# vt-asaplab/porla

Measured on AMD Instinct MI355X. Metric: BN254 G1 MSM Mscalar-mul/s at 2^20 pts, higher is better.
Workload: dtype u32x8 (256-bit modular integer); 1 GPU; KZG scheme, single 2^20-point BN254 G1 MSM per GPU, inputs resident in HBM, output 64-B affine point; pairs_per_gpu=1048576, msm_in_flight=2, warmup_steps_run=38, collective=none (single GPU)

## Files before the change

### include/porla_gpu.h

```cpp
#ifndef PORLA_GPU_H
#define PORLA_GPU_H
#include <stddef.h>
#include <stdint.h>

#if defined(__GNUC__)
#pragma GCC visibility push(default)
#endif
#ifdef __cplusplus
extern "C" {
#endif

#define PORLA_OK            0
#define PORLA_ERR_NO_DEVICE (-1)
#define PORLA_ERR_HIP       (-2)
#define PORLA_ERR_ARG       (-3)
#define PORLA_ERR_STATE     (-4)

#define PORLA_JACOBIAN_BYTES 96
#define PORLA_DIST_ID_BYTES  128

int         porla_gpu_device_count(void);
int         porla_gpu_set_device(int device);
const char *porla_gpu_last_error(void);
int         porla_shard_range(size_t n, int rank, int world, size_t *begin, size_t *end);
int         porla_gpu_profile_enable(int enable);
int         porla_gpu_profile_get(int slot, char *name, size_t name_cap, double *total_ms, long long *launches);
int         porla_gpu_release_msm_workspaces(void);
int         porla_gpu_set_msm_window(int c);
int         porla_gpu_set_msm_small(int on, int window_bits);
int         porla_gpu_set_msm_glv(int on);
int         porla_gpu_last_msm_shape(int *c, int *windows, int *glv);
int         porla_diag_fe_op(int op, int modulus, const uint8_t a_le[32], const uint8_t b_le[32], uint8_t out_le[32]);
int         porla_glv_split(int curve, const uint8_t scalar_be[32], uint8_t k1_mag_be[16], int *k1_neg,
                            uint8_t k2_mag_be[16], int *k2_neg);

int porla_bn254_msm_device(const void *d_scalars, const void *d_points, size_t n, uint8_t out_affine[64],
                           void *hip_stream);
int porla_bn254_msm_device_partial(const void *d_scalars, const void *d_points, size_t n, uint8_t out_jacobian[96],
                                   void *hip_stream);
int porla_bn254_msm_pair_device(const void *d_scalars, const void *d_points_a, const void *d_points_b, size_t n,
                                uint8_t out_a[64], uint8_t out_b[64], void *hip_stream);
int porla_bn254_msm_pair_host(const uint8_t *scalars, const uint8_t *points_a, const uint8_t *points_b, size_t n,
                              uint8_t out_a[64], uint8_t out_b[64]);
int porla_bn254_audit_msm_pair_device(const void *d_store_a, const void *d_store_b, const uint64_t *d_idx, const uint32_t *d_coef,
                                      size_t n, uint8_t out_a[64], uint8_t out_b[64], void *hip_stream);
int porla_bn254_audit_msm_pair_begin(int slot, const void *d_store_a, const void *d_store_b, const uint64_t *d_idx,
                                     const uint32_t *d_coef, size_t n, void *hip_stream);
int porla_bn254_audit_msm_pair_end(int slot, uint8_t out_a[64], uint8_t out_b[64]);
int porla_bn254_msm_device_begin(int slot, const void *d_scalars, const void *d_points, size_t n, void *hip_stream);
int porla_bn254_msm_device_end(int slot, uint8_t *out, int jacobian);
int porla_bn254_msm_host(const uint8_t *scalars, const uint8_t *points, size_t n, uint8_t out_affine[64]);
int porla_bn254_msm_host_multi(const uint8_t *scalars, const uint8_t *points, size_t n, int shards, int devices,
                               uint8_t out_affine[64]);
int porla_gpu_last_msm_multi(int *shards, int *devices);
int porla_bn254_jac_sum(const uint8_t *jacobians, size_t count, uint8_t out_affine[64]);
int porla_bn254_tree_fold(const uint8_t *sums_affine, int windows, int window_bits, uint8_t out_affine[64]);

int porla_secp256k1_msm_device(const void *d_scalars, const void *d_points, size_t n, uint8_t out_affine[64],
                               void *hip_stream);
int porla_secp256k1_msm_pair_device(const void *d_scalars, const void *d_points_a, const void *d_points_b, size_t n,
                                    uint8_t out_a[64], uint8_t out_b[64], void *hip_stream);
int porla_secp256k1_msm_pair_host(const uint8_t *scalars, const uint8_t *points_a, const uint8_t *points_b, size_t n,
                                  uint8_t out_a[64], uint8_t out_b[64]);
int porla_secp256k1_audit_msm_pair_device(const void *d_store_a, const void *d_store_b, const uint64_t *d_idx,
                                          const uint32_t *d_coef, size_t n, uint8_t out_a[64], uint8_t out_b[64], void *hip_stream);
int porla_secp256k1_audit_msm_pair_begin(int slot, const void *d_store_a, const void *d_store_b, const uint64_t *d_idx,
                                         const uint32_t *d_coef, size_t n, void *hip_stream);
int porla_secp256k1_audit_msm_pair_end(int slot, uint8_t out_a[64], uint8_t out_b[64]);
int porla_secp256k1_msm_device_partial(const void *d_scalars, const void *d_points, size_t n,
                                       uint8_t out_jacobian[96], void *hip_stream);
int porla_secp256k1_msm_device_begin(int slot, const void *d_scalars, const void *d_points, size_t n, void *hip_stream);
int porla_secp256k1_msm_device_end(int slot, uint8_t *out, int jacobian);
int porla_secp256k1_msm_host(const uint8_t *scalars, const uint8_t *points, size_t n, uint8_t out_affine[64]);
int porla_secp256k1_msm_host_multi(const uint8_t *scalars, const uint8_t *points, size_t n, int shards, int devices,
                                   uint8_t out_affine[64]);
int porla_secp256k1_jac_sum(const uint8_t *jacobians, size_t count, uint8_t out_affine[64]);
int porla_secp256k1_tree_fold(const uint8_t *sums_affine, int windows, int window_bits, uint8_t out_affine[64]);

int porla_bn254_msm_batch_device(const void *d_scalars, const void *d_points, const uint64_t *offsets, size_t k,
                                 void *d_out, void *hip_stream);
int porla_bn254_msm_batch_host(const uint8_t *scalars, const uint8_t *points, const uint64_t *offsets, size_t k,
                               uint8_t *out);
int porla_secp256k1_msm_batch_device(const void *d_scalars, const void *d_points, const uint64_t *offsets, size_t k,
                                     void *d_out, void *hip_stream);
int porla_secp256k1_msm_batch_host(const uint8_t *scalars, const uint8_t *points, const uint64_t *offsets, size_t k,
                                   uint8_t *out);

int porla_dist_unique_id(uint8_t id_out[PORLA_DIST_ID_BYTES]);
int porla_dist_init(const uint8_t id[PORLA_DIST_ID_BYTES], int rank, int world);
int porla_dist_info(int *rank, int *world);
int porla_dist_finalize(void);
int porla_dist_allgather_partials(const uint8_t partial[PORLA_JACOBIAN_BYTES], uint8_t *all_out );
int porla_bn254_dist_fold(const uint8_t partial[PORLA_JACOBIAN_BYTES], uint8_t out_affine[64]);
int porla_secp256k1_dist_fold(const uint8_t partial[PORLA_JACOBIAN_BYTES], uint8_t out_affine[64]);
int porla_bn254_msm_device_dist(const void *d_scalars, const void *d_points, size_t n_local, uint8_t out_affine[64],
                                void *hip_stream);
int porla_secp256k1_msm_device_dist(const void *d_scalars, const void *d_points, size_t n_local, uint8_t out_affine[64],
                                    void *hip_stream);

typedef struct porla_fixed_base porla_fixed_base;
int  porla_fixed_base_create(int curve, const uint8_t *points, size_t n_points, int window_bits, porla_fixed_base **out);
int  porla_fixed_base_info(const porla_fixed_base *fb, int *window_bits, int *windows, unsigned long long *table_bytes);
int  porla_fixed_base_commit_device(porla_fixed_base *fb, const void *d_rows, size_t n_rows, size_t n_coeffs,
                                    size_t row_stride, void *d_out, void *hip_stream);
int  porla_fixed_base_commit_host(porla_fixed_base *fb, const uint8_t *rows, size_t n_rows, size_t n_coeffs,
                                  size_t row_stride, uint8_t *out);
int porla_ipa_audit_device(porla_fixed_base *generators_fb, const void *d_rows64, const uint64_t *d_idx64,
                           const uint32_t *d_coef64, size_t n64, const void *d_rows32, const uint64_t *d_idx32,
                           const uint32_t *d_coef32, size_t n32, size_t n_cols, const void *d_mac_store,
                           const void *d_align_store, const uint64_t *d_mac_idx, const uint32_t *d_mac_coef, size_t n_macs,
                           uint8_t combined_mac[64], uint8_t combined_align[64], uint8_t align_value[64],
                           uint8_t commitment[64], uint8_t *b_out, void *hip_stream);
void porla_fixed_base_destroy(porla_fixed_base *fb);
int  porla_kzg_commit_batch_device(const void *d_rows, size_t n_rows, void *d_out, void *hip_stream);
int  porla_kzg_commit_batch_host(const uint8_t *rows, size_t n_rows, uint8_t *out);
int  porla_kzg_audit_device(const void *d_rows64, const uint64_t *d_idx64, const uint32_t *d_coef64, size_t n64,
                            const void *d_rows32, const uint64_t *d_idx32, const uint32_t *d_coef32, size_t n32,
                            const void *d_mac_store, const void *d_align_store, const uint64_t *d_mac_idx,
                            const uint32_t *d_mac_coef, size_t n_macs, unsigned long long random_point,
                            uint8_t combined_mac[64], uint8_t combined_align[64], uint8_t align_value[64],
                            uint8_t commitment[64], uint8_t proof_h[64], uint8_t proof_point[32], uint8_t proof_claim[32],
                            uint8_t *b_out, void *hip_stream);
#define PORLA_KZG_AUDIT_RECORD_BYTES 320
#define PORLA_KZG_AUDIT_REQ_BYTES    112
typedef struct {
    const void *d_rows64; const uint64_t *d_idx64; const uint32_t *d_coef64; size_t n64;
    const void *d_rows32; const uint64_t *d_idx32; const uint32_t *d_coef32; size_t n32;
    const void *d_mac_store; const void *d_align_store;
    const uint64_t *d_mac_idx; const uint32_t *d_mac_coef; size_t n_macs;
    unsigned long long random_point;
} porla_kzg_audit_req;
int  porla_kzg_audit_batch_device(const porla_kzg_audit_req *reqs, size_t k, void *d_out, void *d_b_out, void *hip_stream);
#define PORLA_IPA_AUDIT_RECORD_BYTES 655
#define PORLA_IPA_PROOF_BYTES        556
#define PORLA_IPA_AUDIT_REQ_BYTES    136
typedef struct {
    const void *d_rows64; const uint64_t *d_idx64; const uint32_t *d_coef64; size_t n64;
    const void *d_rows32; const uint64_t *d_idx32; const uint32_t *d_coef32; size_t n32;
    const void *d_mac_store; const void *d_align_store;
    const uint64_t *d_mac_idx; const uint32_t *d_mac_coef; size_t n_macs;
    uint8_t a_value[32];
} porla_ipa_audit_req;
int  porla_ipa_audit_batch_device(porla_fixed_base *gens_u_fb, const porla_ipa_audit_req *reqs, size_t k, void *d_out,
                                  void *d_b_out, void *hip_stream);
int  porla_ipa_prove_batch_device(porla_fixed_base *gens_u_fb, const void *d_a, const void *d_b, size_t k, void *d_proofs,
                                  void *hip_stream);
#define PORLA_IPA_VERIFY_REQ_BYTES 96
#define PORLA_IPA_VERIFY_FULL      1
#define PORLA_IPA_VERIFY_PROOF     2
#define PORLA_IPA_VERIFY_MALFORMED 4
#define PORLA_IPA_VERIFY_BVEC      8
typedef struct {
    const void *d_comp_store;
    const uint64_t *d_idx; const uint32_t *d_coef; size_t n;
    uint8_t alpha[32];
    uint8_t a_value[32];
} porla_ipa_verify_req;
int  porla_ipa_verify_batch_device(porla_fixed_base *gens_u_fb, const porla_ipa_verify_req *reqs, size_t k, const void *d_records,
                                   uint8_t *d_status, void *hip_stream);
#define PORLA_KZG_VERIFY_REQ_BYTES 64
#define PORLA_KZG_VERIFY_MAX_K     10922
#define PORLA_KZG_VERIFY_FULL      1
#define PORLA_KZG_VERIFY_PROOF     2
#define PORLA_KZG_VERIFY_MALFORMED 4
typedef struct {
    const void *d_comp_store;
    const uint64_t *d_idx; const uint32_t *d_coef; size_t n;
    uint8_t alpha[32];
} porla_kzg_verify_req;
int  porla_kzg_verify_batch_device(const porla_kzg_verify_req *reqs, size_t k, const void *d_records, const uint8_t *weights,
                                   uint8_t *status, void *hip_stream);
int  porla_kzg_crebuild_stage_device(const void *d_rows_in, size_t n_rows, unsigned long long write_step, void *d_aligned_x,
                                     void *d_aligned_y, void *d_scalars_xy, void *d_commits_xy, const void *d_macs_in,
                                     void *d_macs_x, void *d_macs_y, void *hip_stream);
int  porla_kzg_commit_batch_device_to_host(const void *d_rows, size_t n_rows, uint8_t *out , void *hip_stream);
int  porla_kzg_commit_batch_host_multi(const uint8_t *rows, size_t n_rows, uint8_t *out, int devices);
int  porla_kzg_release_device_memory(void);
int  porla_kzg_digest_batch_device(const void *d_rows, size_t n_rows, void *d_out, void *hip_stream);
int  porla_kzg_complement_batch_device(const void *d_scalars, size_t n, void *d_out, void *hip_stream);
int  porla_kzg_mac_batch_device(const void *d_rows, const void *d_scalars, size_t n_rows, void *d_out, void *hip_stream);
int  porla_kzg_digest_batch_host(const uint8_t *rows, size_t n_rows, uint8_t *out);
int  porla_kzg_complement_batch_host(const uint8_t *scalars, size_t n, uint8_t *out);
int  porla_kzg_mac_batch_host(const uint8_t *rows, const uint8_t *scalars, size_t n_rows, uint8_t *out);
int  porla_bn254_g2_mul_generator(const uint8_t scalar_be[32], uint8_t out[128]);
// ... 341 lines not shown
```

### porla_amd/csrc/engine.hip

```cpp
#include "engine.hpp"
#include "host_fold64.hpp"
#include "../../include/porla_gpu.h"

#include <cstdio>
#include <cstdlib>
#include <mutex>
#include <vector>

namespace porla {

static thread_local std::string g_last_error;
void set_last_error(const std::string& s) { g_last_error = s; }
int hip_fail(hipError_t e, const char* what, const char* file, int line) {
    char buf[512];
    snprintf(buf, sizeof buf, "HIP error %d (%s) at %s:%d: %s", (int)e, hipGetErrorString(e), file, line, what);
    set_last_error(buf);
    return PORLA_ERR_HIP;
}

int ensure_device() {
    static std::once_flag once;
    static int status = PORLA_ERR_NO_DEVICE;
    std::call_once(once, [] {
        int n = 0;
        hipError_t e = hipGetDeviceCount(&n);
        if (e != hipSuccess || n <= 0) {
            set_last_error("porla: no HIP device available (the MSM path has no CPU fallback)");
            status = PORLA_ERR_NO_DEVICE;
            return;
        }
        status = PORLA_OK;
    });
    if (status != PORLA_OK) set_last_error("porla: no HIP device available (the MSM path has no CPU fallback)");
    return status;
}

struct ProfSlot { std::string name; double ms = 0; long long launches = 0; };
struct PendingEv { int slot; int dev; hipEvent_t e0, e1; };
static std::mutex g_prof_mu;
static int g_prof_level = 0;
static std::vector<ProfSlot> g_prof;
static std::vector<PendingEv> g_pending;

static int prof_slot(const char* name) {
    for (size_t i = 0; i < g_prof.size(); i++) if (g_prof[i].name == name) return (int)i;
    g_prof.push_back(ProfSlot{name, 0, 0});
    return (int)g_prof.size() - 1;
}
constexpr int MAX_DEVICES = 16;
static std::vector<hipEvent_t> g_event_pool[MAX_DEVICES];
static int current_device_index() {
    int d = 0;
    if (hipGetDevice(&d) != hipSuccess || d < 0 || d >= MAX_DEVICES) d = 0;
    return d;
}
static hipEvent_t take_event(int dev) {
    auto& pool = g_event_pool[dev];
    if (!pool.empty()) { hipEvent_t e = pool.back(); pool.pop_back(); return e; }
    hipEvent_t e = nullptr;
    (void)hipEventCreate(&e);
    return e;
}
ProfScope::ProfScope(const char* name, hipStream_t s, bool dominant) : slot(-1), stream(s), e0(nullptr), e1(nullptr), on(false) {
    std::lock_guard<std::mutex> lk(g_prof_mu);
    if (g_prof_level == 0 || (g_prof_level == 2 && !dominant)) return;
    on = true;
    slot = prof_slot(name);
    const int dev = current_device_index();
    e0 = take_event(dev);
    e1 = take_event(dev);
    (void)hipEventRecord(e0, stream);
}
ProfScope::~ProfScope() {
    if (!on) return;
    (void)hipEventRecord(e1, stream);
    std::lock_guard<std::mutex> lk(g_prof_mu);
    g_pending.push_back(PendingEv{slot, current_device_index(), e0, e1});
}
void prof_flush() {
    std::lock_guard<std::mutex> lk(g_prof_mu);
    for (auto& p : g_pending) {
        float ms = 0;
        (void)hipEventSynchronize(p.e1);
        if (hipEventElapsedTime(&ms, p.e0, p.e1) == hipSuccess) {
            g_prof[p.slot].ms += ms;
            g_prof[p.slot].launches += 1;
        }
        g_event_pool[p.dev].push_back(p.e0);
        g_event_pool[p.dev].push_back(p.e1);
    }
    g_pending.clear();
}

std::mutex g_ws_mu;
static std::vector<Workspace*> g_ws;
int g_window_override = 0;
int g_small_mode = getenv("PORLA_MSM_SMALL") ? atoi(getenv("PORLA_MSM_SMALL")) : 1;
int g_small_c = 0;
int g_last_shape[3] = {0, 0, 0};
int g_last_multi[2] = {0, 0};
std::mutex g_multi_mu;
int g_use_glv = -1;

int get_workspace_slot(int slot, Workspace** out) {
    if (slot < 0 || slot >= MSM_SLOTS) { set_last_error("porla: MSM slot out of range"); return PORLA_ERR_ARG; }
    int dev = 0;
    PORLA_HIP(hipGetDevice(&dev));
    std::lock_guard<std::mutex> lk(g_ws_mu);
    for (auto* w : g_ws) if (w->device == dev && w->slot == slot) { *out = w; return PORLA_OK; }
    Workspace* w = new Workspace();
    w->device = dev;
    w->slot = slot;
    PORLA_HIP(hipStreamCreateWithFlags(&w->own_stream, hipStreamNonBlocking));
    g_ws.push_back(w);
    *out = w;
    return PORLA_OK;
}
int get_workspace(Workspace** out) { return get_workspace_slot(0, out); }
int lease_blocking_slot(Workspace** out) {
    Workspace* w0 = nullptr;
    int rc = get_workspace_slot(0, &w0);
    if (rc) return rc;
    if (w0->mu.try_lock()) { *out = w0; return PORLA_OK; }
    for (int k = MSM_POOL_SLOT0; k < MSM_POOL_SLOT0 + MSM_POOL_SLOTS; k++) {
        Workspace* w = nullptr;
        if ((rc = get_workspace_slot(k, &w))) return rc;
        if (w->mu.try_lock()) { *out = w; return PORLA_OK; }
    }
    w0->mu.lock();
    *out = w0;
    return PORLA_OK;
}

template <class C>
static int abi_msm_device(const void* d_scalars, const void* d_points, size_t n, uint8_t* out, void* stream, bool jac) {
    using M = typename C::Fp;
    if (n && (!d_scalars || !d_points || !out)) { set_last_error("porla: null argument"); return PORLA_ERR_ARG; }
    XYZZ<M> tot;
    int rc = msm_device<C>((const uint8_t*)d_scalars, (const uint8_t*)d_points, n, (hipStream_t)stream, &tot);
    if (rc) return rc;
    if (jac) h_xyzz_to_jac_bytes<M>(out, tot);
    else h_affine_to_bytes<M>(out, h_xyzz_to_affine64<M>(tot));
    return PORLA_OK;
}
template <class C>
static int abi_msm_host(const uint8_t* scalars, const uint8_t* points, size_t n, uint8_t* out) {
    using M = typename C::Fp;
    if (n && (!scalars || !points || !out)) { set_last_error("porla: null argument"); return PORLA_ERR_ARG; }
    XYZZ<M> tot;
    int rc = msm_host<C>(scalars, points, n, &tot);
    if (rc) return rc;
    h_affine_to_bytes<M>(out, h_xyzz_to_affine64<M>(tot));
    return PORLA_OK;
}
template <class C>
static int abi_msm_pair(const void* scalars, const void* points_a, const void* points_b, size_t n, uint8_t* out_a, uint8_t* out_b, void* stream,
                        bool device) {
    using M = typename C::Fp;
    if (!out_a || !out_b || (n && (!scalars || !points_a || !points_b))) { set_last_error("porla: null argument"); return PORLA_ERR_ARG; }
    XYZZ<M> ta, tb;
    int rc = device ? msm_pair_device<C>((const uint8_t*)scalars, (const uint8_t*)points_a, (const uint8_t*)points_b, n, (hipStream_t)stream, &ta, &tb)
                    : msm_pair_host<C>((const uint8_t*)scalars, (const uint8_t*)points_a, (const uint8_t*)points_b, n, &ta, &tb);
    if (rc) return rc;
    h_affine_to_bytes<M>(out_a, h_xyzz_to_affine64<M>(ta));
    h_affine_to_bytes<M>(out_b, h_xyzz_to_affine64<M>(tb));
    return PORLA_OK;
}
template <class C>
static int abi_audit_msm_pair(const void* d_store_a, const void* d_store_b, const uint64_t* d_idx, const uint32_t* d_coef, size_t n,
                              uint8_t* out_a, uint8_t* out_b, void* stream) {
    using M = typename C::Fp;
    if (!out_a || !out_b || (n && (!d_store_a || !d_store_b || !d_idx || !d_coef))) { set_last_error("porla: null argument"); return PORLA_ERR_ARG; }
    XYZZ<M> ta, tb;
    int rc = msm_pair_gather_device<C>((const uint8_t*)d_store_a, (const uint8_t*)d_store_b, d_idx, d_coef, n, (hipStream_t)stream, &ta, &tb);
    if (rc) return rc;
    h_affine_to_bytes<M>(out_a, h_xyzz_to_affine64<M>(ta));
    h_affine_to_bytes<M>(out_b, h_xyzz_to_affine64<M>(tb));
    return PORLA_OK;
}
static int batch_check(const char* curve, const void* scalars, const void* points, const uint64_t* offsets, size_t k, const void* out) {
    if (k == 0) return PORLA_OK;
    if (!offsets || !out) { set_last_error("porla: null argument (offsets / output of a batched MSM)"); return PORLA_ERR_ARG; }
    if (offsets[0] != 0) { set_last_error("porla: batched MSM offsets must start at 0"); return PORLA_ERR_ARG; }
    for (size_t e = 0; e < k; e++) {
        if (offsets[e + 1] < offsets[e]) { set_last_error("porla: batched MSM offsets must be non-decreasing"); return PORLA_ERR_ARG; }
        if (offsets[e + 1] - offsets[e] > SMALL_MAX_N) {
            set_last_error(std::string("porla: a batched MSM entry holds at most 32768 pairs (entry ") + std::to_string(e) + " has " +
                           std::to_string(offsets[e + 1] - offsets[e]) + "): use porla_" + curve + "_msm_device for large MSMs");
            return PORLA_ERR_ARG;
        }
    }
    const uint64_t total = offsets[k];
    if (total > (uint64_t)(SIZE_MAX / 64) || k > SIZE_MAX / 64) { set_last_error("porla: batched MSM total overflows"); return PORLA_ERR_ARG; }
    if (total && (!scalars || !points)) { set_last_error("porla: null argument (scalars / points of a batched MSM)"); return PORLA_ERR_ARG; }
    return PORLA_OK;
}
template <class C>
static int abi_msm_batch(const char* curve, const void* scalars, const void* points, const uint64_t* offsets, size_t k, void* out,
                         void* stream, bool device) {
    int rc = batch_check(curve, scalars, points, offsets, k, out);
    if (rc) return rc;
    if (k == 0) return PORLA_OK;
    if (device) {
        return msm_batch_device<C>((const uint8_t*)scalars, (const uint8_t*)points, offsets, k, (uint8_t*)out, (hipStream_t)stream);
    }
    return msm_batch_host<C>((const uint8_t*)scalars, (const uint8_t*)points, offsets, k, (uint8_t*)out);
}
template <class C>
static int abi_msm_host_multi(const uint8_t* scalars, const uint8_t* points, size_t n, int shards, int devices, uint8_t* out) {
    using M = typename C::Fp;
    if (n && (!scalars || !points || !out)) { set_last_error("porla: null argument"); return PORLA_ERR_ARG; }
    XYZZ<M> tot;
    int rc = msm_host_multi<C>(scalars, points, n, shards, devices, &tot);
    if (rc) return rc;
    h_affine_to_bytes<M>(out, h_xyzz_to_affine64<M>(tot));
    return PORLA_OK;
}
template <class C>
static int abi_tree_fold(const uint8_t* sums, int W, int c, uint8_t* out) {
    using M = typename C::Fp;
    if (W < 1 || c < 2 || c > 20 || !sums || !out) { set_last_error("porla: bad argument"); return PORLA_ERR_ARG; }
    std::vector<XYZZ<M>> fin((size_t)W * c);
    for (size_t i = 0; i < fin.size(); i++) fin[i] = xyzz_from_affine<M>(h_affine_from_bytes<M>(sums + 64 * i));
    h_affine_to_bytes<M>(out, h_xyzz_to_affine64<M>(h_fold_tree64<M>(fin.data(), W, c)));
    return PORLA_OK;
}
template <class C>
static int abi_jac_sum(const uint8_t* jacs, size_t count, uint8_t* out) {
    using M = typename C::Fp;
    if (count && !jacs) { set_last_error("porla: null argument"); return PORLA_ERR_ARG; }
    XYZZ<M> acc = xyzz_inf<M>();
    for (size_t i = 0; i < count; i++) {
        XYZZ<M> p = h_xyzz_from_jac_bytes<M>(jacs + 96 * i);
        xyzz_add<M>(acc, p);
    }
    h_affine_to_bytes<M>(out, h_xyzz_to_affine64<M>(acc));
    return PORLA_OK;
}

int order_after_caller(Workspace* ws, hipStream_t caller, hipStream_t a, hipStream_t b) {
    if (hipStreamQuery(caller) == hipSuccess) return PORLA_OK;
    (void)hipGetLastError();
    if (!ws->caller_ev) PORLA_HIP(hipEventCreateWithFlags(&ws->caller_ev, hipEventDisableTiming));
    PORLA_HIP(hipEventRecord(ws->caller_ev, caller));
    if (a && a != caller) PORLA_HIP(hipStreamWaitEvent(a, ws->caller_ev, 0));
    if (b && b != caller && b != a) PORLA_HIP(hipStreamWaitEvent(b, ws->caller_ev, 0));
    return PORLA_OK;
}

hipStream_t engine_stream() {
    Workspace* ws;
    if (get_workspace(&ws)) return nullptr;
    return ws->own_stream;
}

}

using namespace porla;

namespace {
struct IccSecp256k1FnHost {
    static constexpr uint32_t P[8] = {0xd0364141u, 0xbfd25e8cu, 0xaf48a03bu, 0xbaaedce6u, 0xfffffffeu, 0xffffffffu, 0xffffffffu, 0xffffffffu};
    static constexpr int SPARE_BITS = 0;
};
}

extern "C" {

int porla_gpu_device_count(void) {
    int n = 0;
    if (hipGetDeviceCount(&n) != hipSuccess) return 0;
    return n;
}
int porla_gpu_set_device(int device) {
    PORLA_HIP(hipSetDevice(device));
    return PORLA_OK;
}
const char* porla_gpu_last_error(void) { return g_last_error.c_str(); }

int porla_gpu_profile_enable(int enable) {
    prof_flush();
    std::lock_guard<std::mutex> lk(g_prof_mu);
    g_prof_level = enable < 0 ? 0 : (enable > 2 ? 1 : enable);
    if (enable) g_prof.clear();
    return PORLA_OK;
}
int porla_gpu_profile_get(int slot, char* name, size_t name_cap, double* total_ms, long long* launches) {
    prof_flush();
    std::lock_guard<std::mutex> lk(g_prof_mu);
    if (slot < 0 || (size_t)slot >= g_prof.size()) return PORLA_ERR_ARG;
    if (name && name_cap) snprintf(name, name_cap, "%s", g_prof[slot].name.c_str());
    if (total_ms) *total_ms = g_prof[slot].ms;
    if (launches) *launches = g_prof[slot].launches;
    return PORLA_OK;
}
int porla_gpu_release_msm_workspaces(void) {
    std::lock_guard<std::mutex> lk(g_ws_mu);
    std::vector<Workspace*> held;
    auto unlock_all = [&]() { for (auto* w : held) w->mu.unlock(); };
    for (auto* w : g_ws) {
        if (!w->mu.try_lock()) { unlock_all(); set_last_error("porla: an MSM is running on a workspace slot"); return PORLA_ERR_STATE; }
        held.push_back(w);
        if (w->pend_W || w->begun) { unlock_all(); set_last_error("porla: an MSM is still pending (call the matching _end first)"); return PORLA_ERR_STATE; }
    }
    int cur = 0;
    (void)hipGetDevice(&cur);
    for (auto* w : g_ws) {
        (void)hipSetDevice(w->device);
        Buf* bufs[] = {&w->pts, &w->keys, &w->entries, &w->counts, &w->starts, &w->fill, &w->cursor, &w->buckets, &w->in_scalars,
                       &w->in_points, &w->order, &w->blk_hist, &w->blk_off, &w->tile_off, &w->heavy, &w->chunk_out, &w->tree_s,
                       &w->tree_m, &w->tree_mt, &w->small_part, &w->multi_acc, &w->batch_list, &w->batch_part, &w->batch_sums,
                       &w->batch_ctrl, &w->batch_out};
        for (Buf* b : bufs) b->release();
        w->batch_list_h.release();
        w->batch_fence.reset();
    }
    (void)hipSetDevice(cur);
    unlock_all();
    return PORLA_OK;
}
int porla_shard_range(size_t n, int rank, int world, size_t* begin, size_t* end) {
    if (world < 1 || rank < 0 || rank >= world || !begin || !end) { set_last_error("porla: bad shard"); return PORLA_ERR_ARG; }
    *begin = (size_t)((unsigned __int128)n * (unsigned)rank / (unsigned)world);
    *end = (size_t)((unsigned __int128)n * (unsigned)(rank + 1) / (unsigned)world);
    return PORLA_OK;
}
int porla_gpu_set_msm_window(int c) { g_window_override = c; return PORLA_OK; }
int porla_gpu_last_msm_shape(int* c, int* windows, int* glv) {
    if (c) *c = g_last_shape[0];
    if (windows) *windows = g_last_shape[1];
    if (glv) *glv = g_last_shape[2];
    return PORLA_OK;
}
int porla_gpu_set_msm_small(int on, int window_bits) {
    g_small_mode = on != 0;
    g_small_c = window_bits >= 1 && window_bits <= SMALL_MAX_C ? window_bits : 0;
    return PORLA_OK;
}
int porla_gpu_set_msm_glv(int on) { g_use_glv = on < 0 ? -1 : (on != 0); return PORLA_OK; }

int porla_glv_split(int curve, const uint8_t scalar_be[32], uint8_t k1_mag_be[16], int* k1_neg, uint8_t k2_mag_be[16], int* k2_neg) {
    if (!scalar_be || !k1_mag_be || !k2_mag_be || !k1_neg || !k2_neg || (curve != 0 && curve != 1)) return PORLA_ERR_ARG;
    uint32_t k[8], m1[4], m2[4];
    bool n1, n2;
    h_load_be(k, scalar_be);
    if (curve == 0) { fe_reduce_plain<Bn254Fr>(k, 8); glv_split<GlvBn254>(k, m1, n1, m2, n2); }
    else { fe_reduce_plain<IccSecp256k1FnHost>(k, 2); glv_split<GlvSecp256k1>(k, m1, n1, m2, n2); }
    for (int i = 0; i < 4; i++) {
        for (int b = 0; b < 4; b++) {
            k1_mag_be[15 - (4 * i + b)] = (uint8_t)(m1[i] >> (8 * b));
            k2_mag_be[15 - (4 * i + b)] = (uint8_t)(m2[i] >> (8 * b));
        }
    }
    *k1_neg = n1; *k2_neg = n2;
    return PORLA_OK;
}

int porla_diag_fe_op(int op, int modulus, const uint8_t a_le[32], const uint8_t b_le[32], uint8_t out_le[32]) {
    if (!a_le || !out_le || (modulus != 0 && modulus != 1) || op < 0 || op > 4 || (op >= 3 && !b_le)) return PORLA_ERR_ARG;
    uint32_t a[8], b[8] = {0, 0, 0, 0, 0, 0, 0, 0}, r[8];
    for (int i = 0; i < 8; i++) {
        a[i] = (uint32_t)a_le[4 * i] | ((uint32_t)a_le[4 * i + 1] << 8) | ((uint32_t)a_le[4 * i + 2] << 16) | ((uint32_t)a_le[4 * i + 3] << 24);
        if (b_le) b[i] = (uint32_t)b_le[4 * i] | ((uint32_t)b_le[4 * i + 1] << 8) | ((uint32_t)b_le[4 * i + 2] << 16) | ((uint32_t)b_le[4 * i + 3] << 24);
    }
    auto run = [&](auto tag, auto ktag) {
        using M = decltype(tag);
        constexpr int K = decltype(ktag)::value;
        Fe<M> x, y, z;
        for (int i = 0; i < 8; i++) { x.v[i] = a[i]; y.v[i] = b[i]; }
        if (op == 0) { for (int i = 0; i < 8; i++) r[i] = a[i]; fe_reduce_small<M, K>(r); return; }
        if (op == 1) z = fe_neg<M>(x);
        else if (op == 2) z = fe_neg_if<M>(x, true);
        else if (op == 3) z = fe_sub<M>(x, y);
        else z = fe_add<M>(x, y);
        for (int i = 0; i < 8; i++) r[i] = z.v[i];
    };
    if (modulus == 0) run(Bn254Fr{}, std::integral_constant<int, 4>{});
    else run(IccSecp256k1FnHost{}, std::integral_constant<int, 0>{});
    for (int i = 0; i < 8; i++)
        for (int k = 0; k < 4; k++) out_le[4 * i + k] = (uint8_t)(r[i] >> (8 * k));
    return PORLA_OK;
}

int porla_bn254_msm_device(const void* d_scalars, const void* d_points, size_t n, uint8_t out_affine[64], void* s) {
    return abi_msm_device<Bn254G1>(d_scalars, d_points, n, out_affine, s, false);
}
int porla_bn254_msm_batch_device(const void* d_scalars, const void* d_points, const uint64_t* offsets, size_t k, void* d_out, void* s) {
    return abi_msm_batch<Bn254G1>("bn254", d_scalars, d_points, offsets, k, d_out, s, true);
}
int porla_bn254_msm_batch_host(const uint8_t* scalars, const uint8_t* points, const uint64_t* offsets, size_t k, uint8_t* out) {
    return abi_msm_batch<Bn254G1>("bn254", scalars, points, offsets, k, out, nullptr, false);
}
int porla_secp256k1_msm_batch_device(const void* d_scalars, const void* d_points, const uint64_t* offsets, size_t k, void* d_out, void* s) {
    return abi_msm_batch<Secp256k1G>("secp256k1", d_scalars, d_points, offsets, k, d_out, s, true);
}
int porla_secp256k1_msm_batch_host(const uint8_t* scalars, const uint8_t* points, const uint64_t* offsets, size_t k, uint8_t* out) {
    return abi_msm_batch<Secp256k1G>("secp256k1", scalars, points, offsets, k, out, nullptr, false);
}
int porla_bn254_msm_device_partial(const void* d_scalars, const void* d_points, size_t n, uint8_t out_jac[96], void* s) {
    return abi_msm_device<Bn254G1>(d_scalars, d_points, n, out_jac, s, true);
}
int porla_bn254_msm_host(const uint8_t* scalars, const uint8_t* points, size_t n, uint8_t out_affine[64]) {
    return abi_msm_host<Bn254G1>(scalars, points, n, out_affine);
}
int porla_bn254_msm_pair_device(const void* d_scalars, const void* d_points_a, const void* d_points_b, size_t n, uint8_t out_a[64],
                                uint8_t out_b[64], void* s) {
    return abi_msm_pair<Bn254G1>(d_scalars, d_points_a, d_points_b, n, out_a, out_b, s, true);
}
int porla_bn254_msm_pair_host(const uint8_t* scalars, const uint8_t* points_a, const uint8_t* points_b, size_t n, uint8_t out_a[64],
                              uint8_t out_b[64]) {
    return abi_msm_pair<Bn254G1>(scalars, points_a, points_b, n, out_a, out_b, nullptr, false);
}
int porla_bn254_audit_msm_pair_device(const void* d_store_a, const void* d_store_b, const uint64_t* d_idx, const uint32_t* d_coef, size_t n,
                                      uint8_t out_a[64], uint8_t out_b[64], void* s) {
    return abi_audit_msm_pair<Bn254G1>(d_store_a, d_store_b, d_idx, d_coef, n, out_a, out_b, s);
}
int porla_bn254_audit_msm_pair_begin(int slot, const void* d_store_a, const void* d_store_b, const uint64_t* d_idx, const uint32_t* d_coef,
                                     size_t n, void* s) {
    if (!d_store_a || !d_store_b || !d_idx || !d_coef) { set_last_error("porla: null argument"); return PORLA_ERR_ARG; }
    if (slot < 1 || slot >= MSM_USER_SLOTS) { set_last_error("porla: MSM slot out of range (1 .. 3; 0 belongs to the blocking calls)"); return PORLA_ERR_ARG; }
    return msm_pair_gather_begin<Bn254G1>(slot, (const uint8_t*)d_store_a, (const uint8_t*)d_store_b, d_idx, d_coef, n, (hipStream_t)s);
}
int porla_bn254_audit_msm_pair_end(int slot, uint8_t out_a[64], uint8_t out_b[64]) {
    if (!out_a || !out_b) { set_last_error("porla: null argument"); return PORLA_ERR_ARG; }
    if (slot < 1 || slot >= MSM_USER_SLOTS) { set_last_error("porla: MSM slot out of range (1 .. 3; 0 belongs to the blocking calls)"); return PORLA_ERR_ARG; }
    XYZZ<Bn254Fp> ta, tb;
    int rc = msm_pair_end<Bn254G1>(slot, &ta, &tb);
    if (rc) return rc;
    h_affine_to_bytes<Bn254Fp>(out_a, h_xyzz_to_affine64<Bn254Fp>(ta));
    h_affine_to_bytes<Bn254Fp>(out_b, h_xyzz_to_affine64<Bn254Fp>(tb));
    return PORLA_OK;
}
int porla_bn254_msm_host_multi(const uint8_t* scalars, const uint8_t* points, size_t n, int shards, int devices, uint8_t out_affine[64]) {
    return abi_msm_host_multi<Bn254G1>(scalars, points, n, shards, devices, out_affine);
}
int porla_secp256k1_msm_pair_device(const void* d_scalars, const void* d_points_a, const void* d_points_b, size_t n, uint8_t out_a[64],
                                    uint8_t out_b[64], void* s) {
    return abi_msm_pair<Secp256k1G>(d_scalars, d_points_a, d_points_b, n, out_a, out_b, s, true);
}
int porla_secp256k1_msm_pair_host(const uint8_t* scalars, const uint8_t* points_a, const uint8_t* points_b, size_t n, uint8_t out_a[64],
                                  uint8_t out_b[64]) {
    return abi_msm_pair<Secp256k1G>(scalars, points_a, points_b, n, out_a, out_b, nullptr, false);
}
int porla_secp256k1_audit_msm_pair_device(const void* d_store_a, const void* d_store_b, const uint64_t* d_idx, const uint32_t* d_coef,
                                          size_t n, uint8_t out_a[64], uint8_t out_b[64], void* s) {
    return abi_audit_msm_pair<Secp256k1G>(d_store_a, d_store_b, d_idx, d_coef, n, out_a, out_b, s);
}
int porla_secp256k1_audit_msm_pair_begin(int slot, const void* d_store_a, const void* d_store_b, const uint64_t* d_idx, const uint32_t* d_coef,
                                         size_t n, void* s) {
    if (!d_store_a || !d_store_b || !d_idx || !d_coef) { set_last_error("porla: null argument"); return PORLA_ERR_ARG; }
    if (slot < 1 || slot >= MSM_USER_SLOTS) { set_last_error("porla: MSM slot out of range (1 .. 3; 0 belongs to the blocking calls)"); return PORLA_ERR_ARG; }
    return msm_pair_gather_begin<Secp256k1G>(slot, (const uint8_t*)d_store_a, (const uint8_t*)d_store_b, d_idx, d_coef, n, (hipStream_t)s);
}
int porla_secp256k1_audit_msm_pair_end(int slot, uint8_t out_a[64], uint8_t out_b[64]) {
    if (!out_a || !out_b) { set_last_error("porla: null argument"); return PORLA_ERR_ARG; }
    if (slot < 1 || slot >= MSM_USER_SLOTS) { set_last_error("porla: MSM slot out of range (1 .. 3; 0 belongs to the blocking calls)"); return PORLA_ERR_ARG; }
    XYZZ<Secp256k1Fp> ta, tb;
    int rc = msm_pair_end<Secp256k1G>(slot, &ta, &tb);
    if (rc) return rc;
    h_affine_to_bytes<Secp256k1Fp>(out_a, h_xyzz_to_affine64<Secp256k1Fp>(ta));
    h_affine_to_bytes<Secp256k1Fp>(out_b, h_xyzz_to_affine64<Secp256k1Fp>(tb));
    return PORLA_OK;
}
int porla_secp256k1_msm_host_multi(const uint8_t* scalars, const uint8_t* points, size_t n, int shards, int devices, uint8_t out_affine[64]) {
    return abi_msm_host_multi<Secp256k1G>(scalars, points, n, shards, devices, out_affine);
}
int porla_gpu_last_msm_multi(int* shards, int* devices) {
    if (shards) *shards = g_last_multi[0];
    if (devices) *devices = g_last_multi[1];
    return PORLA_OK;
}
int porla_bn254_jac_sum(const uint8_t* jacs, size_t count, uint8_t out_affine[64]) {
    return abi_jac_sum<Bn254G1>(jacs, count, out_affine);
}
int porla_bn254_tree_fold(const uint8_t* sums, int windows, int window_bits, uint8_t out_affine[64]) {
    return abi_tree_fold<Bn254G1>(sums, windows, window_bits, out_affine);
}
int porla_secp256k1_tree_fold(const uint8_t* sums, int windows, int window_bits, uint8_t out_affine[64]) {
    return abi_tree_fold<Secp256k1G>(sums, windows, window_bits, out_affine);
}

static int user_slot_ok(int slot) {
    if (slot >= 0 && slot < MSM_USER_SLOTS) return PORLA_OK;
    set_last_error("porla: MSM slot out of range (0..3)");
    return PORLA_ERR_ARG;
}
int porla_bn254_msm_device_begin(int slot, const void* d_scalars, const void* d_points, size_t n, void* s) {
    if (user_slot_ok(slot)) return PORLA_ERR_ARG;
    if (n && (!d_scalars || !d_points)) { set_last_error("porla: null argument"); return PORLA_ERR_ARG; }
    return msm_device_begin<Bn254G1>(slot, (const uint8_t*)d_scalars, (const uint8_t*)d_points, n, (hipStream_t)s);
}
int porla_bn254_msm_device_end(int slot, uint8_t* out, int jacobian) {
    if (user_slot_ok(slot)) return PORLA_ERR_ARG;
    if (!out) { set_last_error("porla: null argument"); return PORLA_ERR_ARG; }
    XYZZ<Bn254Fp> tot;
    int rc = msm_device_end<Bn254G1>(slot, &tot);
    if (rc) return rc;
    if (jacobian) h_xyzz_to_jac_bytes<Bn254Fp>(out, tot);
    else h_affine_to_bytes<Bn254Fp>(out, h_xyzz_to_affine64<Bn254Fp>(tot));
    return PORLA_OK;
}

int porla_secp256k1_msm_device_begin(int slot, const void* d_scalars, const void* d_points, size_t n, void* s) {
    if (user_slot_ok(slot)) return PORLA_ERR_ARG;
    if (n && (!d_scalars || !d_points)) { set_last_error("porla: null argument"); return PORLA_ERR_ARG; }
    return msm_device_begin<Secp256k1G>(slot, (const uint8_t*)d_scalars, (const uint8_t*)d_points, n, (hipStream_t)s);
}
int porla_secp256k1_msm_device_end(int slot, uint8_t* out, int jacobian) {
    if (user_slot_ok(slot)) return PORLA_ERR_ARG;
    if (!out) { set_last_error("porla: null argument"); return PORLA_ERR_ARG; }
    XYZZ<Secp256k1Fp> tot;
    int rc = msm_device_end<Secp256k1G>(slot, &tot);
    if (rc) return rc;
    if (jacobian) h_xyzz_to_jac_bytes<Secp256k1Fp>(out, tot);
    else h_affine_to_bytes<Secp256k1Fp>(out, h_xyzz_to_affine64<Secp256k1Fp>(tot));
    return PORLA_OK;
}

int porla_secp256k1_msm_device(const void* d_scalars, const void* d_points, size_t n, uint8_t out_affine[64], void* s) {
    return abi_msm_device<Secp256k1G>(d_scalars, d_points, n, out_affine, s, false);
}
int porla_secp256k1_msm_device_partial(const void* d_scalars, const void* d_points, size_t n, uint8_t out_jac[96], void* s) {
    return abi_msm_device<Secp256k1G>(d_scalars, d_points, n, out_jac, s, true);
}
int porla_secp256k1_msm_host(const uint8_t* scalars, const uint8_t* points, size_t n, uint8_t out_affine[64]) {
    return abi_msm_host<Secp256k1G>(scalars, points, n, out_affine);
}
int porla_secp256k1_jac_sum(const uint8_t* jacs, size_t count, uint8_t out_affine[64]) {
    return abi_jac_sum<Secp256k1G>(jacs, count, out_affine);
}

int porla_icc_mac_scale_host(const uint8_t mac_in[64], size_t n_total, unsigned long long write_step, int curve, uint8_t mac_out[64]) {
    if (!mac_in || !mac_out || (curve != 0 && curve != 1)) { set_last_error("porla: bad argument"); return PORLA_ERR_ARG; }
    uint8_t wt[32];
    int rc = icc_wt_scalar_be(n_total, write_step, wt);
    if (rc) return rc;
    uint32_t k[8];
    h_load_be(k, wt);
    if (curve == 0) {
        fe_reduce_plain<Bn254Fr>(k, 8);
        h_affine_to_bytes<Bn254Fp>(mac_out, h_xyzz_to_affine64<Bn254Fp>(h_scalar_mul64_glv<Bn254Fp, GlvBn254>(h_affine_from_bytes<Bn254Fp>(mac_in), k)));
    } else {
        fe_reduce_plain<IccSecp256k1FnHost>(k, 2);
        h_affine_to_bytes<Secp256k1Fp>(mac_out, h_xyzz_to_affine64<Secp256k1Fp>(h_scalar_mul64_glv<Secp256k1Fp, GlvSecp256k1>(h_affine_from_bytes<Secp256k1Fp>(mac_in), k)));
    }
    return PORLA_OK;
}

int porla_fixed_base_create(int curve, const uint8_t* points, size_t n_points, int window_bits, porla_fixed_base** out) {
    if (!out || (n_points && !points) || (curve != 0 && curve != 1)) { set_last_error("porla: bad argument"); return PORLA_ERR_ARG; }
    int rc = ensure_device();
    if (rc) return rc;
    hipStream_t s = engine_stream();
    porla_fixed_base* fb = new porla_fixed_base();
    fb->curve = curve;
    rc = curve == 0 ? fb->bn.build_from_host_bytes(points, n_points, window_bits, s)
                    : fb->secp.build_from_host_bytes(points, n_points, window_bits, s);
    if (rc) { porla_fixed_base_destroy(fb); return rc; }
    *out = fb;
    return PORLA_OK;
}
int porla_fixed_base_info(const porla_fixed_base* fb, int* window_bits, int* windows, unsigned long long* table_bytes) {
    if (!fb) return PORLA_ERR_ARG;
    int c = fb->curve == 0 ? fb->bn.c : fb->secp.c, W = fb->curve == 0 ? fb->bn.W : fb->secp.W;
    size_t n = fb->curve == 0 ? fb->bn.n_points : fb->secp.n_points;
    if (window_bits) *window_bits = c;
    if (windows) *windows = W;
    if (table_bytes) *table_bytes = c ? (unsigned long long)n * W * ((size_t)1 << (c - 1)) * 64 : 0;
    return PORLA_OK;
}
int porla_fixed_base_commit_device(porla_fixed_base* fb, const void* d_rows, size_t n_rows, size_t n_coeffs,
                                   size_t row_stride, void* d_out, void* stream) {
    if (!fb || (n_rows && (!d_rows || !d_out))) { set_last_error("porla: null argument"); return PORLA_ERR_ARG; }
    if (fb->curve == 0) {
        std::lock_guard<std::mutex> lk(fb->bn.mu);
        return fb->bn.commit_device((const uint8_t*)d_rows, n_rows, n_coeffs, row_stride, (uint8_t*)d_out, (hipStream_t)stream);
    }
    std::lock_guard<std::mutex> lk(fb->secp.mu);
    return fb->secp.commit_device((const uint8_t*)d_rows, n_rows, n_coeffs, row_stride, (uint8_t*)d_out, (hipStream_t)stream);
}
int porla_fixed_base_commit_host(porla_fixed_base* fb, const uint8_t* rows, size_t n_rows, size_t n_coeffs,
                                 size_t row_stride, uint8_t* out) {
    if (!fb || (n_rows && (!rows || !out))) { set_last_error("porla: null argument"); return PORLA_ERR_ARG; }
    hipStream_t s = engine_stream();
    if (fb->curve == 0) {
        std::lock_guard<std::mutex> lk(fb->bn.mu);
        return fb->bn.commit_host(rows, n_rows, n_coeffs, row_stride, out, s);
    }
    std::lock_guard<std::mutex> lk(fb->secp.mu);
    return fb->secp.commit_host(rows, n_rows, n_coeffs, row_stride, out, s);
}
static std::mutex g_ipa_audit_mu;
static uint8_t* g_ipa_pin = nullptr;
static size_t g_ipa_pin_cap = 0;
static int g_ipa_pin_dev = -1;
int porla_ipa_audit_device(porla_fixed_base* generators_fb, const void* d_rows64, const uint64_t* d_idx64, const uint32_t* d_coef64,
                           size_t n64, const void* d_rows32, const uint64_t* d_idx32, const uint32_t* d_coef32, size_t n32, size_t n_cols,
                           const void* d_mac_store, const void* d_align_store, const uint64_t* d_mac_idx, const uint32_t* d_mac_coef,
                           size_t n_macs, uint8_t combined_mac[64], uint8_t combined_align[64], uint8_t align_value[64],
                           uint8_t commitment[64], uint8_t* b_out, void* hip_stream) {
    if (!generators_fb || generators_fb->curve != 1 || !combined_mac || !combined_align || !align_value || !commitment || n_cols == 0 ||
        (n_macs && (!d_mac_store || !d_align_store || !d_mac_idx || !d_mac_coef))) {
        set_last_error("porla: bad argument to porla_ipa_audit_device (generators_fb must be a secp256k1 fixed base)");
        return PORLA_ERR_ARG;
    }
    int rc = ensure_device();
    if (rc) return rc;
    std::lock_guard<std::mutex> lk(g_ipa_audit_mu);
    int dev = 0;
    PORLA_HIP(hipGetDevice(&dev));
    if (g_ipa_pin_cap < 64 * n_cols || g_ipa_pin_dev != dev) {
        if (g_ipa_pin) PORLA_HIP(hipHostFree(g_ipa_pin));
        g_ipa_pin = nullptr; g_ipa_pin_cap = 0;
        PORLA_HIP(hipHostMalloc((void**)&g_ipa_pin, 64 * n_cols, hipHostMallocMapped | hipHostMallocCoherent));
        g_ipa_pin_cap = 64 * n_cols;
        g_ipa_pin_dev = dev;
    }
    void* pin_dev = nullptr;
    PORLA_HIP(hipHostGetDevicePointer(&pin_dev, g_ipa_pin, 0));
    hipStream_t stream = (hipStream_t)hip_stream;
    Workspace* aw = nullptr;
    if ((rc = get_workspace_slot(MSM_AUDIT_SLOT, &aw))) return rc;
    if ((rc = order_after_caller(aw, (hipStream_t)hip_stream, stream, aw->own_stream))) return rc;
    rc = porla_audit_combine_device(d_rows64, d_idx64, d_coef64, n64, d_rows32, d_idx32, d_coef32, n32, n_cols, 1, nullptr, nullptr,
                                    pin_dev, (uint8_t*)pin_dev + 32 * n_cols, stream);
    const bool pair = n_macs >= 1 && n_macs <= 32768;
    bool pair_begun = false;
    if (rc == PORLA_OK && pair) {
        rc = msm_pair_gather_begin<Secp256k1G>(MSM_AUDIT_SLOT, (const uint8_t*)d_mac_store, (const uint8_t*)d_align_store, d_mac_idx,
                                                   d_mac_coef, n_macs, aw->own_stream);
        pair_begun = rc == PORLA_OK;
    }
    auto collect_pair = [&]() -> int {
        if (!pair_begun) return PORLA_OK;
        XYZZ<Secp256k1Fp> ta, tb;
        int r2 = msm_pair_end<Secp256k1G>(MSM_AUDIT_SLOT, &ta, &tb);
        if (r2) return r2;
        h_affine_to_bytes<Secp256k1Fp>(combined_mac, h_xyzz_to_affine64<Secp256k1Fp>(ta));
        h_affine_to_bytes<Secp256k1Fp>(combined_align, h_xyzz_to_affine64<Secp256k1Fp>(tb));
        return PORLA_OK;
    };
    if (rc == PORLA_OK && hipStreamSynchronize(stream) != hipSuccess) {
        set_last_error("porla: hipStreamSynchronize failed in the audit");
        rc = PORLA_ERR_HIP;
    }
    if (rc) { (void)collect_pair(); return rc; }
    std::vector<uint8_t> two(64 * n_cols);
    memcpy(two.data(), g_ipa_pin + 32 * n_cols, 32 * n_cols);
    memcpy(two.data() + 32 * n_cols, g_ipa_pin, 32 * n_cols);
    if (b_out) memcpy(b_out, g_ipa_pin, 32 * n_cols);
    uint8_t outs[128];
    {
        std::lock_guard<std::mutex> lkfb(generators_fb->secp.mu);
        rc = generators_fb->secp.commit_host(two.data(), 2, n_cols, 32 * n_cols, outs, engine_stream());
    }
    int rc2 = collect_pair();
    if (rc) return rc;
    if (rc2) return rc2;
    if (!pair && (rc = porla_secp256k1_audit_msm_pair_device(d_mac_store, d_align_store, d_mac_idx, d_mac_coef, n_macs, combined_mac,
                                                             combined_align, stream)))
        return rc;
    memcpy(align_value, outs, 64);
    memcpy(commitment, outs + 64, 64);
    return PORLA_OK;
}

void porla_fixed_base_destroy(porla_fixed_base* fb) {
    if (!fb) return;
// ... 7 lines not shown
```

### porla_amd/csrc/engine.hpp

```cpp
#pragma once
#include <hip/hip_runtime.h>
#include <cstddef>
#include <cstdint>
#include <mutex>
#include <string>
#include <utility>
#include <vector>
#include "../../include/porla_gpu.h"
#include "host_curve.hpp"
#include "msm.hip.h"
#include "msm_small.hip.h"

namespace porla {

void set_last_error(const std::string& s);
int hip_fail(hipError_t e, const char* what, const char* file, int line);

#define PORLA_HIP(call)                                                      \
    do {                                                                     \
        hipError_t _e = (call);                                              \
        if (_e != hipSuccess) return ::porla::hip_fail(_e, #call, __FILE__, __LINE__); \
    } while (0)

struct ProfScope {
    ProfScope(const char* name, hipStream_t s, bool dominant = false);
    ~ProfScope();
    int slot;
    hipStream_t stream;
    hipEvent_t e0, e1;
    bool on;
};
void prof_flush();

template <class C>
int msm_device(const uint8_t* d_scalars, const uint8_t* d_points, size_t n, hipStream_t stream,
               XYZZ<typename C::Fp>* total);

template <class C>
int msm_pair_device(const uint8_t* d_scalars, const uint8_t* d_points_a, const uint8_t* d_points_b, size_t n, hipStream_t stream,
                    XYZZ<typename C::Fp>* total_a, XYZZ<typename C::Fp>* total_b);
template <class C>
int msm_pair_gather_device(const uint8_t* d_store_a, const uint8_t* d_store_b, const uint64_t* d_idx, const uint32_t* d_coef, size_t n,
                           hipStream_t stream, XYZZ<typename C::Fp>* total_a, XYZZ<typename C::Fp>* total_b);
template <class C>
int msm_pair_gather_begin(int slot, const uint8_t* d_store_a, const uint8_t* d_store_b, const uint64_t* d_idx, const uint32_t* d_coef, size_t n,
                          hipStream_t stream);
template <class C>
int msm_pair_end(int slot, XYZZ<typename C::Fp>* total_a, XYZZ<typename C::Fp>* total_b);
template <class C>
int msm_pair_host(const uint8_t* scalars, const uint8_t* points_a, const uint8_t* points_b, size_t n, XYZZ<typename C::Fp>* total_a,
                  XYZZ<typename C::Fp>* total_b);
template <class C>
int msm_batch_device(const uint8_t* d_scalars, const uint8_t* d_points, const uint64_t* offsets, size_t k, uint8_t* d_out, hipStream_t stream);
template <class C>
int msm_batch_host(const uint8_t* scalars, const uint8_t* points, const uint64_t* offsets, size_t k, uint8_t* out);
template <class C>
int msm_batch_sums_device(const uint8_t* d_scalars, const uint8_t* d_points, const uint64_t* offsets, size_t k, XYZZ<typename C::Fp>* d_sums,
                          hipStream_t stream);
template <class C>
int msm_device_begin(int slot, const uint8_t* d_scalars, const uint8_t* d_points, size_t n, hipStream_t stream);
template <class C>
int msm_device_end(int slot, XYZZ<typename C::Fp>* total);

template <class C>
int msm_host(const uint8_t* scalars, const uint8_t* points, size_t n, XYZZ<typename C::Fp>* total);
template <class C>
int msm_host_multi(const uint8_t* scalars, const uint8_t* points, size_t n, int shards, int devices,
                   XYZZ<typename C::Fp>* total);

int ensure_device();

struct Buf {
    void* p = nullptr;
    size_t cap = 0;
    int ensure(size_t bytes) {
        if (bytes <= cap) return PORLA_OK;
        if (p) PORLA_HIP(hipFree(p));
        p = nullptr; cap = 0;
        size_t want = bytes + bytes / 8 + 256;
        PORLA_HIP(hipMalloc(&p, want));
        cap = want;
        return PORLA_OK;
    }
    void release() {
        if (p) (void)hipFree(p);
        p = nullptr; cap = 0;
    }
};
struct UseFence {
    hipEvent_t ev = nullptr;
    hipStream_t last = nullptr;
    bool used = false;
    int enter(hipStream_t s) {
        if (used && last != s) PORLA_HIP(hipStreamWaitEvent(s, ev, 0));
        return PORLA_OK;
    }
    int leave(hipStream_t s) {
        if (!ev) PORLA_HIP(hipEventCreateWithFlags(&ev, hipEventDisableTiming));
        PORLA_HIP(hipEventRecord(ev, s));
        last = s;
        used = true;
        return PORLA_OK;
    }
    void reset() { if (ev) (void)hipEventDestroy(ev); ev = nullptr; used = false; last = nullptr; }
};

struct PinnedList {
    void* h = nullptr;
    size_t cap = 0;
    hipEvent_t upload = nullptr;
    std::vector<std::pair<void*, hipEvent_t>> retired;
    int stage(size_t bytes) {
        for (size_t i = 0; i < retired.size();) {
            const hipError_t q = hipEventQuery(retired[i].second);
            if (q == hipErrorNotReady) { i++; continue; }
            PORLA_HIP(q);
            PORLA_HIP(hipHostFree(retired[i].first));
            PORLA_HIP(hipEventDestroy(retired[i].second));
            retired.erase(retired.begin() + (long)i);
        }
        if (upload) {
            const hipError_t q = hipEventQuery(upload);
            if (q == hipErrorNotReady) {
                retired.emplace_back(h, upload);
                h = nullptr;
                cap = 0;
                upload = nullptr;
            } else {
                PORLA_HIP(q);
            }
        }
        if (cap < bytes) {
            if (h) PORLA_HIP(hipHostFree(h));
            h = nullptr;
            cap = 0;
            PORLA_HIP(hipHostMalloc(&h, bytes + bytes / 4 + 4096, hipHostMallocDefault));
            cap = bytes + bytes / 4 + 4096;
        }
        return PORLA_OK;
    }
    int send(void* dst, size_t bytes, hipStream_t stream) {
        PORLA_HIP(hipMemcpyAsync(dst, h, bytes, hipMemcpyHostToDevice, stream));
        if (!upload) PORLA_HIP(hipEventCreateWithFlags(&upload, hipEventDisableTiming));
        PORLA_HIP(hipEventRecord(upload, stream));
        return PORLA_OK;
    }
    void release() {
        if (h) retired.emplace_back(h, upload);
        for (auto& rb : retired) {
            if (rb.second) {
                (void)hipEventSynchronize(rb.second);
                (void)hipEventDestroy(rb.second);
            }
            (void)hipHostFree(rb.first);
        }
        retired.clear();
        h = nullptr;
        cap = 0;
        upload = nullptr;
    }
};

struct Workspace {
    std::mutex mu;
    int device = -1;
    Buf pts, keys, entries, counts, starts, fill, cursor, buckets, in_scalars, in_points;
    Buf order, blk_hist, blk_off, tile_off, heavy, chunk_out;
    Buf small_part;
    uint32_t small_seq = 0;
    Buf tree_s, tree_m, tree_mt;
    Buf multi_acc;
    hipEvent_t merged = nullptr;
    void* h_windows = nullptr;
    size_t h_windows_cap = 0;
    hipStream_t own_stream = nullptr;
    hipStream_t aux_stream = nullptr;
    hipEvent_t fork_ev = nullptr, join_ev = nullptr;
    hipEvent_t front_fork_ev = nullptr, front_join_ev = nullptr;
    hipEvent_t caller_ev = nullptr;
    int slot = 0;
    hipEvent_t done = nullptr;
    int pend_W = 0, pend_c = 0;
    bool lone = false;
    bool pair_pending = false;
    bool begun = false;
    Buf batch_list, batch_part, batch_sums, batch_ctrl, batch_out;
    PinnedList batch_list_h;
    UseFence batch_fence;
};
constexpr int MSM_SLOTS = 17;
constexpr int MSM_POOL_SLOTS = 8;
constexpr int MSM_AUDIT_SLOT = 16;
constexpr int MSM_USER_SLOTS = 4;
constexpr int MSM_MULTI_SLOT0 = 4;
constexpr int MSM_MULTI_SLOTS = 4;
constexpr int MSM_POOL_SLOT0 = 8;
int order_after_caller(Workspace* ws, hipStream_t caller, hipStream_t a, hipStream_t b = nullptr);
constexpr size_t MSM_SCAN_MAX = 1u << 16;
constexpr size_t MSM_RANGE_MAX = 1u << 22;
template <class C>
struct FixedBase {
    int device = -1;
    int c = 0, W = 0;
    size_t n_points = 0;
    Affine<typename C::Fp>* table = nullptr;
    size_t table_cap = 0;
    XYZZ<typename C::Fp>* pow_buf = nullptr;
    size_t pow_cap = 0;
    XYZZ<typename C::Fp>* scratch_buf = nullptr;
    size_t scratch_cap = 0;
    bool keep_build_buffers = false;
    XYZZ<typename C::Fp>* partial = nullptr;
    size_t partial_cap = 0;
    uint8_t* io_rows = nullptr;
    size_t io_rows_cap = 0;
    uint8_t* io_out = nullptr;
    size_t io_out_cap = 0;
    hipStream_t io_stream2 = nullptr;
    uint32_t last_S = 1;
    UseFence fence;
    static constexpr size_t HOST_FINISH_MAX_ROWS = 256;
    void* h_small = nullptr;
    void* d_small = nullptr;
    uint32_t small_seq = 0;
    hipEvent_t small_done = nullptr;
    std::mutex mu;
    void release();
    int build(const Affine<typename C::Fp>* d_base, size_t n, int window_bits, hipStream_t stream);
    int build_from_host_bytes(const uint8_t* points_be, size_t n, int window_bits, hipStream_t stream);
    int commit_device(const uint8_t* d_rows, size_t n_rows, size_t n_coeffs, size_t row_stride, uint8_t* d_out,
                      hipStream_t stream, bool guest_room = false);
    int commit_host(const uint8_t* rows, size_t n_rows, size_t n_coeffs, size_t row_stride, uint8_t* out,
                    hipStream_t stream);
    int commit_small(const uint8_t* const* row_ptrs, size_t n_rows, size_t n_coeffs, uint8_t* const* outs, hipStream_t stream,
                     const uint8_t* d_rows = nullptr, XYZZ<typename C::Fp>* raw_sums = nullptr);
    static bool small_ok(size_t n_rows, size_t n_coeffs);
};

}
struct porla_fixed_base {
    int curve;
    porla::FixedBase<porla::Bn254G1> bn;
    porla::FixedBase<porla::Secp256k1G> secp;
};
namespace porla {

extern std::mutex g_ws_mu;
extern int g_window_override;
extern int g_small_mode;
extern int g_small_c;
extern int g_last_multi[2];
extern int g_last_shape[3];
extern int g_use_glv;
int get_workspace(Workspace** out);
int get_workspace_slot(int slot, Workspace** out);
int lease_blocking_slot(Workspace** out);
hipStream_t engine_stream();

int icc_wt_scalar_be(size_t n_total, unsigned long long write_step, uint8_t out[32]);
int icc_wt_residues(int curve, size_t n_total, unsigned long long write_step, uint32_t wt_p[8], uint32_t wt_q[8], uint8_t plain_be[32]);
int icc_mix_tables_acquire(int curve, size_t n_total, hipStream_t stream, const uint32_t** tw30);
int icc_mix_tables_release(hipStream_t stream);
int icc_encode_tables_acquire(int curve, size_t n_total, hipStream_t stream, const uint32_t** twp, const uint32_t** twq);
int icc_decode_tables_acquire(int curve, size_t n_total, bool want_q, hipStream_t stream, const uint32_t** twp, const uint32_t** twqi);
int mac_mix_tables_acquire(int curve, size_t n_total, hipStream_t stream, const uint32_t** tws, int* quad_max_log);
int mac_mix_tables_release(hipStream_t stream);
void mac_stages_leased(int curve, void* work, size_t points, size_t n_total, bool quad, const uint32_t* tws, const char* scope,
                       hipStream_t stream);
int icc_network_matrix_device(int curve, size_t n, unsigned long long write_step, int part, uint8_t* d_rows_out,
                              hipStream_t stream);

struct KzgAuditDesc {
    const uint8_t* rows64; const uint64_t* idx64; const uint32_t* coef64;
    const uint8_t* rows32; const uint64_t* idx32; const uint32_t* coef32;
    const uint8_t* mac_store; const uint8_t* align_store; const uint64_t* mac_idx; const uint32_t* mac_coef;
    uint32_t n64, n32, n_macs, blk0, nblk, gat0;
    unsigned long long z;
    unsigned long long pair0;
};
static_assert(sizeof(KzgAuditDesc) == 120, "KzgAuditDesc: 80 bytes of pointers, 24 of counts, z, pair0");
int audit_combine_batch_launch(const KzgAuditDesc* d_desc, const uint32_t* d_blk_audit, uint32_t n_blocks, uint32_t k, uint32_t n_cols,
                               uint32_t per_slice, void* d_partial, int curve, uint8_t* d_sc, uint8_t* d_be, size_t audit_stride,
                               hipStream_t stream);
size_t audit_combine_partial_bytes(uint32_t n_blocks, uint32_t n_cols);
constexpr uint32_t AUDIT_BATCH_SLICES = 8;

}
```

### porla_amd/csrc/host_fold64.hpp

```cpp
#pragma once
#include "ec.hip.h"
#include "glv.hip.h"
#include <memory>
#include <mutex>
#include <vector>

namespace porla {

template <class M>
struct Fp64 {
    typedef unsigned __int128 u128;
    uint64_t p[4];
    uint64_t inv;
    Fp64() {
        for (int i = 0; i < 4; i++) p[i] = ((uint64_t)M::P[2 * i + 1] << 32) | M::P[2 * i];
        uint64_t x = 1;
        for (int i = 0; i < 6; i++) x *= 2 - p[0] * x;
        inv = 0 - x;
        adx = false;
#if PORLA_FP64_ADX
        adx = !M::PSEUDO_MERSENNE && (p[3] >> 63) == 0 && host_has_adx();
        adx_pm = M::PSEUDO_MERSENNE && host_has_adx();
#endif
    }
// ... 251 lines not shown
}

template <class M, class G>
inline XYZZ<M> h_scalar_mul64_glv(const Affine<M>& a, const uint32_t k[8]) {
    static const Fp64<M> F;
    typedef typename Fp64<M>::Pt Pt;
    typedef typename Fp64<M>::E E;
    if (aff_is_inf<M>(a)) return xyzz_inf<M>();
    uint32_t nz = 0;
    for (int i = 0; i < 8; i++) nz |= k[i];
    if (!nz) return xyzz_inf<M>();
    static const E beta = [] {
        Fe<M> b, r2;
        for (int i = 0; i < 8; i++) { b.v[i] = G::BETA[i]; r2.v[i] = M::R2[i]; }
        return F.mul(Fp64<M>::from(b), Fp64<M>::from(r2));
    }();
    uint32_t m[2][4];
    bool ng[2];
    glv_split<G>(k, m[0], ng[0], m[1], ng[1]);
    Pt tbl[2][8];
    tbl[0][0].x = Fp64<M>::from(a.x); tbl[0][0].y = Fp64<M>::from(a.y); tbl[0][0].zz = F.one(); tbl[0][0].zzz = F.one();
    for (int i = 1; i < 8; i++) tbl[0][i] = F.padd(tbl[0][i - 1], tbl[0][0]);
    for (int i = 0; i < 8; i++) { tbl[1][i] = tbl[0][i]; tbl[1][i].x = F.mul(tbl[1][i].x, beta); }
    int8_t dig[2][33];
    for (int h = 0; h < 2; h++) {
        uint32_t carry = 0;
        for (int i = 0; i < 32; i++) {
            const uint32_t d = ((m[h][i >> 3] >> ((i & 7) * 4)) & 15u) + carry;
            if (d > 8) { dig[h][i] = (int8_t)((int)d - 16); carry = 1; }
            else { dig[h][i] = (int8_t)d; carry = 0; }
        }
        dig[h][32] = (int8_t)carry;
    }
    Pt acc = F.inf();
    E zero;
    for (int i = 0; i < 4; i++) zero.v[i] = 0;
    for (int i = 32; i >= 0; i--) {
        if (!Fp64<M>::is_zero(acc.zz)) for (int d = 0; d < 4; d++) acc = F.dbl(acc);
        for (int h = 0; h < 2; h++) {
            const int d = dig[h][i];
            if (!d) continue;
            Pt t = tbl[h][(d < 0 ? -d : d) - 1];
            if ((d < 0) != ng[h]) t.y = F.sub(zero, t.y);
            acc = F.padd(acc, t);
        }
    }
    return F.to(acc);
}

template <class M>
inline void h_batch_xyzz_to_affine64(const XYZZ<M>* in, size_t n, Affine<M>* out) {
    static const Fp64<M> F;
    typedef typename Fp64<M>::E E;
    constexpr size_t MAXN = 64;
    E d[MAXN], pre[MAXN];
    for (size_t base = 0; base < n; base += MAXN) {
        const size_t m = n - base < MAXN ? n - base : MAXN;
        E acc = F.one();
        for (size_t i = 0; i < m; i++) {
            const XYZZ<M>& q = in[base + i];
            d[i] = xyzz_is_inf<M>(q) ? F.one() : F.mul(Fp64<M>::from(q.zz), Fp64<M>::from(q.zzz));
            pre[i] = acc;
            acc = F.mul(acc, d[i]);
        }
        E inv = F.inverse(acc);
        for (size_t i = m; i-- > 0;) {
            const XYZZ<M>& q = in[base + i];
            const E di = F.mul(inv, pre[i]);
            inv = F.mul(inv, d[i]);
            Affine<M>& r = out[base + i];
            if (xyzz_is_inf<M>(q)) { r.x = fe_zero<M>(); r.y = fe_zero<M>(); continue; }
            r.x = Fp64<M>::to(F.mul(Fp64<M>::from(q.x), F.mul(di, Fp64<M>::from(q.zzz))));
            r.y = Fp64<M>::to(F.mul(Fp64<M>::from(q.y), F.mul(di, Fp64<M>::from(q.zz))));
        }
    }
}

template <class M>
struct HostFixedBase {
    typedef std::vector<Affine<M>> Table;
    std::mutex mu;
    Affine<M> base;
    std::shared_ptr<const Table> tab;
    static bool same(const Affine<M>& a, const Affine<M>& b) {
        for (int i = 0; i < 8; i++) if (a.x.v[i] != b.x.v[i] || a.y.v[i] != b.y.v[i]) return false;
        return true;
    }
    static std::shared_ptr<const Table> build(const Affine<M>& b) {
        static const Fp64<M> F;
        typedef typename Fp64<M>::Pt Pt;
        std::vector<XYZZ<M>> proj(65 * 8);
        Pt P;
        P.x = Fp64<M>::from(b.x); P.y = Fp64<M>::from(b.y); P.zz = F.one(); P.zzz = F.one();
        for (int i = 0; i < 65; i++) {
            Pt acc = P;
            for (int j = 0; j < 8; j++) {
                proj[(size_t)i * 8 + j] = F.to(acc);
                if (j < 7) acc = F.padd(acc, P);
            }
            for (int d = 0; d < 4; d++) P = F.dbl(P);
        }
        auto t = std::make_shared<Table>(65 * 8);
        h_batch_xyzz_to_affine64<M>(proj.data(), proj.size(), t->data());
        return t;
    }
    XYZZ<M> mul(const Affine<M>& b, const uint32_t k[8]) {
        static const Fp64<M> F;
        typedef typename Fp64<M>::Pt Pt;
        typedef typename Fp64<M>::E E;
        if (aff_is_inf<M>(b)) return xyzz_inf<M>();
        std::shared_ptr<const Table> t;
        {
            std::lock_guard<std::mutex> lk(mu);
            if (!tab || !same(base, b)) { tab = build(b); base = b; }
            t = tab;
        }
        Pt acc = F.inf();
        E zero;
        for (int i = 0; i < 4; i++) zero.v[i] = 0;
        uint32_t carry = 0;
        for (int i = 0; i < 65; i++) {
            uint32_t d = carry;
            if (i < 64) d += (k[i >> 3] >> ((i & 7) * 4)) & 15u;
            int dg;
            if (d > 8) { dg = (int)d - 16; carry = 1; } else { dg = (int)d; carry = 0; }
            if (dg == 0) continue;
            const Affine<M>& e = (*t)[(size_t)i * 8 + (size_t)((dg < 0 ? -dg : dg) - 1)];
            if (aff_is_inf<M>(e)) continue;
            Pt q;
            q.x = Fp64<M>::from(e.x); q.y = Fp64<M>::from(e.y); q.zz = F.one(); q.zzz = F.one();
            if (dg < 0) q.y = F.sub(zero, q.y);
            acc = F.padd(acc, q);
        }
        return F.to(acc);
    }
};

template <class M>
inline XYZZ<M> h_fold_tree64(const XYZZ<M>* fin, int W, int c) {
    static const Fp64<M> F;
    typename Fp64<M>::Pt acc = F.inf();
    for (int w = W - 1; w >= 0; w--) {
        const XYZZ<M>* f = fin + (size_t)w * c;
        if (!Fp64<M>::is_zero(acc.zz)) acc = F.dbl(acc);
        for (int k = c - 2; k >= 0; k--) {
            if (!Fp64<M>::is_zero(acc.zz)) acc = F.dbl(acc);
            acc = F.padd(acc, F.from(f[1 + k]));
        }
        acc = F.padd(acc, F.from(f[0]));
    }
    return F.to(acc);
}

}
```

### porla_amd/csrc/msm.hip.h

```cpp
#pragma once
#include "ec.hip.h"
#include "ec30.hip.h"
#include "glv.hip.h"
#include <type_traits>

namespace porla {

struct Bn254G1 {
    using Fp = Bn254Fp;
    static constexpr uint32_t ORDER[8] = {0xf0000001u, 0x43e1f593u, 0x79b97091u, 0x2833e848u,
                                          0x8181585du, 0xb85045b6u, 0xe131a029u, 0x30644e72u};
    static constexpr int SCALAR_BITS = 254;
    static constexpr int MAX_Q = 5;
    using Glv = GlvBn254;
    static constexpr bool GLV_DEFAULT = false;
    static constexpr size_t GLV_BELOW = (size_t)1 << 17;
    static constexpr bool F30_BUCKETS = true;
    static constexpr bool F30_LAZY = true;
    static constexpr int BUCKET_SUM_WAVES = 4;
    static constexpr int FB_COMMIT_WAVES = 3;
    static constexpr int MACQ_WAVES = 4;
};
struct Secp256k1G {
    using Fp = Secp256k1Fp;
// ... 596 lines not shown
        for (int k = 0; k < 8; k++) d[k] = z;
    }
    if (full) {
        uint32_t pos = atomicAdd(&next[0], full);
        for (uint32_t j = 0; j < full; j++) order[pos + j] = make_uint2(i, j);
    }
    if (rem) {
        uint32_t pos = atomicAdd(&next[CHUNK - rem], 1u);
        order[pos] = make_uint2(i, full);
    }
    if (items > 1) {
        chunk_base[i] = atomicAdd(&ctrl[1], items);
        heavy_list[atomicAdd(&ctrl[2], 1u)] = i;
    } else {
        chunk_base[i] = NO_CHUNK;
    }
}

template <class C>
__global__ void __launch_bounds__(256) __attribute__((amdgpu_waves_per_eu(C::BUCKET_SUM_WAVES, 4)))
k_bucket_sum30(const Affine<typename C::Fp>* __restrict__ pts, const uint32_t* __restrict__ entries,
               const uint32_t* __restrict__ starts, const uint32_t* __restrict__ counts,
               const uint2* __restrict__ order, const uint32_t* __restrict__ chunk_base,
               const uint32_t* __restrict__ ctrl, XYZZ<typename C::Fp>* __restrict__ buckets,
               XYZZ<typename C::Fp>* __restrict__ chunk_out, uint32_t accumulate) {
    using M = typename C::Fp;
    uint32_t tid = blockIdx.x * blockDim.x + threadIdx.x;
    if (tid >= ctrl[3]) return;
    uint2 item = order[tid];
    const uint32_t b = item.x;
    const uint32_t first = item.y * CHUNK;
    uint32_t cnt = counts[b] - first;
    if (cnt > CHUNK) cnt = CHUNK;
    const uint32_t* e = entries + starts[b] + first;
    const uint32_t cb = chunk_base[b];
    XYZZ30<M> acc = xyzz30_infinity<M>();
    if constexpr (C::F30_LAZY) {
        if (accumulate && cb == NO_CHUNK) acc = xyzz30_load_lazy<M>(buckets + b);
    }
    bool flip = false;
    uint32_t ent = e[0];
    uint32_t k = 0;
    if (acc.inf) {
        const uint32_t cur = ent;
        if (cnt > 1) ent = e[1];
        Affine<M> a = load_affine<M>(pts, cur & 0x7fffffffu);
        if (!aff_is_inf<M>(a)) {
            a = aff_neg_if<M>(a, (cur >> 31) != 0);
            acc.x = f30_from_fe<M>(a.x); acc.y = f30_from_fe<M>(a.y);
            acc.zz = f30_const<M>(M::R1_30); acc.zzz = acc.zz;
            acc.inf = false;
        }
        k = 1;
        if (!acc.inf && cnt > 1) {
            const uint32_t cur2 = ent;
            uint32_t nxt = cur2;
            if (cnt > 2) nxt = e[2];
            Affine<M> a2 = load_affine<M>(pts, cur2 & 0x7fffffffu);
            const bool a2_inf = aff_is_inf<M>(a2);
            a2 = aff_neg_if<M>(a2, xyzz30_flip_neg<M>((cur2 >> 31) != 0, flip));
            if (xyzz30_mmadd_flip_fast<M>(acc, flip, f30_from_fe<M>(a2.x), f30_from_fe<M>(a2.y), a2_inf)) { ent = nxt; k = 2; }
        }
    }
    {
        for (; k < cnt; k++) {
            const uint32_t cur = ent;
            uint32_t nxt = cur;
            if (k + 1 < cnt) nxt = e[k + 1];
            Affine<M> a = load_affine<M>(pts, cur & 0x7fffffffu);
            const bool a_inf = aff_is_inf<M>(a);
            a = aff_neg_if<M>(a, xyzz30_flip_neg<M>((cur >> 31) != 0, flip));
            if (!xyzz30_madd_flip_fast<M>(acc, flip, f30_from_fe<M>(a.x), f30_from_fe<M>(a.y), a_inf)) break;
            ent = nxt;
        }
    }
    for (; k < cnt; k++) {
        const uint32_t cur = ent;
        if (k + 1 < cnt) ent = e[k + 1];
        Affine<M> a = load_affine<M>(pts, cur & 0x7fffffffu);
        if (aff_is_inf<M>(a)) continue;
        a = aff_neg_if<M>(a, xyzz30_flip_neg<M>((cur >> 31) != 0, flip));
        xyzz30_madd_flip<M>(acc, flip, f30_from_fe<M>(a.x), f30_from_fe<M>(a.y));
    }
    xyzz30_flip_finish<M>(acc, flip);
    XYZZ<M>* dst = cb == NO_CHUNK ? buckets + b : chunk_out + cb + item.y;
    if constexpr (C::F30_LAZY) xyzz30_store_lazy<M>(dst, acc);
    else store_xyzz<M>(dst, xyzz30_to_xyzz<M>(acc));
}


template <class M>
__device__ __forceinline__ XYZZ<M> xyzz_shfl_xor(const XYZZ<M>& p, int mask) {
    XYZZ<M> r;
#pragma unroll
    for (int i = 0; i < 8; i++) {
        r.x.v[i] = __shfl_xor(p.x.v[i], mask, 64);
        r.y.v[i] = __shfl_xor(p.y.v[i], mask, 64);
        r.zz.v[i] = __shfl_xor(p.zz.v[i], mask, 64);
        r.zzz.v[i] = __shfl_xor(p.zzz.v[i], mask, 64);
    }
    return r;
}
template <class M>
struct TreeLevelArgs {
    const XYZZ<M>* s_prev;
    const XYZZ<M>* s_prev2;
    const XYZZ<M>* m_prev;
    XYZZ<M>* s_out;
    XYZZ<M>* m_out;
    XYZZ<M>* fin;
    uint32_t n;
    uint32_t m_prev_stride, m_out_stride;
    uint32_t l;
    uint32_t nlev;
    uint32_t last;
};

template <class C>
struct Node {
    using M = typename C::Fp;
    using T = typename std::conditional<C::F30_LAZY, XYZZ30<M>, XYZZ<M>>::type;
    static __device__ __forceinline__ T load(const XYZZ<M>* p) {
        if constexpr (C::F30_LAZY) return xyzz30_load_lazy<M>(p);
        else return load_xyzz<M>(p);
    }
    static __device__ __forceinline__ void add(T& a, const T& b) {
        if constexpr (C::F30_LAZY) xyzz30_add<M>(a, b);
        else xyzz_add_cold<M>(&a, &b);
    }
    static __device__ __forceinline__ void store(XYZZ<M>* p, const T& a) {
        if constexpr (C::F30_LAZY) xyzz30_store_lazy<M>(p, a);
        else store_xyzz<M>(p, a);
    }
    static __device__ __forceinline__ void store_final(XYZZ<M>* p, const T& a) {
        if constexpr (C::F30_LAZY) store_xyzz<M>(p, xyzz30_to_xyzz<M>(a));
        else store_xyzz<M>(p, a);
    }
    static __device__ __forceinline__ T inf() {
        if constexpr (C::F30_LAZY) { T r; r.x = r.y = r.zz = r.zzz = F30<M>{}; r.inf = true; return r; }
        else return xyzz_inf<M>();
    }
};

template <class M>
struct TreeOp {
    const XYZZ<M>*pa, *pb;
    XYZZ<M>* out;
    bool final;
    bool copy;
};
template <class M>
__device__ __forceinline__ TreeOp<M> tree_op(const TreeLevelArgs<M>& a, uint32_t s, uint32_t i, uint32_t jp, uint32_t jo) {
    TreeOp<M> o;
    o.final = a.last != 0;
    o.copy = (s == a.l + 1);
    if (o.copy) {
        o.pa = a.s_prev + 2 * (size_t)i + 1; o.pb = o.pa;
        o.out = a.fin + (size_t)i * (a.nlev + 1) + 1 + a.l;
        return o;
    }
    if (s == a.l) { o.pa = a.s_prev + 2 * (size_t)i; o.pb = o.pa + 1; }
    else if (s + 1 == a.l) { o.pa = a.s_prev2 + 4 * (size_t)i + 1; o.pb = o.pa + 2; }
    else { o.pa = a.m_prev + (size_t)s * a.m_prev_stride + 2 * (size_t)jp; o.pb = o.pa + 1; }
    if (a.last) o.out = a.fin + (size_t)i * (a.nlev + 1) + (s == a.l ? 0 : 1 + s);
    else o.out = (s == a.l) ? a.s_out + i : a.m_out + (size_t)s * a.m_out_stride + jo;
    return o;
}
template <class C>
__device__ __forceinline__ void tree_task(const TreeLevelArgs<typename C::Fp>& a, uint32_t s, uint32_t i, uint32_t jp, uint32_t jo) {
    using M = typename C::Fp;
    using N = Node<C>;
    const TreeOp<M> o = tree_op<M>(a, s, i, jp, jo);
    typename N::T x = N::load(o.pa);
    if (!o.copy) {
        typename N::T y = N::load(o.pb);
        N::add(x, y);
    }
    if (o.final) N::store_final(o.out, x);
    else N::store(o.out, x);
}
template <class C>
__device__ __forceinline__ void tree_task_quad(const TreeLevelArgs<typename C::Fp>& a, uint32_t s, uint32_t i, uint32_t jp, uint32_t jo,
                                               bool live, uint32_t lane) {
    using M = typename C::Fp;
    const TreeOp<M> o = tree_op<M>(a, s, i, jp, jo);
    if (o.copy) {
        if (live && (lane & 3u) == 0u) Node<C>::store_final(o.out, Node<C>::load(o.pa));
        return;
    }
    xyzz30_add_quad<M>(o.pa, o.pb, o.out, o.final, live, lane);
}

template <class C>
__global__ void __launch_bounds__(256)
k_tree_level(TreeLevelArgs<typename C::Fp> a) {
    uint32_t t = blockIdx.x * blockDim.x + threadIdx.x;
    uint32_t slots = a.l + 1 + a.last;
    if (t >= slots * a.n) return;
    const uint32_t i = t % a.n;
    tree_task<C>(a, t / a.n, i, i, i);
}

template <class C>
__global__ void __launch_bounds__(256)
k_tree_level_quad(TreeLevelArgs<typename C::Fp> a) {
    const uint32_t tid = blockIdx.x * blockDim.x + threadIdx.x;
    const uint32_t total = (a.l + 1 + a.last) * a.n;
    uint32_t t = tid >> 2;
    const bool live = t < total;
    if (!live) t = total - 1;
    const uint32_t i = t % a.n;
    tree_task_quad<C>(a, t / a.n, i, i, i, live, threadIdx.x & 63u);
}

template <class C>
__global__ void __launch_bounds__(256)
k_tree_front2(TreeLevelArgs<typename C::Fp> a, XYZZ<typename C::Fp>* __restrict__ s1_out) {
    using M = typename C::Fp;
    using N = Node<C>;
    const uint32_t i = blockIdx.x * blockDim.x + threadIdx.x;
    if (i >= a.n) return;
    const XYZZ<M>* bk = a.s_prev + 4 * (size_t)i;
    typename N::T x = N::inf(), y = N::inf(), keep = N::inf();
#pragma unroll 1
    for (uint32_t s = 0; s < 4; s++) {
        if (s == 0) { x = N::load(bk); y = N::load(bk + 1); }
        else if (s == 1) { x = y; y = N::load(bk + 3); }
        else if (s == 2) { x = N::load(bk + 2); }
        else { y = x; x = keep; }
        N::add(x, y);
        if (s == 0) keep = x;
        else N::store(s == 1 ? a.m_out + i : (s == 2 ? a.s_out + 2 * (size_t)i + 1 : s1_out + i), x);
    }
}

template <class M>
struct TreeTailArgs {
    const XYZZ<M>* buckets;
    XYZZ<M>* s_lev[24];
    const XYZZ<M>* m_global;
    XYZZ<M>* m_tail[2];
    XYZZ<M>* fin;
    uint32_t nb;
    uint32_t B;
    uint32_t per_window;
    uint32_t l0;
    uint32_t nlev;
};
template <class C, bool QUAD>
__global__ void __launch_bounds__(512)
k_tree_tail(TreeTailArgs<typename C::Fp> a) {
    using M = typename C::Fp;
    const uint32_t w = blockIdx.x;
    for (uint32_t l = a.l0; l < a.nlev; l++) {
        const uint32_t nw = a.B >> (l + 1);
        TreeLevelArgs<M> lv;
        lv.s_prev = l ? a.s_lev[l - 1] : a.buckets;
        lv.s_prev2 = l >= 2 ? a.s_lev[l - 2] : a.buckets;
        lv.n = a.nb >> (l + 1);
        const bool first = (l == a.l0);
        lv.m_prev = first ? a.m_global : a.m_tail[(l + 1) & 1] + (size_t)w * a.per_window;
        lv.m_prev_stride = first ? 2 * lv.n : 2 * nw;
        lv.s_out = a.s_lev[l];
        lv.m_out = a.m_tail[l & 1] + (size_t)w * a.per_window;
        lv.m_out_stride = nw;
        lv.fin = a.fin;
        lv.l = l;
        lv.nlev = a.nlev;
        lv.last = (l + 1 == a.nlev) ? 1u : 0u;
        const uint32_t tasks = (l + 1 + lv.last) * nw;
        if constexpr (QUAD) {
            const uint32_t per_pass = blockDim.x >> 2;
            for (uint32_t t0 = 0; t0 < tasks; t0 += per_pass) {
                uint32_t t = t0 + (threadIdx.x >> 2);
                const bool live = t < tasks;
                if (!live) t = tasks - 1;
                const uint32_t j = t % nw, i = w * nw + j;
                tree_task_quad<C>(lv, t / nw, i, first ? i : j, j, live, threadIdx.x & 63u);
            }
        } else {
            for (uint32_t t = threadIdx.x; t < tasks; t += blockDim.x) {
                const uint32_t j = t % nw, i = w * nw + j;
                tree_task<C>(lv, t / nw, i, first ? i : j, j);
            }
        }
        __threadfence();
        __syncthreads();
    }
}

template <class C>
__global__ void __launch_bounds__(64)
k_bucket_combine(const uint32_t* __restrict__ heavy_list, const uint32_t* __restrict__ chunk_base,
                 const uint32_t* __restrict__ counts, const uint32_t* __restrict__ ctrl,
                 const XYZZ<typename C::Fp>* __restrict__ chunk_out, XYZZ<typename C::Fp>* __restrict__ buckets,
                 uint32_t accumulate) {
    using M = typename C::Fp;
    using N = Node<C>;
    __shared__ XYZZ<M> stage[64];
    const uint32_t n_heavy = ctrl[2];
    for (uint32_t h = blockIdx.x; h < n_heavy; h += gridDim.x) {
        const uint32_t b = heavy_list[h];
        const uint32_t items = (counts[b] + CHUNK - 1) / CHUNK;
        const XYZZ<M>* src = chunk_out + chunk_base[b];
        typename N::T acc = N::inf();
        if (accumulate && threadIdx.x == 0) acc = N::load(buckets + b);
        for (uint32_t k = threadIdx.x; k < items; k += 64) {
            typename N::T p = N::load(src + k);
            N::add(acc, p);
        }
        for (uint32_t m = 32; m >= 1; m >>= 1) {
            N::store(&stage[threadIdx.x], acc);
            __syncthreads();
            if (threadIdx.x < m) {
                typename N::T o = N::load(&stage[threadIdx.x + m]);
                N::add(acc, o);
            }
            __syncthreads();
        }
        if (threadIdx.x == 0) N::store(buckets + b, acc);
    }
}

}
```

### porla_amd/csrc/msm_impl.hip.h

```cpp
#pragma once
#include "engine.hpp"
#include "host_fold64.hpp"
#include "msm_small.hip.h"
#include "msm_tree.hip.h"
#include <cstdlib>
#include <chrono>
#include <thread>
#include <vector>
#include <cstdio>
#include "../../include/porla_gpu.h"

namespace porla {

static inline int ilog2(size_t n) { int l = 0; while (n >>= 1) l++; return l; }

constexpr double TREE_US_PER_ADD = 1.5e-4;
constexpr double TREE_LEVEL_US = 12.5;
constexpr double TREE_QUAD_LEVEL_US = 7.0;
constexpr double TREE_TAIL_LEVEL_US = 6.5;
static inline int choose_window(size_t m, int bits) {
    if (g_window_override >= 2 && g_window_override <= 20) return g_window_override;
    int best = 2;
    double best_cost = 1e300;
    for (int c = 2; c <= 20; c++) {
        const int W = (bits + 1 + c - 1) / c;
        const int top = bits + 1 - c * (W - 1);
        const double B = (double)((size_t)1 << (c - 1));
        const double load = (double)m / B;
        const double top_load = W > 1 ? (double)m / (double)((size_t)1 << (top > 1 ? top - 1 : 0)) : 0.0;
        const double items = (double)W * B * (load > 20.0 ? 1.0 : 1.0 - __builtin_exp(-load));
        const double waves = items / 64.0;
        const double rounds = waves / 4096.0;
        const double adds = (double)W * (double)m > items ? (double)W * (double)m - items : 0.0;
        double t_sum = rounds >= 1.0 ? adds / 14.0e3 * (1.0 + 0.22 / rounds)
                                     : (waves > 0.5 ? load * (4.0 + 15.4 * rounds) : 0.0);
        double chain = load + 4.0 * __builtin_sqrt(load) + 1.0;
        const double top_chain = top_load < (double)CHUNK ? top_load : (double)CHUNK;
        if (top_chain > chain) chain = top_chain;
        if (chain > (double)CHUNK) chain = (double)CHUNK;
        if (t_sum < chain * 5.6) t_sum = chain * 5.6;
        double t_combine = 0.0;
        if (top_load > (double)CHUNK) t_combine = 50.0 + top_load / CHUNK / 64.0 * 7.0;
        if (load > 0.6 * CHUNK) t_combine += 1e6;
        double t_reduce = 0.3 * W * c;
        {
            const uint32_t Bu = 1u << (c - 1), nlev = (uint32_t)(c - 1);
            const uint32_t l0 = tree_tail_start(Bu, nlev, true);
            for (uint32_t l = 0; l < nlev; l++) {
                const double tasks = (double)W * (l + 1) * (double)(Bu >> (l + 1));
                if (l >= l0) t_reduce += TREE_TAIL_LEVEL_US;
                else if (tasks <= (double)TREE_QUAD_MAX_TASKS) t_reduce += TREE_QUAD_LEVEL_US;
                else { const double t = tasks * TREE_US_PER_ADD; t_reduce += t > TREE_LEVEL_US ? t : TREE_LEVEL_US; }
            }
        }
        const double t_sort = (double)W * (double)m * 6.6e-6 * (c <= 16 ? 1.0 : (c == 17 ? 1.1 : 4.5));
        const double cost = 6.0 * W + t_sum + t_sort + t_combine + t_reduce;
        if (cost < best_cost) { best_cost = cost; best = c; }
    }
    return best;
}

constexpr uint32_t SMALL_PAIR_STRIDE = 64 * 1024;
template <class C>
static int msm_small_pair_launch(Workspace* ws, const uint8_t* d_scalars, const uint8_t* d_points_a, const uint8_t* d_points_b, size_t n,
                                 hipStream_t stream, int bits_hint = 0) {
    using M = typename C::Fp;
    int rc;
    const uint32_t sets = d_points_b ? 2u : 1u;
    if (ws->h_windows_cap < sets * SMALL_PAIR_STRIDE) {
        if (ws->h_windows) PORLA_HIP(hipHostFree(ws->h_windows));
        ws->h_windows_cap = sets * SMALL_PAIR_STRIDE;
        PORLA_HIP(hipHostMalloc(&ws->h_windows, ws->h_windows_cap, hipHostMallocMapped | hipHostMallocCoherent));
    }
    const size_t part_bytes = (size_t)SMALL_BLOCKS * SMALL_MAX_C * sizeof(XYZZ<M>);
    if (ws->small_part.cap < part_bytes + 2048) {
        if ((rc = ws->small_part.ensure(part_bytes + 2048))) return rc;
        PORLA_HIP(hipMemsetAsync(ws->small_part.p, 0, part_bytes + 2048, stream));
    }
    void* h_dev = nullptr;
    PORLA_HIP(hipHostGetDevicePointer(&h_dev, ws->h_windows, 0));
    uint32_t* counters = (uint32_t*)((uint8_t*)ws->small_part.p + part_bytes);
    ws->small_seq++;
    if (ws->small_seq == 0) ws->small_seq = 1;
    for (uint32_t set = 0; set < sets; set++) ((volatile uint32_t*)((uint8_t*)ws->h_windows + set * SMALL_PAIR_STRIDE))[0] = 0;
    {
        ProfScope ps("small_msm", stream, true);
        const unsigned blocks = d_points_b ? (n <= 8192 ? 96u : (unsigned)SMALL_BLOCKS / 2) : small_lone_blocks(n);
        hipLaunchKernelGGL((k_small_msm<C>), dim3(blocks, sets), dim3(SMALL_THREADS), 0, stream, d_scalars, d_points_a, (uint32_t)n,
                           g_small_c | (g_use_glv == 0 ? 0x100 : 0) | (bits_hint << 16), (XYZZ<M>*)ws->small_part.p, counters,
                           (uint32_t*)h_dev, (XYZZ<M>*)((uint8_t*)h_dev + SMALL_HDR_WORDS * 4), ws->small_seq, d_points_b, SMALL_PAIR_STRIDE);
    }
    PORLA_HIP(hipGetLastError());
    if (!ws->done) PORLA_HIP(hipEventCreateWithFlags(&ws->done, hipEventDisableTiming));
    PORLA_HIP(hipEventRecord(ws->done, stream));
    return PORLA_OK;
}
template <class C>
static int msm_small_launch(Workspace* ws, const uint8_t* d_scalars, const uint8_t* d_points_be, size_t n, hipStream_t stream) {
    const int rc = msm_small_pair_launch<C>(ws, d_scalars, d_points_be, nullptr, n, stream);
    if (rc) return rc;
    ws->pend_W = -1;
    ws->pend_c = 0;
    return PORLA_OK;
}
template <class C>
static int msm_small_pair_finish(Workspace* ws, int which, XYZZ<typename C::Fp>* total) {
    using M = typename C::Fp;
    const uint8_t* region = (const uint8_t*)ws->h_windows + (size_t)which * SMALL_PAIR_STRIDE;
    const volatile uint32_t* hdr = (const volatile uint32_t*)region;
    const auto t_spin = std::chrono::steady_clock::now();
    bool seen = false;
    for (uint32_t it = 0;; it++) {
        if (__atomic_load_n((const uint32_t*)&hdr[0], __ATOMIC_ACQUIRE) == ws->small_seq) { seen = true; break; }
        __builtin_ia32_pause();
        if ((it & 1023u) == 1023u && std::chrono::steady_clock::now() - t_spin > std::chrono::milliseconds(2)) break;
    }
    if (!seen) PORLA_HIP(hipEventSynchronize(ws->done));
    const int W = (int)hdr[1], c = (int)hdr[2];
    if (hdr[0] != ws->small_seq || W < 1 || c < 1 || c > SMALL_MAX_C || (size_t)W * c * sizeof(XYZZ<M>) + SMALL_HDR_WORDS * 4 > SMALL_PAIR_STRIDE) {
        set_last_error("porla: the single-launch MSM pair left no valid result header");
        return PORLA_ERR_HIP;
    }
    g_last_shape[0] = c; g_last_shape[1] = W; g_last_shape[2] = (int)hdr[3];
    *total = h_fold_tree64<M>((const XYZZ<M>*)(region + SMALL_HDR_WORDS * 4), W, c);
    return PORLA_OK;
}

struct MsmShape {
    bool glv;
    int bits, c, W;
};
template <class C>
static inline bool msm_use_glv(size_t n) {
    if (g_use_glv >= 0) return g_use_glv != 0;
    return C::GLV_DEFAULT || n <= C::GLV_BELOW;
}
template <class C>
static inline MsmShape msm_full_shape(size_t n_range) {
    MsmShape sh;
    sh.glv = msm_use_glv<C>(n_range);
    sh.bits = sh.glv ? C::Glv::BITS : C::SCALAR_BITS;
    sh.c = choose_window(sh.glv ? 2 * n_range : n_range, sh.bits);
    sh.W = (sh.bits + 1 + sh.c - 1) / sh.c;
    return sh;
}
template <class C>
static int msm_tree_launch(Workspace* ws, const XYZZ<typename C::Fp>* buckets, int c, int W, bool glv, hipStream_t stream);

template <class C>
static int msm_launch(Workspace* ws, const uint8_t* d_scalars, const uint8_t* d_points_be, size_t n, hipStream_t stream,
                      const MsmShape* forced = nullptr, XYZZ<typename C::Fp>* bucket_out = nullptr, bool accumulate = false,
                      hipEvent_t after = nullptr) {
    using M = typename C::Fp;
    ws->pend_W = 0;
    if (n == 0) return PORLA_OK;
    if (n >= (1ull << 30)) { set_last_error("porla: MSM length must be < 2^30 per call (range-split larger inputs)"); return PORLA_ERR_ARG; }
    if (!forced && n <= SMALL_MAX_N && g_small_mode != 0 && g_window_override == 0) return msm_small_launch<C>(ws, d_scalars, d_points_be, n, stream);
    if (!forced && n > MSM_RANGE_MAX && C::F30_LAZY && g_window_override == 0) {
        const size_t R = (n + MSM_RANGE_MAX - 1) / MSM_RANGE_MAX;
        const MsmShape shape = msm_full_shape<C>((n + R - 1) / R);
        int rc2;
        if ((rc2 = ws->multi_acc.ensure(((size_t)shape.W << (shape.c - 1)) * sizeof(XYZZ<M>)))) return rc2;
        XYZZ<M>* acc = (XYZZ<M>*)ws->multi_acc.p;
        for (size_t r = 0; r < R; r++) {
            const size_t lo = (size_t)((unsigned __int128)r * n / R), hi = (size_t)((unsigned __int128)(r + 1) * n / R);
            if ((rc2 = msm_launch<C>(ws, d_scalars + 32 * lo, d_points_be + 64 * lo, hi - lo, stream, &shape, acc, r > 0, nullptr))) return rc2;
        }
        return msm_tree_launch<C>(ws, acc, shape.c, shape.W, shape.glv, stream);
    }
    bool glv = forced ? forced->glv : msm_use_glv<C>(n);
    int bits = glv ? C::Glv::BITS : C::SCALAR_BITS;
    if (!forced && n <= MSM_SCAN_MAX) {
        if (ws->h_windows_cap < 64 * 1024) {
            if (ws->h_windows) PORLA_HIP(hipHostFree(ws->h_windows));
            ws->h_windows_cap = 64 * 1024;
            PORLA_HIP(hipHostMalloc(&ws->h_windows, ws->h_windows_cap, hipHostMallocMapped | hipHostMallocCoherent));
        }
        int rc0;
        if ((rc0 = ws->cursor.ensure((CTRL_WORDS + 8) * 4))) return rc0;
        uint32_t* d_or = (uint32_t*)ws->cursor.p + CTRL_WORDS;
        PORLA_HIP(hipMemsetAsync(d_or, 0, 32, stream));
        unsigned blocks = (unsigned)((n + 255) / 256);
        if (blocks > 512) blocks = 512;
        hipLaunchKernelGGL(k_scalar_or, dim3(blocks), dim3(256), 0, stream, d_scalars, (uint32_t)n, d_or);
        PORLA_HIP(hipMemcpyAsync(ws->h_windows, d_or, 32, hipMemcpyDeviceToHost, stream));
        PORLA_HIP(hipStreamSynchronize(stream));
        const uint32_t* h_or = (const uint32_t*)ws->h_windows;
        int top = 7;
        while (top > 0 && h_or[top] == 0) top--;
        int used = h_or[top] ? 32 * top + (32 - __builtin_clz(h_or[top])) : 1;
        if (glv && g_use_glv < 0 && used <= C::Glv::BITS) { glv = false; bits = C::SCALAR_BITS; }
        if (used < 250 && used < bits) bits = used;
    }
    const size_t n_sub = glv ? 2 * n : n;
    const int c = forced ? forced->c : choose_window(n_sub, bits);
    const int W = (bits + 1 + c - 1) / c;
    const SortFrontPlan sf = sort_front_plan(n, glv, c, W);
    const uint32_t tile_cap = sf.tile_cap, T_tiles = sf.T_tiles;
    const int lowbits = sf.lowbits;
    const uint32_t B = 1u << (c - 1);
    const size_t nb = (size_t)W * B;
    const uint32_t n32 = (uint32_t)n;

    int rc;
    if ((rc = ws->pts.ensure(n_sub * sizeof(Affine<M>)))) return rc;
    const uint32_t nblk = (uint32_t)((nb + 1023) / 1024);
    const size_t max_entries = (size_t)W * n_sub;
    if (max_entries >= (1ull << 32)) { set_last_error("porla: MSM too large for one launch (windows x sub-scalars >= 2^32): range-split it (porla_*_msm_host_multi)"); return PORLA_ERR_ARG; }
    const size_t max_items = nb + max_entries / CHUNK;
    const size_t max_chunk_out = 2 * (max_entries / CHUNK) + 2;
    if ((rc = ws->keys.ensure((size_t)W * T_tiles * tile_cap * 4))) return rc;
    if ((rc = ws->tile_off.ensure((size_t)W * T_tiles * (MAX_PARTS + 1) * 2))) return rc;
    if ((rc = ws->entries.ensure(max_entries * 4))) return rc;
    if ((rc = ws->counts.ensure(nb * 4))) return rc;
    if ((rc = ws->starts.ensure(nb * 4))) return rc;
    if ((rc = ws->fill.ensure(nb * 4))) return rc;
    if ((rc = ws->cursor.ensure((CTRL_WORDS + 8) * 4))) return rc;
    if ((rc = ws->order.ensure(max_items * sizeof(uint2)))) return rc;
    if ((rc = ws->heavy.ensure((max_entries / CHUNK + 2) * 4))) return rc;
    if ((rc = ws->chunk_out.ensure(max_chunk_out * sizeof(XYZZ<M>)))) return rc;
    if ((rc = ws->blk_hist.ensure((size_t)CHUNK * nblk * 4))) return rc;
    if ((rc = ws->blk_off.ensure((size_t)CHUNK * nblk * 4))) return rc;
    XYZZ<M>* bk = bucket_out;
    if (!bk) {
        if ((rc = ws->buckets.ensure(nb * sizeof(XYZZ<M>)))) return rc;
        bk = (XYZZ<M>*)ws->buckets.p;
    }
    uint32_t* ctrl = (uint32_t*)ws->cursor.p;
    const Affine<M>* pts = (const Affine<M>*)ws->pts.p;
    const bool front_split = ws->lone && !forced && n >= ((size_t)1 << 18);
    hipStream_t pst = stream;
    if (front_split) {
        if (!ws->aux_stream) PORLA_HIP(hipStreamCreateWithFlags(&ws->aux_stream, hipStreamNonBlocking));
        if (!ws->front_fork_ev) PORLA_HIP(hipEventCreateWithFlags(&ws->front_fork_ev, hipEventDisableTiming));
        if (!ws->front_join_ev) PORLA_HIP(hipEventCreateWithFlags(&ws->front_join_ev, hipEventDisableTiming));
        PORLA_HIP(hipEventRecord(ws->front_fork_ev, stream));
        PORLA_HIP(hipStreamWaitEvent(ws->aux_stream, ws->front_fork_ev, 0));
        pst = ws->aux_stream;
    }
    {
        ProfScope ps("points_to_mont", pst);
        if (glv)
            hipLaunchKernelGGL((k_points_to_mont<C, true, C::F30_BUCKETS>), dim3((n32 + 255) / 256), dim3(256), 0, pst, d_points_be,
                               (Affine<M>*)ws->pts.p, n32);
        else
            hipLaunchKernelGGL((k_points_to_mont<C, false, C::F30_BUCKETS>), dim3((n32 + 255) / 256), dim3(256), 0, pst, d_points_be,
                               (Affine<M>*)ws->pts.p, n32);
    }
    if (front_split) PORLA_HIP(hipEventRecord(ws->front_join_ev, ws->aux_stream));
    {
        ProfScope ps("digits_partition", stream);
        if (glv)
            hipLaunchKernelGGL((k_digits_partition<C, true>), dim3(T_tiles, sf.wg), dim3(TILE_THREADS), 0, stream, d_scalars, n32, c, W,
                               lowbits, (uint32_t*)ws->keys.p, (uint16_t*)ws->tile_off.p, ctrl);
        else
            hipLaunchKernelGGL((k_digits_partition<C, false>), dim3(T_tiles, sf.wg), dim3(TILE_THREADS), 0, stream, d_scalars, n32, c, W,
                               lowbits, (uint32_t*)ws->keys.p, (uint16_t*)ws->tile_off.p, ctrl);
    }
    {
        ProfScope ps("partition_sort", stream);
        sort_launch(sf, c, W, stream, (const uint32_t*)ws->keys.p, (const uint16_t*)ws->tile_off.p, (uint32_t*)ws->counts.p,
                    (uint32_t*)ws->starts.p, (uint32_t*)ws->entries.p, ctrl);
    }
    {
        ProfScope ps("size_order", stream);
        hipLaunchKernelGGL(k_size_hist, dim3(nblk), dim3(1024), 0, stream, (const uint32_t*)ws->counts.p, (uint32_t)nb,
                           (uint32_t*)ws->blk_hist.p, nblk, ctrl);
        hipLaunchKernelGGL(k_size_scan, dim3(CHUNK), dim3(1024), 0, stream, (const uint32_t*)ws->blk_hist.p,
                           (uint32_t*)ws->blk_off.p, nblk, ctrl);
        hipLaunchKernelGGL(k_size_order, dim3(nblk), dim3(1024), 0, stream, (const uint32_t*)ws->counts.p, (uint32_t)nb,
                           (const uint32_t*)ws->blk_off.p, nblk, (uint2*)ws->order.p, (uint32_t*)ws->fill.p,
                           (uint32_t*)ws->heavy.p, ctrl, accumulate ? (uint4*)nullptr : (uint4*)bk);
    }
    if (accumulate) {
        if (!C::F30_LAZY) { set_last_error("porla: merged pair ranges need the reduced-radix bucket form"); return PORLA_ERR_STATE; }
        if (after) PORLA_HIP(hipStreamWaitEvent(stream, after, 0));
    }
    if (front_split) PORLA_HIP(hipStreamWaitEvent(stream, ws->front_join_ev, 0));
    {
        ProfScope ps("bucket_sum", stream, true);
        hipLaunchKernelGGL((k_bucket_sum30<C>), dim3((unsigned)((max_items + 255) / 256)), dim3(256), 0, stream, pts,
                           (const uint32_t*)ws->entries.p, (const uint32_t*)ws->starts.p,
                           (const uint32_t*)ws->counts.p, (const uint2*)ws->order.p, (const uint32_t*)ws->fill.p,
                           (const uint32_t*)ctrl, bk, (XYZZ<M>*)ws->chunk_out.p, accumulate ? 1u : 0u);
    }
    {
        ProfScope ps("bucket_combine", stream);
        hipLaunchKernelGGL((k_bucket_combine<C>), dim3(2048), dim3(64), 0, stream, (const uint32_t*)ws->heavy.p,
                           (const uint32_t*)ws->fill.p, (const uint32_t*)ws->counts.p, (const uint32_t*)ctrl,
                           (const XYZZ<M>*)ws->chunk_out.p, bk, accumulate ? 1u : 0u);
    }
    PORLA_HIP(hipGetLastError());
    if (forced) return PORLA_OK;
    return msm_tree_launch<C>(ws, bk, c, W, glv, stream);
}

template <class C>
static int msm_tree_launch(Workspace* ws, const XYZZ<typename C::Fp>* buckets, int c, int W, bool glv, hipStream_t stream) {
    using M = typename C::Fp;
    int rc;
    static thread_local TreePlan plan;
    static thread_local int plan_c = 0, plan_W = 0, plan_lone = -1;
    if (plan_c != c || plan_W != W || plan_lone != (ws->lone ? 1 : 0)) {
        plan_c = 0;
        const std::string refused = tree_plan(plan, c, W, ws->lone, C::F30_LAZY);
        if (!refused.empty()) { set_last_error("porla: reduction tree: " + refused); return PORLA_ERR_STATE; }
        plan_c = c; plan_W = W; plan_lone = ws->lone ? 1 : 0;
    }
    if ((rc = ws->tree_s.ensure(plan.s_entries * sizeof(XYZZ<M>)))) return rc;
    if ((rc = ws->tree_m.ensure(plan.m_entries * sizeof(XYZZ<M>)))) return rc;
    if ((rc = ws->tree_mt.ensure(plan.mt_entries * sizeof(XYZZ<M>)))) return rc;
    if (ws->h_windows_cap < (size_t)W * c * sizeof(XYZZ<M>) || ws->h_windows_cap < 64 * 1024) {
        if (ws->h_windows) PORLA_HIP(hipHostFree(ws->h_windows));
        ws->h_windows_cap = 64 * 1024;
        PORLA_HIP(hipHostMalloc(&ws->h_windows, ws->h_windows_cap, hipHostMallocMapped | hipHostMallocCoherent));
    }
    void* h_windows_dev = nullptr;
    PORLA_HIP(hipHostGetDevicePointer(&h_windows_dev, ws->h_windows, 0));
    const int parts = (int)plan.parts;
    if (parts == 2) {
        if (!ws->aux_stream) PORLA_HIP(hipStreamCreateWithFlags(&ws->aux_stream, hipStreamNonBlocking));
        if (!ws->fork_ev) PORLA_HIP(hipEventCreateWithFlags(&ws->fork_ev, hipEventDisableTiming));
        if (!ws->join_ev) PORLA_HIP(hipEventCreateWithFlags(&ws->join_ev, hipEventDisableTiming));
        PORLA_HIP(hipEventRecord(ws->fork_ev, stream));
        PORLA_HIP(hipStreamWaitEvent(ws->aux_stream, ws->fork_ev, 0));
    }
    PORLA_HIP((tree_enqueue<C, ProfScope>(plan, buckets, (XYZZ<M>*)ws->tree_s.p, (XYZZ<M>*)ws->tree_m.p, (XYZZ<M>*)ws->tree_mt.p,
                                          (XYZZ<M>*)h_windows_dev, stream, ws->aux_stream)));
    if (parts == 2) {
        PORLA_HIP(hipEventRecord(ws->join_ev, ws->aux_stream));
        PORLA_HIP(hipStreamWaitEvent(stream, ws->join_ev, 0));
    }
    if (!ws->done) PORLA_HIP(hipEventCreateWithFlags(&ws->done, hipEventDisableTiming));
    PORLA_HIP(hipEventRecord(ws->done, stream));
    ws->pend_W = W;
    ws->pend_c = c;
    g_last_shape[0] = c; g_last_shape[1] = W; g_last_shape[2] = glv ? 1 : 0;
    return PORLA_OK;
}

template <class C>
static int msm_finish(Workspace* ws, XYZZ<typename C::Fp>* total) {
    using M = typename C::Fp;
    if (ws->pend_W == 0) { *total = xyzz_inf<M>(); return PORLA_OK; }
    if (ws->pend_W < 0) {
        const volatile uint32_t* hdr = (const volatile uint32_t*)ws->h_windows;
        const auto t_spin = std::chrono::steady_clock::now();
        bool seen = false;
        for (uint32_t it = 0;; it++) {
            if (__atomic_load_n((const uint32_t*)&hdr[0], __ATOMIC_ACQUIRE) == ws->small_seq) { seen = true; break; }
            __builtin_ia32_pause();
            if ((it & 1023u) == 1023u && std::chrono::steady_clock::now() - t_spin > std::chrono::milliseconds(2)) break;
        }
        if (!seen) PORLA_HIP(hipEventSynchronize(ws->done));
        const int W = (int)hdr[1], c = (int)hdr[2];
        ws->pend_W = 0;
        if (hdr[0] != ws->small_seq || W < 1 || c < 1 || c > SMALL_MAX_C || (size_t)W * c * sizeof(XYZZ<M>) + SMALL_HDR_WORDS * 4 > ws->h_windows_cap) {
            set_last_error("porla: the single-launch MSM left no valid result header");
            return PORLA_ERR_HIP;
        }
        g_last_shape[0] = c; g_last_shape[1] = W; g_last_shape[2] = (int)hdr[3];
        *total = h_fold_tree64<M>((const XYZZ<M>*)((const uint8_t*)ws->h_windows + SMALL_HDR_WORDS * 4), W, c);
        return PORLA_OK;
    }
    PORLA_HIP(hipEventSynchronize(ws->done));
    *total = h_fold_tree64<M>((const XYZZ<M>*)ws->h_windows, ws->pend_W, ws->pend_c);
    ws->pend_W = 0;
    return PORLA_OK;
}

template <class C>
static int msm_core(Workspace* ws, const uint8_t* d_scalars, const uint8_t* d_points_be, size_t n, hipStream_t stream,
                    XYZZ<typename C::Fp>* total) {
    int rc = msm_launch<C>(ws, d_scalars, d_points_be, n, stream);
    if (rc) return rc;
    return msm_finish<C>(ws, total);
}

template <class C>
int msm_device(const uint8_t* d_scalars, const uint8_t* d_points, size_t n, hipStream_t stream,
               XYZZ<typename C::Fp>* total) {
    int rc = ensure_device();
    if (rc) return rc;
    Workspace* ws;
    if ((rc = lease_blocking_slot(&ws))) return rc;
    std::lock_guard<std::mutex> lk(ws->mu, std::adopt_lock);
    ws->lone = true;
    return msm_core<C>(ws, d_scalars, d_points, n, stream, total);
}
template <class C>
static int msm_pair_locked(Workspace* ws, const uint8_t* d_scalars, const uint8_t* d_points_a, const uint8_t* d_points_b, size_t n,
                           hipStream_t stream, XYZZ<typename C::Fp>* total_a, XYZZ<typename C::Fp>* total_b, int bits_hint = 0) {
    int rc;
    ws->lone = true;
    if (n <= SMALL_MAX_N && g_small_mode != 0 && g_window_override == 0) {
        ws->pend_W = 0;
        if ((rc = msm_small_pair_launch<C>(ws, d_scalars, d_points_a, d_points_b, n, stream, bits_hint))) return rc;
        if ((rc = msm_small_pair_finish<C>(ws, 0, total_a))) return rc;
        return msm_small_pair_finish<C>(ws, 1, total_b);
    }
    if ((rc = msm_core<C>(ws, d_scalars, d_points_a, n, stream, total_a))) return rc;
    return msm_core<C>(ws, d_scalars, d_points_b, n, stream, total_b);
}
template <class C>
int msm_pair_device(const uint8_t* d_scalars, const uint8_t* d_points_a, const uint8_t* d_points_b, size_t n, hipStream_t stream,
                    XYZZ<typename C::Fp>* total_a, XYZZ<typename C::Fp>* total_b) {
    int rc = ensure_device();
    if (rc) return rc;
    if (n == 0) { *total_a = xyzz_inf<typename C::Fp>(); *total_b = *total_a; return PORLA_OK; }
    Workspace* ws;
    if ((rc = lease_blocking_slot(&ws))) return rc;
    std::lock_guard<std::mutex> lk(ws->mu, std::adopt_lock);
    return msm_pair_locked<C>(ws, d_scalars, d_points_a, d_points_b, n, stream, total_a, total_b);
}
template <class C>
int msm_device_begin(int slot, const uint8_t* d_scalars, const uint8_t* d_points, size_t n, hipStream_t stream) {
    int rc = ensure_device();
    if (rc) return rc;
    Workspace* ws;
    if ((rc = get_workspace_slot(slot, &ws))) return rc;
    std::lock_guard<std::mutex> lk(ws->mu);
    if (ws->begun) { set_last_error("porla: MSM slot still has a pending result (call the matching _end first)"); return PORLA_ERR_STATE; }
    ws->lone = false;
    rc = msm_launch<C>(ws, d_scalars, d_points, n, stream);
    if (rc == PORLA_OK) ws->begun = true;
    return rc;
}
template <class C>
int msm_device_end(int slot, XYZZ<typename C::Fp>* total) {
    Workspace* ws;
    int rc = get_workspace_slot(slot, &ws);
    if (rc) return rc;
    std::lock_guard<std::mutex> lk(ws->mu);
    if (!ws->begun || ws->pair_pending) {
        set_last_error("porla: no MSM was begun on this slot of the current device (end must run with the device of its begin; a pair "
                       "is collected with *_audit_msm_pair_end)");
        return PORLA_ERR_STATE;
    }
    ws->begun = false;
    return msm_finish<C>(ws, total);
}

template <class C>
static int msm_host_launch(Workspace* ws, const uint8_t* scalars, const uint8_t* points, size_t n) {
    int rc;
    ws->pend_W = 0;
    if (n == 0) return PORLA_OK;
    if ((rc = ws->in_scalars.ensure(n * 32))) return rc;
    if ((rc = ws->in_points.ensure(n * 64))) return rc;
    hipStream_t s = ws->own_stream;
    PORLA_HIP(hipMemcpyAsync(ws->in_scalars.p, scalars, n * 32, hipMemcpyHostToDevice, s));
    PORLA_HIP(hipMemcpyAsync(ws->in_points.p, points, n * 64, hipMemcpyHostToDevice, s));
    return msm_launch<C>(ws, (const uint8_t*)ws->in_scalars.p, (const uint8_t*)ws->in_points.p, n, s);
}

static inline size_t msm_multi_min_range() {
    static const size_t v = (size_t)1 << 17;
    return v < 1 ? 1 : v;
}
static inline int msm_multi_pipeline() {
    static const int v = 4;
    return v < 1 ? 1 : (v > 64 ? 64 : v);
}
extern std::mutex g_multi_mu;
static inline bool msm_multi_shared_buckets() {
    static const bool v = !(getenv("PORLA_MSM_SHARED_BUCKETS") && getenv("PORLA_MSM_SHARED_BUCKETS")[0] == '0');
    return v;
}
template <class C>
int msm_host_multi(const uint8_t* scalars, const uint8_t* points, size_t n, int shards, int devices,
                   XYZZ<typename C::Fp>* total) {
    using M = typename C::Fp;
    int rc = ensure_device();
    if (rc) return rc;
    *total = xyzz_inf<M>();
    if (n == 0) return PORLA_OK;
    int visible = 0, first = 0;
    PORLA_HIP(hipGetDeviceCount(&visible));
    PORLA_HIP(hipGetDevice(&first));
    int G = devices;
    if (G <= 0 && getenv("PORLA_MSM_DEVICES")) G = atoi(getenv("PORLA_MSM_DEVICES"));
    if (G <= 0) {
        size_t by_size = n / msm_multi_min_range();
        G = by_size < 1 ? 1 : (by_size > (size_t)visible ? visible : (int)by_size);
    }
    if (G > visible) G = visible;
    if (G < 1) G = 1;
    int S = shards;
    if (S <= 0) {
        size_t per_dev = n / G / msm_multi_min_range();
        size_t pipe = (size_t)msm_multi_pipeline();
        S = G * (int)(per_dev < 1 ? 1 : (per_dev > pipe ? pipe : per_dev));
    }
    if ((size_t)S > n) S = (int)n;
    if (S < G) G = S;
    std::vector<XYZZ<M>> part((size_t)G, xyzz_inf<M>());
    std::vector<int> dev_rc((size_t)G, PORLA_OK);
    std::vector<std::string> dev_err((size_t)G);
    std::lock_guard<std::mutex> lk_multi(g_multi_mu);
    auto worker = [&](int g) {
        int r = PORLA_OK;
        auto fail = [&](int code) { if (!r) { r = code; dev_err[g] = porla_gpu_last_error(); } };
        const int dev = (first + g) % visible;
        if (hipSetDevice(dev) != hipSuccess) { set_last_error("porla: hipSetDevice failed"); fail(PORLA_ERR_HIP); dev_rc[g] = r; return; }
        const int s0 = (int)((long long)g * S / G), s1 = (int)((long long)(g + 1) * S / G), R = s1 - s0;
        std::vector<size_t> bound((size_t)R + 1);
        size_t max_cnt = 0;
        for (int j = 0; j <= R; j++) {
            bound[(size_t)j] = (size_t)((unsigned __int128)(s0 + j) * n / (unsigned)S);
            if (j && bound[(size_t)j] - bound[(size_t)j - 1] > max_cnt) max_cnt = bound[(size_t)j] - bound[(size_t)j - 1];
        }
        constexpr int PIPE = MSM_MULTI_SLOTS;
        Workspace* slot_ws[PIPE] = {nullptr, nullptr, nullptr, nullptr};
        const int used_slots = R < PIPE ? R : PIPE;
        Workspace* found[PIPE] = {nullptr, nullptr, nullptr, nullptr};
        for (int k = 0; k < used_slots && !r; k++) {
            int rr = get_workspace_slot(MSM_MULTI_SLOT0 + k, &found[k]);
            if (rr) { found[k] = nullptr; fail(rr); }
        }
        for (int k = 0; k < used_slots && !r; k++) {
// ... 222 lines not shown
```

### porla_amd/csrc/msm_small.hip.h

```cpp
#pragma once
#include "msm.hip.h"

namespace porla {

constexpr uint32_t SMALL_MAX_N = 32768;
constexpr int SMALL_THREADS = 256;
constexpr int SMALL_BLOCKS = 256;
constexpr int SMALL_MAX_C = 8;
constexpr int SMALL_MAX_B = 1 << (SMALL_MAX_C - 1);
#if defined(__HIP_DEVICE_COMPILE__) && !defined(__gfx950__)
#error "msm_small.hip.h sizes its per-block state (about 105 KB of static LDS) for gfx950's 160 KB of LDS per CU; there is no smaller-LDS variant"
#endif
constexpr uint32_t SMALL_MAX_SUB = 8192;
constexpr int SMALL_MAX_S = 32;
constexpr int SMALL_DONE_SLOT = 255;
constexpr uint32_t SMALL_HDR_WORDS = 32;

inline uint32_t small_lone_blocks(uint64_t n) { return n <= 4096 ? 192u : (uint32_t)SMALL_BLOCKS; }

constexpr int FB_SMALL_MAX_ROWS = 64;
constexpr int FB_SMALL_MAX_SLICES = 8;

struct SmallCfg {
    int glv;
// ... 216 lines not shown
        __syncthreads();
    }
    if (tid < B) cursor[tid] -= hist[tid];
    __syncthreads();
    const uint32_t T = SMALL_THREADS / B;
    const uint32_t my_b = tid / T, my_t = tid % T;
    const uint32_t my_start = cursor[my_b], my_cnt = hist[my_b];
    __syncthreads();
    for (uint32_t j = tid; j < (i1 - i0) * SUBS; j += SMALL_THREADS) {
        const uint32_t p = raw[j];
        if (p != 0xffffffffu) {
            const uint32_t pos = atomicAdd(&cursor[p >> 14], 1u);
            ent[pos] = (i0 * SUBS + (p & 0x1fffu)) | (((p >> 13) & 1u) << 31);
        }
    }
    __syncthreads();

    SMALL_STAMP(3);
    {
        XYZZ30<M> acc;
        acc.inf = true;
        bool flip = false;
        uint32_t en = 0;
        Affine<M> nx;
        if (my_t < my_cnt) {
            en = ent[my_start + my_t];
            const uint32_t i = g.glv ? (en & 0x7fffffffu) >> 1 : (en & 0x7fffffffu);
            load_be256(nx.x.v, points + (size_t)i * 64);
            load_be256(nx.y.v, points + (size_t)i * 64 + 32);
        }
        for (uint32_t e = my_t; e < my_cnt; e += T) {
            const uint32_t cur = en;
            Affine<M> a = nx;
            if (e + T < my_cnt) {
                en = ent[my_start + e + T];
                const uint32_t i = g.glv ? (en & 0x7fffffffu) >> 1 : (en & 0x7fffffffu);
                load_be256(nx.x.v, points + (size_t)i * 64);
                load_be256(nx.y.v, points + (size_t)i * 64 + 32);
            }
            fe_reduce_plain<M>(a.x.v, 6);
            fe_reduce_plain<M>(a.y.v, 6);
            if (aff_is_inf<M>(a)) continue;
            a = aff_neg_if<M>(a, xyzz30_flip_neg<M>((cur >> 31) != 0, flip));
            F30<M> ax = f30_from_fe<M>(a.x), ay = f30_from_fe<M>(a.y);
            if constexpr (!M::PSEUDO_MERSENNE) {
                ax = f30_mul<M>(ax, f30_const<M>(M::RR_30));
                ay = f30_mul<M>(ay, f30_const<M>(M::RR_30));
            }
            if (g.glv && (cur & 1u)) ax = f30_mul<M>(ax, f30_const<M>(C::Glv::BETA_30));
            xyzz30_madd_flip<M>(acc, flip, ax, ay);
        }
        xyzz30_flip_finish<M>(acc, flip);
        xyzz30_store_lazy<M>(&pts[tid], acc);
    }
    __syncthreads();

    SMALL_STAMP(4);
    for (uint32_t h = 1; h < T; h <<= 1) {
        const bool last = (h << 1) == T;
        small_quad_adds<M>(SMALL_THREADS / (2 * h), [&](uint32_t t, const XYZZ<M>*& pa, const XYZZ<M>*& pb, XYZZ<M>*& out) {
            pa = &pts[t * 2 * h]; pb = pa + h;
            out = last ? &bk[t] : &pts[t * 2 * h];
        });
        __syncthreads();
    }
    SMALL_STAMP(5);
    const uint32_t nlev = (uint32_t)(cw - 1);
    auto s_level = [&](uint32_t l) { return slev + (B - (B >> l)); };
    auto m_half = [&](uint32_t h) { return mlev + (h & 1u) * (SMALL_MAX_B / 4 + 1); };
    for (uint32_t l = 0; l < nlev; l++) {
        const uint32_t nl = B >> (l + 1);
        const XYZZ<M>* sp = l ? s_level(l - 1) : bk;
        const XYZZ<M>* sp2 = l >= 2 ? s_level(l - 2) : bk;
        const XYZZ<M>* mp = m_half(l + 1);
        XYZZ<M>* so = s_level(l);
        XYZZ<M>* mo = m_half(l);
        small_quad_adds<M>((l + 1) * nl, [&](uint32_t t, const XYZZ<M>*& pa, const XYZZ<M>*& pb, XYZZ<M>*& out) {
            const uint32_t sl = t / nl, i = t % nl;
            if (sl == l) { pa = sp + 2 * i; pb = pa + 1; out = so + i; }
            else if (sl + 1 == l) { pa = sp2 + 4 * i + 1; pb = pa + 2; out = mo + sl * nl + i; }
            else { pa = mp + sl * 2 * nl + 2 * i; pb = pa + 1; out = mo + sl * nl + i; }
        });
        __syncthreads();
    }
    SMALL_STAMP(6);
    XYZZ<M>* mine = part + (size_t)bx * SMALL_MAX_C;
    if (tid < (uint32_t)c * 8) {
        const uint32_t kk = tid >> 3, q = tid & 7;
        const XYZZ<M>* src = nullptr;
        if (kk == 0) src = nlev ? s_level(nlev - 1) : bk;
        else if (kk > nlev) src = nullptr;
        else if (kk == nlev) src = (nlev >= 2 ? s_level(nlev - 2) : bk) + 1;
        else src = m_half(nlev - 1) + (kk - 1);
        reinterpret_cast<uint4*>(mine + kk)[q] = src ? reinterpret_cast<const uint4*>(src)[q] : make_uint4(0, 0, 0, 0);
    }
    SMALL_STAMP(7);
    __threadfence();
    __syncthreads();
    if (tid == 0) {
        const uint32_t old = atomicAdd(&counters[w], 1u);
        last_flag = (old == (uint32_t)g.S - 1) ? 1u : 0u;
        if (last_flag) counters[w] = 0;
    }
    __syncthreads();
    if (!last_flag) return {g, w, nullptr};
    __threadfence();
    SMALL_STAMP(8);
    {
        const uint4* src = reinterpret_cast<const uint4*>(part + (size_t)w * g.S * SMALL_MAX_C);
        uint4* dst = reinterpret_cast<uint4*>(pts);
        const uint32_t total = (uint32_t)g.S * (uint32_t)c * 8;
        for (uint32_t x = tid; x < total; x += SMALL_THREADS) {
            const uint32_t e = x >> 3, q = x & 7;
            dst[x] = src[(size_t)((e / (uint32_t)c) * SMALL_MAX_C + e % (uint32_t)c) * 8 + q];
        }
    }
    __syncthreads();
    for (uint32_t cnt = (uint32_t)g.S; cnt > 1;) {
        const uint32_t half = (cnt + 1) / 2, pairs = cnt - half;
        small_quad_adds<M>(pairs * (uint32_t)c, [&](uint32_t t, const XYZZ<M>*& pa, const XYZZ<M>*& pb, XYZZ<M>*& out) {
            const uint32_t sl = t / (uint32_t)c, kk = t % (uint32_t)c;
            pa = &pts[sl * c + kk]; pb = &pts[(sl + half) * c + kk];
            out = &pts[sl * c + kk];
        });
        __syncthreads();
        cnt = half;
    }
    return {g, w, pts};
}

template <class C>
__global__ void __launch_bounds__(SMALL_THREADS) __attribute__((amdgpu_waves_per_eu(1, 1)))
k_small_msm(const uint8_t* __restrict__ scalars, const uint8_t* __restrict__ points, uint32_t n, int c_override,
            XYZZ<typename C::Fp>* __restrict__ part, uint32_t* __restrict__ counters, uint32_t* __restrict__ hdr,
            XYZZ<typename C::Fp>* __restrict__ fin, uint32_t seq, const uint8_t* __restrict__ points_b,
            uint32_t pair_stride_bytes SMALL_STAMP_ARG) {
    using M = typename C::Fp;
    if (blockIdx.y) {
        points = points_b;
        part += (size_t)gridDim.x * SMALL_MAX_C;
        counters += 256;
        hdr = reinterpret_cast<uint32_t*>(reinterpret_cast<uint8_t*>(hdr) + pair_stride_bytes);
        fin = reinterpret_cast<XYZZ<M>*>(reinterpret_cast<uint8_t*>(fin) + pair_stride_bytes);
    }
    const SmallWindow<M> win = small_block<C>(scalars, points, n, blockIdx.x, (int)gridDim.x, c_override, (c_override >> 16) & 0x1ff, part,
                                              counters, [](const SmallCfg&) { return true; } SMALL_STAMP_PASS(stamps));
    if (!win.sums) return;
    const uint32_t tid = threadIdx.x;
    const int c = win.g.c;
    if (tid < (uint32_t)c) Node<C>::store_final(fin + (size_t)win.w * c + tid, Node<C>::load(&win.sums[tid]));
    SMALL_STAMP(9);
    __threadfence_system();
    __syncthreads();
    if (tid == 0) {
        const uint32_t old = atomicAdd(&counters[SMALL_DONE_SLOT], 1u);
        if (old == (uint32_t)win.g.W - 1) {
            counters[SMALL_DONE_SLOT] = 0;
            hdr[1] = (uint32_t)win.g.W; hdr[2] = (uint32_t)c; hdr[3] = (uint32_t)win.g.glv;
            __threadfence_system();
            __atomic_store_n(&hdr[0], seq, __ATOMIC_RELEASE);
        }
    }
}

}
```

### porla_amd/csrc/msm_tree.hip.h

```cpp
#pragma once
#include "msm.hip.h"
#include <cstdio>
#include <string>
#include <vector>

namespace porla {

static inline uint32_t tree_tail_threads() { return 512u; }
static inline bool tree_quad() { return true; }
constexpr uint32_t TREE_QUAD_MAX_TASKS = 16384;
constexpr uint32_t TREE_QUAD_MAX_TASKS_LONE = 65536;
static inline uint32_t tree_tail_start(uint32_t B, uint32_t nlev, bool quad) {
    const uint32_t cap = quad ? tree_tail_threads() / 4 : tree_tail_threads();
    uint32_t l = 0;
    while (l + 1 < nlev && (l + 1) * (B >> (l + 1)) > cap) l++;
    return l;
}

struct TreeOptions {
    int parts = -1;
    int front2 = -1;
    long long quad_max_tasks = -1;
    int l0 = -1;
};

enum TreeKind : uint32_t { TREE_FRONT2 = 0, TREE_LEVEL = 1, TREE_LEVEL_QUAD = 2, TREE_TAIL = 3 };
static inline const char* tree_kind_name(uint32_t k) {
    return k == TREE_FRONT2 ? "front2" : k == TREE_LEVEL ? "level" : k == TREE_LEVEL_QUAD ? "level_quad" : "tail";
}

struct TreeLaunch {
    uint32_t kind, part;
    uint32_t l;
    uint32_t n;
    uint32_t grid, block;
    size_t bk;
    bool s_prev_bk, s_prev2_bk;
    size_t s_prev, s_prev2, s_out, s1_out;
    size_t m_prev, m_out;
    uint32_t m_prev_stride, m_out_stride;
    size_t s_lev[24];
    size_t m_global;
    size_t m_tail[2];
    size_t fin;
    uint32_t per_window, nb, B, nlev;
};

struct TreePlan {
    uint32_t c, W, lone, parts, nlev, B;
    size_t s_entries, m_entries, mt_entries, fin_entries;
    struct Part { uint32_t w0, Wp, l0, front2; unsigned long long quad_max; } part[2];
    std::vector<TreeLaunch> launches;
};

static inline std::string tree_plan(TreePlan& p, int c, int W, bool lone, bool lazy, const TreeOptions& o = TreeOptions()) {
    if (c < 2 || c > 24 || W < 1 || ((size_t)W << (c - 1)) > ((size_t)1 << 31)) return "shape out of range";
    const uint32_t B = 1u << (c - 1);
    const size_t nb = (size_t)W * B;
    const uint32_t nlev = (uint32_t)(c - 1);
    const bool quad = lazy && tree_quad();
    if (!quad) return "the tail runs four lanes per addition: curves with the reduced-radix memory form only";
    p.c = (uint32_t)c; p.W = (uint32_t)W; p.lone = lone ? 1u : 0u; p.nlev = nlev; p.B = B;
    p.s_entries = nb + 2;
    p.m_entries = 2 * (nb / 4) + 6;
    p.mt_entries = 2 * (size_t)W * (B / 4 + 1) + 4;
    p.fin_entries = (size_t)W * c;
    const int parts = o.parts >= 0 ? o.parts : ((lone && W >= 4 && nb >= ((size_t)1 << 18)) ? 2 : 1);
    if (parts != 1 && parts != 2) return "parts must be 1 or 2";
    if (parts == 2 && W < 2) return "two parts need at least two windows";
    const uint32_t l0 = o.l0 >= 0 ? (uint32_t)o.l0 : tree_tail_start(B, nlev, quad);
    if (l0 >= nlev) return "the tail must start below the last level (l0 < nlev)";
    const unsigned long long quad_max = o.quad_max_tasks >= 0 ? (unsigned long long)o.quad_max_tasks
                                                               : (lone ? TREE_QUAD_MAX_TASKS_LONE : TREE_QUAD_MAX_TASKS);
    p.parts = (uint32_t)parts;
    p.launches.clear();
    p.launches.reserve(2 * (size_t)c);
    size_t s_off = 0, m_off = 0, mt_off = 0;
    for (int part = 0, w0 = 0; part < parts; part++) {
        const int Wp = parts == 1 ? W : (part == 0 ? W / 2 : W - W / 2);
        const size_t nbp = (size_t)Wp * B;
        const size_t m_half[2] = {m_off, m_off + nbp / 4 + 1};
        auto s_level = [&](uint32_t l) { return s_off + (nbp - (nbp >> l)); };
        const bool front2 = o.front2 >= 0 ? o.front2 != 0
                                          : (!lone && l0 >= 2 && (nbp & 3) == 0 && nbp / 2 > (size_t)TREE_QUAD_MAX_TASKS);
        if (front2 && (l0 < 2 || (nbp & 3) != 0)) return "front2 needs l0 >= 2 and a bucket count per part divisible by 4";
        p.part[part] = {(uint32_t)w0, (uint32_t)Wp, l0, front2 ? 1u : 0u, quad_max};
        TreeLaunch z{};
        z.part = (uint32_t)part; z.bk = (size_t)w0 * B; z.nlev = nlev; z.B = B; z.nb = (uint32_t)nbp;
        uint32_t l_first = 0;
        if (front2) {
            TreeLaunch a = z;
            a.kind = TREE_FRONT2; a.l = 1;
            a.s_prev_bk = a.s_prev2_bk = true; a.s_prev = a.s_prev2 = 0; a.m_prev = m_half[0];
            a.s_out = s_level(0); a.s1_out = s_level(1);
            a.m_out = m_half[1];
            a.n = (uint32_t)(nbp >> 2);
            a.m_prev_stride = 0; a.m_out_stride = a.n;
            a.grid = (a.n + 255) / 256; a.block = 256;
            p.launches.push_back(a);
            l_first = 2;
        }
        for (uint32_t l = l_first; l < l0; l++) {
            TreeLaunch a = z;
            a.l = l;
            a.s_prev_bk = l == 0; a.s_prev = l ? s_level(l - 1) : 0;
            a.s_prev2_bk = l < 2; a.s_prev2 = l >= 2 ? s_level(l - 2) : 0;
            a.m_prev = m_half[(l + 1) & 1];
            a.s_out = s_level(l);
            a.m_out = m_half[l & 1];
            a.n = (uint32_t)(nbp >> (l + 1));
            a.m_prev_stride = 2 * a.n; a.m_out_stride = a.n;
            const size_t tasks = (size_t)(l + 1) * a.n;
            a.block = 256;
            if (tasks <= quad_max) { a.kind = TREE_LEVEL_QUAD; a.grid = (unsigned)((4 * tasks + 255) / 256); }
            else { a.kind = TREE_LEVEL; a.grid = (unsigned)((tasks + 255) / 256); }
            p.launches.push_back(a);
        }
        {
            TreeLaunch t = z;
            t.kind = TREE_TAIL; t.l = l0; t.n = (uint32_t)Wp;
            for (uint32_t l = 0; l < 24; l++) t.s_lev[l] = l < nlev ? s_level(l) : 0;
            t.m_global = m_half[(l0 + 1) & 1];
            t.per_window = B / 4 + 1;
            t.m_tail[0] = mt_off; t.m_tail[1] = mt_off + (size_t)Wp * t.per_window + 1;
            t.fin = (size_t)w0 * c;
            uint32_t need = (l0 + 2) * (B >> (l0 + 1)) * 4u;
            uint32_t threads = (need + 63) / 64 * 64;
            if (threads > tree_tail_threads()) threads = tree_tail_threads();
            if (threads < 64) threads = 64;
            t.grid = (uint32_t)Wp; t.block = threads;
            p.launches.push_back(t);
        }
        s_off += nbp + 1; m_off += 2 * (nbp / 4) + 2; mt_off += 2 * (size_t)Wp * (B / 4 + 1) + 2;
        w0 += Wp;
    }
    return "";
}

struct TreeNoScope { TreeNoScope(const char*, hipStream_t) {} };

template <class C, class Scope = TreeNoScope>
static hipError_t tree_enqueue(const TreePlan& p, const XYZZ<typename C::Fp>* buckets, XYZZ<typename C::Fp>* s_area,
                               XYZZ<typename C::Fp>* m_area, XYZZ<typename C::Fp>* mt_area, XYZZ<typename C::Fp>* fin,
                               hipStream_t st0, hipStream_t st1) {
    using M = typename C::Fp;
    static_assert(C::F30_LAZY, "the tree's quad forms read the reduced-radix memory form");
    size_t at = 0;
    for (uint32_t part = 0; part < p.parts; part++) {
        hipStream_t st = part == 0 ? st0 : st1;
        {
            Scope ps("tree_levels", st);
            for (; at < p.launches.size() && p.launches[at].part == part && p.launches[at].kind != TREE_TAIL; at++) {
                const TreeLaunch& q = p.launches[at];
                TreeLevelArgs<M> a;
                a.s_prev = q.s_prev_bk ? buckets + q.bk : s_area + q.s_prev;
                a.s_prev2 = q.s_prev2_bk ? buckets + q.bk : s_area + q.s_prev2;
                a.m_prev = m_area + q.m_prev;
                a.s_out = s_area + q.s_out;
                a.m_out = m_area + q.m_out;
                a.fin = nullptr;
                a.n = q.n;
                a.m_prev_stride = q.m_prev_stride; a.m_out_stride = q.m_out_stride;
                a.l = q.l; a.nlev = q.nlev; a.last = 0;
                if (q.kind == TREE_FRONT2) hipLaunchKernelGGL((k_tree_front2<C>), dim3(q.grid), dim3(q.block), 0, st, a, s_area + q.s1_out);
                else if (q.kind == TREE_LEVEL_QUAD) hipLaunchKernelGGL((k_tree_level_quad<C>), dim3(q.grid), dim3(q.block), 0, st, a);
                else hipLaunchKernelGGL((k_tree_level<C>), dim3(q.grid), dim3(q.block), 0, st, a);
            }
        }
        if (at < p.launches.size() && p.launches[at].part == part) {
            const TreeLaunch& q = p.launches[at++];
            Scope ps("tree_tail", st);
            TreeTailArgs<M> t;
            t.buckets = buckets + q.bk;
            for (uint32_t l = 0; l < 24; l++) t.s_lev[l] = l < q.nlev ? s_area + q.s_lev[l] : nullptr;
            t.m_global = m_area + q.m_global;
            t.per_window = q.per_window;
            t.m_tail[0] = mt_area + q.m_tail[0]; t.m_tail[1] = mt_area + q.m_tail[1];
            t.fin = fin + q.fin;
            t.nb = q.nb; t.B = q.B; t.l0 = q.l; t.nlev = q.nlev;
            hipLaunchKernelGGL((k_tree_tail<C, true>), dim3(q.grid), dim3(q.block), 0, st, t);
        }
        const hipError_t e = hipGetLastError();
        if (e != hipSuccess) return e;
    }
    return hipSuccess;
}

static inline std::string tree_plan_text(const TreePlan& p) {
    char b[1024];
    std::string out;
    snprintf(b, sizeof b, "plan c=%u W=%u lone=%u parts=%u nlev=%u B=%u s_entries=%zu m_entries=%zu mt_entries=%zu fin_entries=%zu tail_threads=%u\n",
             p.c, p.W, p.lone, p.parts, p.nlev, p.B, p.s_entries, p.m_entries, p.mt_entries, p.fin_entries, tree_tail_threads());
    out += b;
    for (uint32_t i = 0; i < p.parts; i++) {
        snprintf(b, sizeof b, "part part=%u w0=%u Wp=%u l0=%u front2=%u quad_max=%llu\n", i, p.part[i].w0, p.part[i].Wp, p.part[i].l0,
                 p.part[i].front2, p.part[i].quad_max);
        out += b;
    }
    for (const TreeLaunch& q : p.launches) {
        if (q.kind != TREE_TAIL) {
            snprintf(b, sizeof b, "launch part=%u kind=%s l=%u n=%u grid=%u block=%u bk=%zu s_prev_bk=%d s_prev=%zu s_prev2_bk=%d s_prev2=%zu "
                     "s_out=%zu s1_out=%zu m_prev=%zu m_out=%zu m_prev_stride=%u m_out_stride=%u nb=%u nlev=%u\n",
                     q.part, tree_kind_name(q.kind), q.l, q.n, q.grid, q.block, q.bk, (int)q.s_prev_bk, q.s_prev, (int)q.s_prev2_bk, q.s_prev2,
                     q.s_out, q.s1_out, q.m_prev, q.m_out, q.m_prev_stride, q.m_out_stride, q.nb, q.nlev);
            out += b;
            continue;
        }
        snprintf(b, sizeof b, "launch part=%u kind=tail l=%u n=%u grid=%u block=%u bk=%zu m_global=%zu m_tail0=%zu m_tail1=%zu per_window=%u "
                 "fin=%zu nb=%u B=%u nlev=%u s_lev=", q.part, q.l, q.n, q.grid, q.block, q.bk, q.m_global, q.m_tail[0], q.m_tail[1],
                 q.per_window, q.fin, q.nb, q.B, q.nlev);
        out += b;
        for (uint32_t l = 0; l < q.nlev; l++) { snprintf(b, sizeof b, "%s%zu", l ? "," : "", q.s_lev[l]); out += b; }
        out += "\n";
    }
    return out;
}

}
```

### porla_amd/loader.py

```python
import ctypes
import os
import sys

_HERE = os.path.dirname(os.path.abspath(__file__))
lib_path = os.path.join(_HERE, "libmultiexp.so")
_lib = None


class GoSlice(ctypes.Structure):
    _fields_ = [("data", ctypes.c_void_p), ("len", ctypes.c_longlong), ("cap", ctypes.c_longlong)]


class KzgAuditReq(ctypes.Structure):
    _fields_ = [("d_rows64", ctypes.c_void_p), ("d_idx64", ctypes.c_void_p), ("d_coef64", ctypes.c_void_p), ("n64", ctypes.c_size_t),
                ("d_rows32", ctypes.c_void_p), ("d_idx32", ctypes.c_void_p), ("d_coef32", ctypes.c_void_p), ("n32", ctypes.c_size_t),
                ("d_mac_store", ctypes.c_void_p), ("d_align_store", ctypes.c_void_p), ("d_mac_idx", ctypes.c_void_p),
                ("d_mac_coef", ctypes.c_void_p), ("n_macs", ctypes.c_size_t), ("random_point", ctypes.c_ulonglong)]


class IpaAuditReq(ctypes.Structure):
    _fields_ = KzgAuditReq._fields_[:13] + [("a_value", ctypes.c_uint8 * 32)]


class KzgVerifyReq(ctypes.Structure):
# ... 65 lines not shown
assert ctypes.sizeof(IccDecodeRaggedReq) == PORLA_ICC_DECODE_RAGGED_REQ_BYTES


class IccMacDecodeReq(ctypes.Structure):
    _fields_ = [("d_macs", ctypes.c_void_p), ("d_out", ctypes.c_void_p), ("d_write_steps", ctypes.c_void_p), ("d_sub", ctypes.c_void_p)]


PORLA_ICC_MAC_DECODE_REQ_BYTES = 32
assert ctypes.sizeof(IccMacDecodeReq) == PORLA_ICC_MAC_DECODE_REQ_BYTES


class RetrieveReq(ctypes.Structure):
    _fields_ = [("d_rows", ctypes.c_void_p), ("d_macs", ctypes.c_void_p), ("d_prf", ctypes.c_void_p), ("d_out", ctypes.c_void_p),
                ("d_status", ctypes.c_void_p), ("d_counts", ctypes.c_void_p)]


PORLA_RETRIEVE_REQ_BYTES = 48
PORLA_RETRIEVE_ROW_OK = 1
assert ctypes.sizeof(RetrieveReq) == PORLA_RETRIEVE_REQ_BYTES


class RetrieveAlignedReq(ctypes.Structure):
    _fields_ = [("d_rows", ctypes.c_void_p), ("d_macs", ctypes.c_void_p), ("d_prf", ctypes.c_void_p), ("d_align", ctypes.c_void_p),
                ("d_write_steps", ctypes.c_void_p), ("d_out", ctypes.c_void_p), ("d_status", ctypes.c_void_p), ("d_counts", ctypes.c_void_p)]


PORLA_RETRIEVE_ALIGNED_REQ_BYTES = 64
assert ctypes.sizeof(RetrieveAlignedReq) == PORLA_RETRIEVE_ALIGNED_REQ_BYTES


class ExtractReq(ctypes.Structure):
    _fields_ = [("write_step", ctypes.c_ulonglong), ("data_x", ctypes.c_void_p), ("mac_x", ctypes.c_void_p), ("d_top_rows", ctypes.c_void_p),
                ("d_top_macs", ctypes.c_void_p), ("d_top_align", ctypes.c_void_p), ("d_prf", ctypes.c_void_p), ("d_work", ctypes.c_void_p),
                ("d_blocks", ctypes.c_void_p), ("d_steps", ctypes.c_void_p), ("d_flags", ctypes.c_void_p), ("d_row_status", ctypes.c_void_p),
                ("d_counts", ctypes.c_void_p)]


PORLA_EXTRACT_REQ_BYTES = 104
PORLA_EXTRACT_FOUND, PORLA_EXTRACT_UNSURE, PORLA_EXTRACT_RESIDUE = 1, 2, 4
assert ctypes.sizeof(ExtractReq) == PORLA_EXTRACT_REQ_BYTES


class ExtractXyReq(ctypes.Structure):
    _fields_ = ExtractReq._fields_ + [("data_y", ctypes.c_void_p), ("mac_y", ctypes.c_void_p), ("align_y", ctypes.c_void_p),
                                      ("d_prf_y", ctypes.c_void_p), ("d_work_y", ctypes.c_void_p), ("d_row_status_y", ctypes.c_void_p),
                                      ("y_levels", ctypes.c_ulonglong)]


PORLA_EXTRACT_XY_REQ_BYTES = 160
PORLA_EXTRACT_FROM_Y = 8
PORLA_EXTRACT_ROW_NOT_TRIED = 2
assert ctypes.sizeof(ExtractXyReq) == PORLA_EXTRACT_XY_REQ_BYTES


class ExtractXytReq(ctypes.Structure):
    _fields_ = ExtractXyReq._fields_ + [("d_top_rows_y", ctypes.c_void_p), ("d_top_macs_y", ctypes.c_void_p), ("d_top_align_y", ctypes.c_void_p),
                                        ("d_prf_top_y", ctypes.c_void_p), ("d_top_patch", ctypes.c_void_p),
                                        ("d_row_status_top_y", ctypes.c_void_p), ("top_step", ctypes.c_ulonglong), ("top_y", ctypes.c_ulonglong)]


PORLA_EXTRACT_XYT_REQ_BYTES = 224
assert ctypes.sizeof(ExtractXytReq) == PORLA_EXTRACT_XYT_REQ_BYTES


class PrfRun(ctypes.Structure):
    _fields_ = [("level", ctypes.c_int), ("index0", ctypes.c_int), ("count", ctypes.c_ulonglong), ("time0", ctypes.c_longlong),
                ("time_stride", ctypes.c_longlong)]


PORLA_PRF_RUN_BYTES = 32
assert ctypes.sizeof(PrfRun) == PORLA_PRF_RUN_BYTES


class AuditLevel(ctypes.Structure):
    _fields_ = [("data_x", ctypes.c_ulonglong), ("data_y", ctypes.c_ulonglong), ("mac_x", ctypes.c_ulonglong), ("mac_y", ctypes.c_ulonglong),
                ("form", ctypes.c_int), ("pad", ctypes.c_int)]


PORLA_AUDIT_LEVEL_BYTES = 40
assert ctypes.sizeof(AuditLevel) == PORLA_AUDIT_LEVEL_BYTES


class AuditChallengeReq(ctypes.Structure):
    _fields_ = [("seed", ctypes.c_uint8 * 16), ("write_step", ctypes.c_ulonglong), ("num_blocks", ctypes.c_ulonglong),
                ("levels", ctypes.POINTER(AuditLevel)), ("d_idx64", ctypes.c_void_p), ("d_coef64", ctypes.c_void_p),
                ("d_idx32", ctypes.c_void_p), ("d_coef32", ctypes.c_void_p), ("d_mac_idx", ctypes.c_void_p), ("d_mac_coef", ctypes.c_void_p)]


PORLA_AUDIT_CHALLENGE_REQ_BYTES = 88
assert ctypes.sizeof(AuditChallengeReq) == PORLA_AUDIT_CHALLENGE_REQ_BYTES


class AuditChallengeInfo(ctypes.Structure):
    _fields_ = [("n64", ctypes.c_ulonglong), ("n32", ctypes.c_ulonglong), ("n_macs", ctypes.c_ulonglong), ("random_point", ctypes.c_ulonglong),
                ("a_raw", ctypes.c_int), ("pad", ctypes.c_int), ("a_value", ctypes.c_uint8 * 32)]


PORLA_AUDIT_CHALLENGE_INFO_BYTES = 72
assert ctypes.sizeof(AuditChallengeInfo) == PORLA_AUDIT_CHALLENGE_INFO_BYTES


class AuditScalarReq(ctypes.Structure):
    _fields_ = [("seed", ctypes.c_uint8 * 16), ("write_step", ctypes.c_ulonglong), ("num_blocks", ctypes.c_ulonglong)]


PORLA_AUDIT_SCALAR_REQ_BYTES = 32
assert ctypes.sizeof(AuditScalarReq) == PORLA_AUDIT_SCALAR_REQ_BYTES


def load():
    global _lib
    if _lib is not None:
        return _lib
    if not os.path.exists(lib_path):
        raise ImportError(
            "porla_amd: %s is missing -- build it with `python -c 'import __graft_entry__ as g; g.build()'` "
            "or `make -C porla_amd/csrc` (hipcc, gfx950). There is no CPU fallback." % lib_path)
    if os.environ.get("PORLA_NO_TORCH", "0") != "1":
        try:
            import torch
        except Exception:
            pass
    _lib = ctypes.CDLL(lib_path, mode=ctypes.RTLD_GLOBAL)
    _declare(_lib)
    return _lib


def _declare(L):
    P = ctypes.POINTER(GoSlice)
    vp, sz, u8p = ctypes.c_void_p, ctypes.c_size_t, ctypes.c_char_p
    L.init_key.argtypes = [P, P]; L.init_key.restype = None
    L.init_SRS.argtypes = [ctypes.c_longlong, P, ctypes.POINTER(ctypes.c_longlong)]; L.init_SRS.restype = None
    L.init_SRS_from_data.argtypes = [ctypes.c_longlong, P]; L.init_SRS_from_data.restype = None
    for name in ("compute_digest", "compute_digest_complement", "compute_digest_from_srs", "add_point", "mult_point"):
        getattr(L, name).argtypes = [P, P]; getattr(L, name).restype = None
    L.compute_multi_exp.argtypes = [P, P, ctypes.c_longlong, P]; L.compute_multi_exp.restype = None
    L.compare_commitment.argtypes = [P, P]; L.compare_commitment.restype = ctypes.c_ubyte
    L.create_proof.argtypes = [ctypes.c_ulonglong, P, P, P, P, P]; L.create_proof.restype = None
    L.verify_proof.argtypes = [P, P, P, P]; L.verify_proof.restype = ctypes.c_ubyte
    L.neg_point.argtypes = [P]; L.neg_point.restype = None
    L.set_inf_point.argtypes = [P]; L.set_inf_point.restype = None

    L.porla_gpu_device_count.argtypes = []; L.porla_gpu_device_count.restype = ctypes.c_int
    L.porla_gpu_set_device.argtypes = [ctypes.c_int]; L.porla_gpu_set_device.restype = ctypes.c_int
    L.porla_gpu_last_error.argtypes = []; L.porla_gpu_last_error.restype = ctypes.c_char_p
    L.porla_gpu_profile_enable.argtypes = [ctypes.c_int]; L.porla_gpu_profile_enable.restype = ctypes.c_int
    L.porla_gpu_profile_get.argtypes = [ctypes.c_int, ctypes.c_char_p, sz, ctypes.POINTER(ctypes.c_double),
                                        ctypes.POINTER(ctypes.c_longlong)]
    L.porla_gpu_profile_get.restype = ctypes.c_int
    L.porla_gpu_set_msm_window.argtypes = [ctypes.c_int]; L.porla_gpu_set_msm_window.restype = ctypes.c_int
    L.porla_gpu_set_msm_glv.argtypes = [ctypes.c_int]; L.porla_gpu_set_msm_glv.restype = ctypes.c_int
    L.porla_gpu_set_msm_small.argtypes = [ctypes.c_int, ctypes.c_int]; L.porla_gpu_set_msm_small.restype = ctypes.c_int
    L.porla_gpu_last_msm_shape.argtypes = [ctypes.POINTER(ctypes.c_int)] * 3; L.porla_gpu_last_msm_shape.restype = ctypes.c_int
    L.porla_glv_split.argtypes = [ctypes.c_int, u8p, u8p, ctypes.POINTER(ctypes.c_int), u8p, ctypes.POINTER(ctypes.c_int)]
    L.porla_glv_split.restype = ctypes.c_int
    L.porla_diag_fe_op.argtypes = [ctypes.c_int, ctypes.c_int, u8p, u8p, u8p]; L.porla_diag_fe_op.restype = ctypes.c_int
    for curve in ("bn254", "secp256k1"):
        f = getattr(L, "porla_%s_msm_device_begin" % curve); f.argtypes = [ctypes.c_int, vp, vp, sz, vp]; f.restype = ctypes.c_int
        f = getattr(L, "porla_%s_msm_device_end" % curve); f.argtypes = [ctypes.c_int, u8p, ctypes.c_int]; f.restype = ctypes.c_int
    for curve in ("bn254", "secp256k1"):
        f = getattr(L, "porla_%s_msm_device" % curve); f.argtypes = [vp, vp, sz, u8p, vp]; f.restype = ctypes.c_int
        f = getattr(L, "porla_%s_msm_device_partial" % curve); f.argtypes = [vp, vp, sz, u8p, vp]; f.restype = ctypes.c_int
        f = getattr(L, "porla_%s_msm_host" % curve); f.argtypes = [u8p, u8p, sz, u8p]; f.restype = ctypes.c_int
        f = getattr(L, "porla_%s_msm_pair_device" % curve); f.argtypes = [vp, vp, vp, sz, u8p, u8p, vp]; f.restype = ctypes.c_int
        f = getattr(L, "porla_%s_audit_msm_pair_device" % curve); f.argtypes = [vp, vp, vp, vp, sz, u8p, u8p, vp]; f.restype = ctypes.c_int
        f = getattr(L, "porla_%s_audit_msm_pair_begin" % curve); f.argtypes = [ctypes.c_int, vp, vp, vp, vp, sz, vp]; f.restype = ctypes.c_int
        f = getattr(L, "porla_%s_audit_msm_pair_end" % curve); f.argtypes = [ctypes.c_int, u8p, u8p]; f.restype = ctypes.c_int
        f = getattr(L, "porla_%s_msm_pair_host" % curve); f.argtypes = [u8p, u8p, u8p, sz, u8p, u8p]; f.restype = ctypes.c_int
        u64p = ctypes.POINTER(ctypes.c_uint64)
        f = getattr(L, "porla_%s_msm_batch_device" % curve); f.argtypes = [vp, vp, u64p, sz, vp, vp]; f.restype = ctypes.c_int
        f = getattr(L, "porla_%s_msm_batch_host" % curve); f.argtypes = [u8p, u8p, u64p, sz, u8p]; f.restype = ctypes.c_int
        f = getattr(L, "porla_%s_msm_host_multi" % curve); f.argtypes = [u8p, u8p, sz, ctypes.c_int, ctypes.c_int, u8p]; f.restype = ctypes.c_int
        f = getattr(L, "porla_%s_dist_fold" % curve); f.argtypes = [u8p, u8p]; f.restype = ctypes.c_int
        f = getattr(L, "porla_%s_msm_device_dist" % curve); f.argtypes = [vp, vp, sz, u8p, vp]; f.restype = ctypes.c_int
        f = getattr(L, "porla_%s_jac_sum" % curve); f.argtypes = [u8p, sz, u8p]; f.restype = ctypes.c_int
        f = getattr(L, "porla_%s_tree_fold" % curve); f.argtypes = [u8p, ctypes.c_int, ctypes.c_int, u8p]; f.restype = ctypes.c_int
    L.porla_icc_hadd_host.argtypes = [u8p, sz, sz, ctypes.c_ulonglong, ctypes.c_int, u8p, u8p, ctypes.c_int, u8p]; L.porla_icc_hadd_host.restype = ctypes.c_int
    L.porla_icc_mac_scale_host.argtypes = [u8p, sz, ctypes.c_ulonglong, ctypes.c_int, u8p]; L.porla_icc_mac_scale_host.restype = ctypes.c_int
    L.porla_kzg_hadd_host.argtypes = [u8p, u8p, sz, ctypes.c_ulonglong, u8p, u8p, u8p]; L.porla_kzg_hadd_host.restype = ctypes.c_int
    L.porla_icc_hrebuild_host.argtypes = [ctypes.POINTER(vp), ctypes.c_int, sz, sz, ctypes.c_int]; L.porla_icc_hrebuild_host.restype = ctypes.c_int
    L.porla_icc_mac_hrebuild_host.argtypes = [ctypes.POINTER(vp), ctypes.c_int, sz, ctypes.c_int]; L.porla_icc_mac_hrebuild_host.restype = ctypes.c_int
    L.porla_shard_range.argtypes = [sz, ctypes.c_int, ctypes.c_int, ctypes.POINTER(sz), ctypes.POINTER(sz)]; L.porla_shard_range.restype = ctypes.c_int
    L.porla_kzg_commit_batch_host_multi.argtypes = [u8p, sz, u8p, ctypes.c_int]; L.porla_kzg_commit_batch_host_multi.restype = ctypes.c_int
    L.porla_icc_encode_cols_host.argtypes = [u8p, sz, sz, sz, sz, ctypes.c_int, ctypes.c_ulonglong, ctypes.c_int, vp, vp, vp, ctypes.c_int]
    L.porla_icc_encode_cols_host.restype = ctypes.c_int
    L.porla_icc_encode_host_multi.argtypes = [u8p, sz, sz, ctypes.c_int, ctypes.c_ulonglong, ctypes.c_int, vp, vp, vp, ctypes.c_int, ctypes.c_int]
    L.porla_icc_encode_host_multi.restype = ctypes.c_int
    L.porla_gpu_last_msm_multi.argtypes = [ctypes.POINTER(ctypes.c_int)] * 2; L.porla_gpu_last_msm_multi.restype = ctypes.c_int
    L.porla_dist_unique_id.argtypes = [u8p]; L.porla_dist_unique_id.restype = ctypes.c_int
    L.porla_dist_init.argtypes = [u8p, ctypes.c_int, ctypes.c_int]; L.porla_dist_init.restype = ctypes.c_int
    L.porla_dist_info.argtypes = [ctypes.POINTER(ctypes.c_int)] * 2; L.porla_dist_info.restype = ctypes.c_int
    L.porla_dist_finalize.argtypes = []; L.porla_dist_finalize.restype = ctypes.c_int
    L.porla_dist_allgather_partials.argtypes = [u8p, u8p]; L.porla_dist_allgather_partials.restype = ctypes.c_int
    L.porla_fixed_base_create.argtypes = [ctypes.c_int, u8p, sz, ctypes.c_int, ctypes.POINTER(vp)]
    L.porla_fixed_base_create.restype = ctypes.c_int
    L.porla_fixed_base_info.argtypes = [vp, ctypes.POINTER(ctypes.c_int), ctypes.POINTER(ctypes.c_int),
                                        ctypes.POINTER(ctypes.c_ulonglong)]
    L.porla_fixed_base_info.restype = ctypes.c_int
    L.porla_fixed_base_commit_device.argtypes = [vp, vp, sz, sz, sz, vp, vp]; L.porla_fixed_base_commit_device.restype = ctypes.c_int
    L.porla_fixed_base_commit_host.argtypes = [vp, u8p, sz, sz, sz, u8p]; L.porla_fixed_base_commit_host.restype = ctypes.c_int
    L.porla_fixed_base_destroy.argtypes = [vp]; L.porla_fixed_base_destroy.restype = None
    L.porla_kzg_commit_batch_device.argtypes = [vp, sz, vp, vp]; L.porla_kzg_commit_batch_device.restype = ctypes.c_int
    L.porla_kzg_commit_batch_host.argtypes = [u8p, sz, u8p]; L.porla_kzg_commit_batch_host.restype = ctypes.c_int
    L.porla_kzg_commit_batch_device_to_host.argtypes = [vp, sz, u8p, vp]; L.porla_kzg_commit_batch_device_to_host.restype = ctypes.c_int
    L.porla_ipa_audit_device.argtypes = [vp, vp, vp, vp, sz, vp, vp, vp, sz, sz, vp, vp, vp, vp, sz] + [u8p] * 5 + [vp]
    L.porla_ipa_audit_device.restype = ctypes.c_int
    L.porla_kzg_audit_device.argtypes = [vp, vp, vp, sz, vp, vp, vp, sz, vp, vp, vp, vp, sz, ctypes.c_ulonglong] + [u8p] * 8 + [vp]
    L.porla_kzg_audit_device.restype = ctypes.c_int
    L.porla_kzg_audit_batch_device.argtypes = [ctypes.POINTER(KzgAuditReq), sz, vp, vp, vp]
    L.porla_kzg_audit_batch_device.restype = ctypes.c_int
    L.porla_ipa_audit_batch_device.argtypes = [vp, ctypes.POINTER(IpaAuditReq), sz, vp, vp, vp]
    L.porla_ipa_audit_batch_device.restype = ctypes.c_int
    L.porla_kzg_update_batch_device.argtypes = [ctypes.POINTER(UpdateReq), sz, sz, vp]; L.porla_kzg_update_batch_device.restype = ctypes.c_int
    L.porla_ipa_update_batch_device.argtypes = [vp, ctypes.POINTER(UpdateReq), sz, sz, vp]; L.porla_ipa_update_batch_device.restype = ctypes.c_int
    L.porla_kzg_client_update_batch_device.argtypes = [ctypes.POINTER(ClientUpdateReq), sz, sz, vp]
    L.porla_kzg_client_update_batch_device.restype = ctypes.c_int
    L.porla_ipa_client_update_batch_device.argtypes = [vp, vp, ctypes.POINTER(ClientUpdateReq), sz, sz, vp]
    L.porla_ipa_client_update_batch_device.restype = ctypes.c_int
    L.porla_kzg_client_rebuild_batch_device.argtypes = [ctypes.POINTER(ClientRebuildReq), sz, sz, vp]
    L.porla_kzg_client_rebuild_batch_device.restype = ctypes.c_int
    L.porla_ipa_client_rebuild_batch_device.argtypes = [vp, vp, ctypes.POINTER(ClientRebuildReq), sz, sz, vp]
    L.porla_ipa_client_rebuild_batch_device.restype = ctypes.c_int
    L.porla_server_rebuild_batch_device.argtypes = [ctypes.POINTER(ServerRebuildReq), sz, sz, sz, ctypes.c_int, vp]
    L.porla_server_rebuild_batch_device.restype = ctypes.c_int
    L.porla_kzg_server_rebuild_aligned_batch_device.argtypes = [ctypes.POINTER(ServerRebuildReq), sz, sz, vp]
    L.porla_kzg_server_rebuild_aligned_batch_device.restype = ctypes.c_int
    L.porla_ipa_server_rebuild_aligned_batch_device.argtypes = [vp, ctypes.POINTER(ServerRebuildReq), sz, sz, vp]
    L.porla_ipa_server_rebuild_aligned_batch_device.restype = ctypes.c_int
    L.porla_icc_decode_batch_device.argtypes = [ctypes.POINTER(IccDecodeReq), sz, sz, sz, sz, ctypes.c_int, ctypes.c_int, vp]
    L.porla_icc_decode_batch_device.restype = ctypes.c_int
    L.porla_icc_decode_ragged_batch_device.argtypes = [ctypes.POINTER(IccDecodeRaggedReq), sz, sz, sz, ctypes.c_int, ctypes.c_int, vp]
    L.porla_icc_decode_ragged_batch_device.restype = ctypes.c_int
    L.porla_icc_decode_host.argtypes = [u8p, sz, sz, sz, ctypes.c_int, ctypes.c_int, ctypes.POINTER(ctypes.c_ulonglong), vp,
                                        ctypes.POINTER(ctypes.c_uint)]
    L.porla_icc_decode_host.restype = ctypes.c_int
    L.porla_icc_mac_decode_batch_device.argtypes = [ctypes.POINTER(IccMacDecodeReq), sz, sz, sz, ctypes.c_int, vp]
    L.porla_icc_mac_decode_batch_device.restype = ctypes.c_int
    L.porla_icc_mac_decode_host.argtypes = [u8p, sz, sz, ctypes.c_int, ctypes.POINTER(ctypes.c_ulonglong), u8p, vp]
    L.porla_icc_mac_decode_host.restype = ctypes.c_int
    L.porla_kzg_retrieve_batch_device.argtypes = [ctypes.POINTER(RetrieveReq), sz, sz, sz, vp]
    L.porla_kzg_retrieve_batch_device.restype = ctypes.c_int
    L.porla_ipa_retrieve_batch_device.argtypes = [vp, vp, ctypes.POINTER(RetrieveReq), sz, sz, sz, vp]
    L.porla_ipa_retrieve_batch_device.restype = ctypes.c_int
    L.porla_kzg_retrieve_host.argtypes = [u8p, u8p, u8p, sz, sz, vp, vp, ctypes.POINTER(ctypes.c_uint)]
    L.porla_kzg_retrieve_host.restype = ctypes.c_int
    L.porla_ipa_retrieve_host.argtypes = [vp, vp, u8p, u8p, u8p, sz, sz, vp, vp, ctypes.POINTER(ctypes.c_uint)]
    L.porla_ipa_retrieve_host.restype = ctypes.c_int
    L.porla_kzg_retrieve_aligned_batch_device.argtypes = [ctypes.POINTER(RetrieveAlignedReq), sz, sz, sz, ctypes.c_int, vp]
    L.porla_kzg_retrieve_aligned_batch_device.restype = ctypes.c_int
    L.porla_ipa_retrieve_aligned_batch_device.argtypes = [vp, vp, u8p, ctypes.POINTER(RetrieveAlignedReq), sz, sz, sz, ctypes.c_int, vp]
    L.porla_ipa_retrieve_aligned_batch_device.restype = ctypes.c_int
    L.porla_kzg_extract_batch_device.argtypes = [ctypes.POINTER(ExtractReq), sz, sz, ctypes.c_int, vp]
    L.porla_kzg_extract_batch_device.restype = ctypes.c_int
    L.porla_ipa_extract_batch_device.argtypes = [vp, vp, u8p, ctypes.POINTER(ExtractReq), sz, sz, ctypes.c_int, vp]
    L.porla_ipa_extract_batch_device.restype = ctypes.c_int
    L.porla_kzg_extract_xy_batch_device.argtypes = [ctypes.POINTER(ExtractXyReq), sz, sz, ctypes.c_int, vp]
    L.porla_kzg_extract_xy_batch_device.restype = ctypes.c_int
    L.porla_ipa_extract_xy_batch_device.argtypes = [vp, vp, u8p, ctypes.POINTER(ExtractXyReq), sz, sz, ctypes.c_int, vp]
    L.porla_ipa_extract_xy_batch_device.restype = ctypes.c_int
    L.porla_kzg_extract_xyt_batch_device.argtypes = [ctypes.POINTER(ExtractXytReq), sz, sz, ctypes.c_int, vp]
    L.porla_kzg_extract_xyt_batch_device.restype = ctypes.c_int
    L.porla_ipa_extract_xyt_batch_device.argtypes = [vp, vp, u8p, ctypes.POINTER(ExtractXytReq), sz, sz, ctypes.c_int, vp]
    L.porla_ipa_extract_xyt_batch_device.restype = ctypes.c_int
    L.porla_kzg_retrieve_aligned_host.argtypes = [u8p, u8p, u8p, u8p, vp, sz, sz, ctypes.c_int, vp, vp, ctypes.POINTER(ctypes.c_uint)]
    L.porla_kzg_retrieve_aligned_host.restype = ctypes.c_int
    L.porla_ipa_retrieve_aligned_host.argtypes = [vp, vp, u8p, u8p, u8p, u8p, u8p, vp, sz, sz, ctypes.c_int, vp, vp,
                                                  ctypes.POINTER(ctypes.c_uint)]
    L.porla_ipa_retrieve_aligned_host.restype = ctypes.c_int
    L.porla_mac_prf_batch_device.argtypes = [u8p, ctypes.POINTER(PrfRun), sz, vp, vp]; L.porla_mac_prf_batch_device.restype = ctypes.c_int
    L.porla_mac_prf_host.argtypes = [u8p, ctypes.POINTER(PrfRun), sz, vp]; L.porla_mac_prf_host.restype = ctypes.c_int
    L.porla_client_prf_runs.argtypes = [ctypes.c_int, ctypes.c_int, ctypes.c_ulonglong, ctypes.c_int, sz, ctypes.POINTER(PrfRun), sz,
                                        ctypes.POINTER(sz), ctypes.POINTER(sz)]
    L.porla_client_prf_runs.restype = ctypes.c_int
    L.porla_audit_challenge_batch_device.argtypes = [ctypes.POINTER(AuditChallengeReq), sz, ctypes.POINTER(AuditChallengeInfo), vp]
    L.porla_audit_challenge_batch_device.restype = ctypes.c_int
    L.porla_audit_challenge_host.argtypes = [ctypes.POINTER(AuditChallengeReq), sz, ctypes.POINTER(AuditChallengeInfo)]
    L.porla_audit_challenge_host.restype = ctypes.c_int
    L.porla_audit_complement_scalar_batch_device.argtypes = [u8p, ctypes.POINTER(AuditScalarReq), sz, ctypes.c_int, vp, vp]
    L.porla_audit_complement_scalar_batch_device.restype = ctypes.c_int
    L.porla_audit_complement_scalar_host.argtypes = [u8p, ctypes.POINTER(AuditScalarReq), sz, ctypes.c_int, vp]
    L.porla_audit_complement_scalar_host.restype = ctypes.c_int
    L.porla_diag_audit_walk.argtypes = [vp, sz, ctypes.c_ulonglong, ctypes.c_ulonglong, ctypes.POINTER(AuditLevel), ctypes.c_int, vp, vp, vp, vp,
                                        vp, vp, ctypes.POINTER(AuditChallengeInfo)]
    L.porla_diag_audit_walk.restype = ctypes.c_int
    L.porla_ipa_prove_batch_device.argtypes = [vp, vp, vp, sz, vp, vp]; L.porla_ipa_prove_batch_device.restype = ctypes.c_int
    L.porla_ipa_verify_batch_device.argtypes = [vp, ctypes.POINTER(IpaVerifyReq), sz, vp, vp, vp]
    L.porla_ipa_verify_batch_device.restype = ctypes.c_int
    L.porla_kzg_verify_batch_device.argtypes = [ctypes.POINTER(KzgVerifyReq), sz, vp, u8p, u8p, vp]
    L.porla_kzg_verify_batch_device.restype = ctypes.c_int
    L.porla_kzg_digest_batch_device.argtypes = [vp, sz, vp, vp]; L.porla_kzg_digest_batch_device.restype = ctypes.c_int
    L.porla_kzg_complement_batch_device.argtypes = [vp, sz, vp, vp]; L.porla_kzg_complement_batch_device.restype = ctypes.c_int
    L.porla_kzg_mac_batch_device.argtypes = [vp, vp, sz, vp, vp]; L.porla_kzg_mac_batch_device.restype = ctypes.c_int
    L.porla_kzg_digest_batch_host.argtypes = [ctypes.c_char_p, sz, ctypes.c_char_p]; L.porla_kzg_digest_batch_host.restype = ctypes.c_int
    L.porla_kzg_complement_batch_host.argtypes = [ctypes.c_char_p, sz, ctypes.c_char_p]; L.porla_kzg_complement_batch_host.restype = ctypes.c_int
    L.porla_kzg_mac_batch_host.argtypes = [ctypes.c_char_p, ctypes.c_char_p, sz, ctypes.c_char_p]; L.porla_kzg_mac_batch_host.restype = ctypes.c_int
    L.porla_bn254_g2_mul_generator.argtypes = [u8p, u8p]; L.porla_bn254_g2_mul_generator.restype = ctypes.c_int
    L.porla_bn254_pairing_product_is_one.argtypes = [u8p, u8p, u8p, u8p, ctypes.c_int]; L.porla_bn254_pairing_product_is_one.restype = ctypes.c_int
    L.porla_kzg_set_commit_window.argtypes = [ctypes.c_int]; L.porla_kzg_set_commit_window.restype = ctypes.c_int
    L.porla_kzg_commit_shape.argtypes = [ctypes.POINTER(ctypes.c_int)] * 2; L.porla_kzg_commit_shape.restype = ctypes.c_int
    L.porla_kzg_row_coefficients.argtypes = [ctypes.POINTER(ctypes.c_size_t)]; L.porla_kzg_row_coefficients.restype = ctypes.c_int
    L.porla_kzg_release_device_memory.argtypes = []; L.porla_kzg_release_device_memory.restype = ctypes.c_int
    L.porla_gpu_release_msm_workspaces.argtypes = []; L.porla_gpu_release_msm_workspaces.restype = ctypes.c_int
    L.porla_icc_mac_encode_device.argtypes = [vp, sz, ctypes.c_int, ctypes.c_ulonglong, ctypes.c_int, vp, vp]
    L.porla_icc_mac_encode_device.restype = ctypes.c_int
    L.porla_icc_encode_xy_device.argtypes = [vp, sz, sz, ctypes.c_int, ctypes.c_ulonglong, vp, vp, vp, vp, vp, vp, ctypes.c_int, vp]
    L.porla_icc_encode_xy_device.restype = ctypes.c_int
# ... 28 lines not shown
```

### porla_amd/multiexp.py

```python
import ctypes

from .loader import GoSlice, IpaAuditReq, IpaVerifyReq, KzgAuditReq, KzgVerifyReq, lib

MAC_SIZE = 64
SCALAR_SIZE = 32


def _slice(buf):
    return GoSlice(ctypes.cast(buf, ctypes.c_void_p), len(buf), len(buf))


def _buf(data):
    return ctypes.create_string_buffer(bytes(data), len(data))


def _check(rc):
    if rc != 0:
        raise RuntimeError("porla engine error %d: %s" % (rc, lib.porla_gpu_last_error().decode()))


def bn254_add(a, b):
    ba, bb = _buf(a), _buf(b)
    sa, sb = _slice(ba), _slice(bb)
    lib.add_point(ctypes.byref(sa), ctypes.byref(sb))
# ... 625 lines not shown


def split_audit_records(raw, k):
    out = []
    for i in range(k):
        r = raw[KZG_AUDIT_RECORD_BYTES * i:KZG_AUDIT_RECORD_BYTES * (i + 1)]
        out.append(dict(commitment=r[0:64], proof_h=r[64:128], point=r[128:160], claim=r[160:192], combined_mac=r[192:256],
                        combined_align=r[256:320]))
    return out


IPA_AUDIT_RECORD_BYTES = 655
IPA_PROOF_BYTES = 556


def ipa_audit_requests(audits):
    arr = (IpaAuditReq * max(len(audits), 1))()
    for i, a in enumerate(audits):
        if len(a) != 14:
            raise ValueError("ipa_audit_batch_device: audit %d has %d fields, want 14" % (i, len(a)))
        v = a[13].to_bytes(32, "big") if isinstance(a[13], int) else bytes(a[13]).rjust(32, b"\0")
        if len(v) != 32:
            raise ValueError("ipa_audit_batch_device: audit %d: a_value longer than 32 bytes" % i)
        arr[i] = IpaAuditReq(*[(x or None) if j in _REQ_POINTERS else x for j, x in enumerate(a[:13])], (ctypes.c_uint8 * 32)(*v))
    return arr


def split_ipa_records(raw, k):
    out = []
    le = lambda b: int.from_bytes(b, "little")
    for i in range(k):
        r = raw[IPA_AUDIT_RECORD_BYTES * i:IPA_AUDIT_RECORD_BYTES * (i + 1)]
        p = r[99:]
        tail = p[32 + 6 * 66:]
        out.append(dict(commitment=r[0:33], combined_mac=r[33:66], combined_align=r[66:99], proof=p, c=le(p[:32]),
                        rounds=[(p[32 + 66 * j:65 + 66 * j], p[65 + 66 * j:98 + 66 * j]) for j in range(6)],
                        a0=le(tail[0:32]), b0=le(tail[32:64]), a1=le(tail[64:96]), b1=le(tail[96:128])))
    return out


IPA_VERIFY_FULL = 1
IPA_VERIFY_PROOF = 2
IPA_VERIFY_MALFORMED = 4
IPA_VERIFY_BVEC = 8
IPA_VERIFY_PASS = IPA_VERIFY_FULL | IPA_VERIFY_PROOF
IPA_VERIFY_PASS_BOUND = IPA_VERIFY_PASS | IPA_VERIFY_BVEC


def _be32(v, what, i):
    b = v.to_bytes(32, "big") if isinstance(v, int) else bytes(v)
    if len(b) > 32:
        raise ValueError("ipa_verify_batch_device: %s of reply %d is longer than 32 bytes" % (what, i))
    return (ctypes.c_uint8 * 32)(*b.rjust(32, b"\0"))


def ipa_verify_requests(verifs):
    arr = (IpaVerifyReq * max(len(verifs), 1))()
    for i, v in enumerate(verifs):
        if len(v) != 6:
            raise ValueError("ipa_verify_batch_device: reply %d has %d fields, want 6" % (i, len(v)))
        comp, idx, coef, n, alpha, a_value = v
        arr[i] = IpaVerifyReq(comp or None, idx or None, coef or None, n, _be32(alpha, "alpha", i), _be32(a_value, "a_value", i))
    return arr


KZG_VERIFY_FULL = 1
KZG_VERIFY_PROOF = 2
KZG_VERIFY_MALFORMED = 4
KZG_VERIFY_PASS = KZG_VERIFY_FULL | KZG_VERIFY_PROOF
KZG_VERIFY_MAX_K = 10922


def kzg_verify_requests(verifs):
    arr = (KzgVerifyReq * max(len(verifs), 1))()
    for i, v in enumerate(verifs):
        if len(v) != 5:
            raise ValueError("kzg_verify_batch_device: reply %d has %d fields, want 5" % (i, len(v)))
        comp, idx, coef, n, alpha = v
        alpha = bytes(alpha)
        if len(alpha) > 32:
            raise ValueError("kzg_verify_batch_device: alpha of reply %d is longer than 32 bytes" % i)
        arr[i] = KzgVerifyReq(comp or None, idx or None, coef or None, n, (ctypes.c_uint8 * 32)(*alpha.rjust(32, b"\0")))
    return arr


def kzg_verify_batch_device(verifs, d_records, weights=None, stream=0):
    k = len(verifs)
    arr = kzg_verify_requests(verifs)
    w = None
    if weights is not None:
        if len(weights) != k:
            raise ValueError("kzg_verify_batch_device: %d weights for %d replies" % (len(weights), k))
        w = b"".join(x.to_bytes(16, "big") if isinstance(x, int) else bytes(x) for x in weights)
        if len(w) != 16 * k:
            raise ValueError("kzg_verify_batch_device: every weight is 16 bytes")
    status = ctypes.create_string_buffer(max(k, 1))
    _check(lib.porla_kzg_verify_batch_device(arr, k, ctypes.c_void_p(d_records or None), w, status, ctypes.c_void_p(stream)))
    return list(status.raw[:k])


def kzg_digest_batch_device(d_rows, n_rows, d_out, stream=0):
    _check(lib.porla_kzg_digest_batch_device(ctypes.c_void_p(d_rows), n_rows, ctypes.c_void_p(d_out), ctypes.c_void_p(stream)))


def kzg_complement_batch_device(d_scalars, n, d_out, stream=0):
    _check(lib.porla_kzg_complement_batch_device(ctypes.c_void_p(d_scalars), n, ctypes.c_void_p(d_out), ctypes.c_void_p(stream)))


def kzg_mac_batch_device(d_rows, d_scalars, n_rows, d_out, stream=0):
    _check(lib.porla_kzg_mac_batch_device(ctypes.c_void_p(d_rows), ctypes.c_void_p(d_scalars), n_rows, ctypes.c_void_p(d_out),
                                          ctypes.c_void_p(stream)))


def kzg_digest_batch_host(rows, n_rows):
    out = ctypes.create_string_buffer(64 * n_rows)
    _check(lib.porla_kzg_digest_batch_host(rows, n_rows, out))
    return out.raw


def kzg_complement_batch_host(scalars, n):
    out = ctypes.create_string_buffer(64 * n)
    _check(lib.porla_kzg_complement_batch_host(scalars, n, out))
    return out.raw


def kzg_mac_batch_host(rows, scalars, n_rows):
    out = ctypes.create_string_buffer(64 * n_rows)
    _check(lib.porla_kzg_mac_batch_host(rows, scalars, n_rows, out))
    return out.raw


def profile_enable(on=True):
    lib.porla_gpu_profile_enable(int(on))


def kzg_row_coefficients():
    n = ctypes.c_size_t(0)
    _check(lib.porla_kzg_row_coefficients(ctypes.byref(n)))
    return n.value


def kzg_commit_shape():
    c, w = ctypes.c_int(0), ctypes.c_int(0)
    lib.porla_kzg_commit_shape(ctypes.byref(c), ctypes.byref(w))
    return c.value, w.value


def last_msm_shape():
    c, w, g = ctypes.c_int(0), ctypes.c_int(0), ctypes.c_int(0)
    lib.porla_gpu_last_msm_shape(ctypes.byref(c), ctypes.byref(w), ctypes.byref(g))
    return c.value, w.value, bool(g.value)


def profile_get():
    res = []
    i = 0
    while True:
        name = ctypes.create_string_buffer(64)
        ms = ctypes.c_double(0)
        cnt = ctypes.c_longlong(0)
        if lib.porla_gpu_profile_get(i, name, 64, ctypes.byref(ms), ctypes.byref(cnt)) != 0:
            break
        res.append((name.value.decode(), ms.value, cnt.value))
        i += 1
    return res
```

Measured before the change: 785.2 Mmul/s.

## Group tree tail bits on GPU and publish MSM completion via polled host header

The reduction-tree tail kernel now pre-combines each window's per-bit sums into groups of bits on the device, so the host fold has fewer points to process. The kernel also publishes a sequence word into mapped host memory through a last-block atomic, letting the host spin-poll instead of waiting on an event. Per-level device-wide fences become workgroup-only by default, and single-lane copies are widened to quad-lane vector copies. It adds timing stamps and diagnostic APIs, at the cost of extra in-kernel serial doubling work and host spin-polling CPU time.

```diff
diff --git a/include/porla_gpu.h b/include/porla_gpu.h
--- a/include/porla_gpu.h
+++ b/include/porla_gpu.h
@@ -30,6 +30,8 @@
 int         porla_gpu_set_msm_small(int on, int window_bits);
 int         porla_gpu_set_msm_glv(int on);
 int         porla_gpu_last_msm_shape(int *c, int *windows, int *glv);
+int         porla_gpu_msm_tail_stamps(double *wait_us, double *fold_us, double *affine_us);
+int         porla_gpu_msm_completion_word(int slot, unsigned int *header_word, unsigned int *workspace_seq);
 int         porla_diag_fe_op(int op, int modulus, const uint8_t a_le[32], const uint8_t b_le[32], uint8_t out_le[32]);
 int         porla_glv_split(int curve, const uint8_t scalar_be[32], uint8_t k1_mag_be[16], int *k1_neg,
                             uint8_t k2_mag_be[16], int *k2_neg);
diff --git a/porla_amd/csrc/engine.hip b/porla_amd/csrc/engine.hip
--- a/porla_amd/csrc/engine.hip
+++ b/porla_amd/csrc/engine.hip
@@ -98,6 +98,7 @@
 int g_small_mode = getenv("PORLA_MSM_SMALL") ? atoi(getenv("PORLA_MSM_SMALL")) : 1;
 int g_small_c = 0;
 int g_last_shape[3] = {0, 0, 0};
+thread_local MsmTailStamps g_tail_stamps;
 int g_last_multi[2] = {0, 0};
 std::mutex g_multi_mu;
 int g_use_glv = -1;
@@ -132,6 +133,12 @@
     return PORLA_OK;
 }
 
+template <class M>
+static void affine_out_stamped(uint8_t* out, const XYZZ<M>& tot) {
+    const double t0 = tail_clock_us();
+    h_affine_to_bytes<M>(out, h_xyzz_to_affine64<M>(tot));
+    g_tail_stamps.affine_us = tail_clock_us() - t0;
+}
 template <class C>
 static int abi_msm_device(const void* d_scalars, const void* d_points, size_t n, uint8_t* out, void* stream, bool jac) {
     using M = typename C::Fp;
@@ -140,7 +147,7 @@
     int rc = msm_device<C>((const uint8_t*)d_scalars, (const uint8_t*)d_points, n, (hipStream_t)stream, &tot);
     if (rc) return rc;
     if (jac) h_xyzz_to_jac_bytes<M>(out, tot);
-    else h_affine_to_bytes<M>(out, h_xyzz_to_affine64<M>(tot));
+    else affine_out_stamped<M>(out, tot);
     return PORLA_OK;
 }
 template <class C>
@@ -309,7 +316,7 @@
         (void)hipSetDevice(w->device);
         Buf* bufs[] = {&w->pts, &w->keys, &w->entries, &w->counts, &w->starts, &w->fill, &w->cursor, &w->buckets, &w->in_scalars,
                        &w->in_points, &w->order, &w->blk_hist, &w->blk_off, &w->tile_off, &w->heavy, &w->chunk_out, &w->tree_s,
-                       &w->tree_m, &w->tree_mt, &w->small_part, &w->multi_acc, &w->batch_list, &w->batch_part, &w->batch_sums,
+                       &w->tree_m, &w->tree_mt, &w->tree_done, &w->small_part, &w->multi_acc, &w->batch_list, &w->batch_part, &w->batch_sums,
                        &w->batch_ctrl, &w->batch_out};
         for (Buf* b : bufs) b->release();
         w->batch_list_h.release();
@@ -330,6 +337,22 @@
     if (c) *c = g_last_shape[0];
     if (windows) *windows = g_last_shape[1];
     if (glv) *glv = g_last_shape[2];
+    return PORLA_OK;
+}
+int porla_gpu_msm_tail_stamps(double* wait_us, double* fold_us, double* affine_us) {
+    if (wait_us) *wait_us = g_tail_stamps.wait_us;
+    if (fold_us) *fold_us = g_tail_stamps.fold_us;
+    if (affine_us) *affine_us = g_tail_stamps.affine_us;
+    return PORLA_OK;
+}
+int porla_gpu_msm_completion_word(int slot, unsigned int* header_word, unsigned int* workspace_seq) {
+    Workspace* ws = nullptr;
+    int rc = get_workspace_slot(slot, &ws);
+    if (rc) return rc;
+    std::lock_guard<std::mutex> lk(ws->mu);
+    if (!ws->h_windows) { set_last_error("porla: this workspace slot has not run an MSM yet"); return PORLA_ERR_STATE; }
+    if (header_word) *header_word = __atomic_load_n((const uint32_t*)ws->h_windows, __ATOMIC_ACQUIRE);
+    if (workspace_seq) *workspace_seq = ws->small_seq;
     return PORLA_OK;
 }
 int porla_gpu_set_msm_small(int on, int window_bits) {
@@ -497,7 +520,7 @@
     int rc = msm_device_end<Bn254G1>(slot, &tot);
     if (rc) return rc;
     if (jacobian) h_xyzz_to_jac_bytes<Bn254Fp>(out, tot);
-    else h_affine_to_bytes<Bn254Fp>(out, h_xyzz_to_affine64<Bn254Fp>(tot));
+    else affine_out_stamped<Bn254Fp>(out, tot);
     return PORLA_OK;
 }
 
@@ -513,7 +536,7 @@
     int rc = msm_device_end<Secp256k1G>(slot, &tot);
     if (rc) return rc;
     if (jacobian) h_xyzz_to_jac_bytes<Secp256k1Fp>(out, tot);
-    else h_affine_to_bytes<Secp256k1Fp>(out, h_xyzz_to_affine64<Secp256k1Fp>(tot));
+    else affine_out_stamped<Secp256k1Fp>(out, tot);
     return PORLA_OK;
 }
 
diff --git a/porla_amd/csrc/engine.hpp b/porla_amd/csrc/engine.hpp
--- a/porla_amd/csrc/engine.hpp
+++ b/porla_amd/csrc/engine.hpp
@@ -1,5 +1,6 @@
 #pragma once
 #include <hip/hip_runtime.h>
+#include <chrono>
 #include <cstddef>
 #include <cstdint>
 #include <mutex>
@@ -169,6 +170,7 @@
     Buf small_part;
     uint32_t small_seq = 0;
     Buf tree_s, tree_m, tree_mt;
+    Buf tree_done;
     Buf multi_acc;
     hipEvent_t merged = nullptr;
     void* h_windows = nullptr;
@@ -181,6 +183,7 @@
     int slot = 0;
     hipEvent_t done = nullptr;
     int pend_W = 0, pend_c = 0;
+    int pend_g = 0;
     bool lone = false;
     bool pair_pending = false;
     bool begun = false;
@@ -252,6 +255,11 @@
 extern int g_last_multi[2];
 extern int g_last_shape[3];
 extern int g_use_glv;
+struct MsmTailStamps { double wait_us = 0, fold_us = 0, affine_us = 0; };
+extern thread_local MsmTailStamps g_tail_stamps;
+static inline double tail_clock_us() {
+    return std::chrono::duration<double, std::micro>(std::chrono::steady_clock::now().time_since_epoch()).count();
+}
 int get_workspace(Workspace** out);
 int get_workspace_slot(int slot, Workspace** out);
 int lease_blocking_slot(Workspace** out);
diff --git a/porla_amd/csrc/host_fold64.hpp b/porla_amd/csrc/host_fold64.hpp
--- a/porla_amd/csrc/host_fold64.hpp
+++ b/porla_amd/csrc/host_fold64.hpp
@@ -427,4 +427,36 @@
     return F.to(acc);
 }
 
-}
+template <class M>
+inline XYZZ<M> h_fold_tree_grouped64(const XYZZ<M>* fin, int W, int c, int g) {
+    static const Fp64<M> F;
+    const int nbit = c - 1, ng = (nbit + g - 1) / g;
+    typename Fp64<M>::Pt acc = F.inf();
+    for (int w = W - 1; w >= 0; w--) {
+        const XYZZ<M>* f = fin + (size_t)w * ng;
+        if (!Fp64<M>::is_zero(acc.zz)) acc = F.dbl(acc);
+        for (int j = ng - 1; j >= 0; j--) {
+            const int bits = nbit - g * j < g ? nbit - g * j : g;
+            for (int d = 0; d < bits && !Fp64<M>::is_zero(acc.zz); d++) acc = F.dbl(acc);
+            acc = F.padd(acc, F.from(f[j]));
+        }
+    }
+    return F.to(acc);
+}
+template <class M>
+inline void h_group_tree_bits64(const XYZZ<M>* fin, int W, int c, int g, XYZZ<M>* out) {
+    static const Fp64<M> F;
+    const int nbit = c - 1, ng = (nbit + g - 1) / g;
+    for (int w = 0; w < W; w++) {
+        const XYZZ<M>* f = fin + (size_t)w * c;
+        for (int j = 0; j < ng; j++) {
+            const int lo = g * j, top = lo + g - 1 < nbit - 1 ? lo + g - 1 : nbit - 1;
+            typename Fp64<M>::Pt acc = F.from(f[1 + top]);
+            for (int k = top - 1; k >= lo; k--) acc = F.padd(F.dbl(acc), F.from(f[1 + k]));
+            if (j == 0) acc = F.padd(acc, F.from(f[0]));
+            out[(size_t)w * ng + j] = F.to(acc);
+        }
+    }
+}
+
+}
diff --git a/porla_amd/csrc/msm.hip.h b/porla_amd/csrc/msm.hip.h
--- a/porla_amd/csrc/msm.hip.h
+++ b/porla_amd/csrc/msm.hip.h
@@ -772,7 +772,7 @@
 template <class M>
 __device__ __forceinline__ TreeOp<M> tree_op(const TreeLevelArgs<M>& a, uint32_t s, uint32_t i, uint32_t jp, uint32_t jo) {
     TreeOp<M> o;
-    o.final = a.last != 0;
+    o.final = a.last == 1;
     o.copy = (s == a.l + 1);
     if (o.copy) {
         o.pa = a.s_prev + 2 * (size_t)i + 1; o.pb = o.pa;
@@ -805,7 +805,12 @@
     using M = typename C::Fp;
     const TreeOp<M> o = tree_op<M>(a, s, i, jp, jo);
     if (o.copy) {
-        if (live && (lane & 3u) == 0u) Node<C>::store_final(o.out, Node<C>::load(o.pa));
+        if (live && !o.final) {
+            const uint4* q = reinterpret_cast<const uint4*>(reinterpret_cast<const uint32_t*>(o.pa) + 8 * (lane & 3u));
+            uint4* d = reinterpret_cast<uint4*>(reinterpret_cast<uint32_t*>(o.out) + 8 * (lane & 3u));
+            const uint4 v0 = q[0], v1 = q[1];
+            d[0] = v0; d[1] = v1;
+        } else if (live && (lane & 3u) == 0u) Node<C>::store_final(o.out, Node<C>::load(o.pa));
         return;
     }
     xyzz30_add_quad<M>(o.pa, o.pb, o.out, o.final, live, lane);
@@ -867,11 +872,33 @@
     uint32_t l0;
     uint32_t nlev;
 };
-template <class C, bool QUAD>
-__global__ void __launch_bounds__(512)
-k_tree_tail(TreeTailArgs<typename C::Fp> a) {
+template <class M>
+struct TreeTailExt {
+    XYZZ<M>* bits;
+    uint32_t group_bits;
+    uint32_t* arrivals;
+    uint32_t arrive_total;
+    uint32_t* hdr;
+    uint32_t seq, hdr_W;
+    uint32_t wg_fence;
+};
+
+__device__ __forceinline__ void publish_when_last(uint32_t* counter, uint32_t total, uint32_t* hdr, uint32_t seq, uint32_t w1, uint32_t w2,
+                                                  uint32_t w3) {
+    const uint32_t old = atomicAdd(counter, 1u);
+    if (old == total - 1) {
+        *counter = 0;
+        hdr[1] = w1; hdr[2] = w2; hdr[3] = w3;
+        __threadfence_system();
+        __atomic_store_n(&hdr[0], seq, __ATOMIC_RELEASE);
+    }
+}
+
+template <class C, bool QUAD, bool EXT>
+__device__ __forceinline__ void tree_tail_body(const TreeTailArgs<typename C::Fp>& a, const TreeTailExt<typename C::Fp>& x) {
     using M = typename C::Fp;
     const uint32_t w = blockIdx.x;
+    const bool grouped = EXT && x.group_bits != 0;
     for (uint32_t l = a.l0; l < a.nlev; l++) {
         const uint32_t nw = a.B >> (l + 1);
         TreeLevelArgs<M> lv;
@@ -884,11 +911,12 @@
         lv.s_out = a.s_lev[l];
         lv.m_out = a.m_tail[l & 1] + (size_t)w * a.per_window;
         lv.m_out_stride = nw;
-        lv.fin = a.fin;
+        lv.fin = grouped ? x.bits : a.fin;
         lv.l = l;
         lv.nlev = a.nlev;
-        lv.last = (l + 1 == a.nlev) ? 1u : 0u;
-        const uint32_t tasks = (l + 1 + lv.last) * nw;
+        const bool last = l + 1 == a.nlev;
+        lv.last = last ? (grouped ? 2u : 1u) : 0u;
+        const uint32_t tasks = (l + 1 + (last ? 1u : 0u)) * nw;
         if constexpr (QUAD) {
             const uint32_t per_pass = blockDim.x >> 2;
             for (uint32_t t0 = 0; t0 < tasks; t0 += per_pass) {
@@ -904,9 +932,49 @@
                 tree_task<C>(lv, t / nw, i, first ? i : j, j);
             }
         }
-        __threadfence();
+        if (!(EXT && x.wg_fence)) __threadfence();
         __syncthreads();
     }
+    if constexpr (EXT && QUAD) {
+        if (grouped) {
+            const uint32_t g = x.group_bits, nbit = a.nlev, ng = (nbit + g - 1) / g;
+            const uint32_t lane = threadIdx.x & 63u, q = threadIdx.x >> 2;
+            const bool wave0 = threadIdx.x < 64u;
+            const bool mine = wave0 && q < ng;
+            const uint32_t j = mine ? q : 0u;
+            const uint32_t lo = g * j, top = (lo + g - 1 < nbit - 1) ? lo + g - 1 : nbit - 1;
+            XYZZ<M>* bits = x.bits + (size_t)w * (a.nlev + 1);
+            XYZZ<M>* out = a.fin + (size_t)w * ng + j;
+            XYZZ<M>* acc = bits + 1 + top;
+            for (uint32_t i = g - 1; i-- > 0;) {
+                const bool act = mine && lo + i < top;
+                if (wave0) xyzz30_dbl_quad<M>(acc, acc, act, lane);
+                __syncthreads();
+                const bool fin_here = act && i == 0u && j != 0u;
+                if (wave0) xyzz30_add_quad<M>(acc, bits + 1 + (act ? lo + i : top), fin_here ? out : acc, fin_here, act, lane);
+                __syncthreads();
+            }
+            if (mine && j == 0u) xyzz30_add_quad<M>(acc, bits, out, true, true, lane);
+            else if (mine && top == lo && (lane & 3u) == 0u) Node<C>::store_final(out, Node<C>::load(acc));
+        }
+    }
+    if constexpr (EXT) {
+        if (x.hdr) {
+            if (!grouped || threadIdx.x < 64u) __threadfence_system();
+            __syncthreads();
+            if (threadIdx.x == 0) publish_when_last(x.arrivals, x.arrive_total, x.hdr, x.seq, x.hdr_W, a.nlev + 1, x.group_bits);
+        }
+    }
+}
+template <class C, bool QUAD>
+__global__ void __launch_bounds__(512)
+k_tree_tail(TreeTailArgs<typename C::Fp> a) {
+    tree_tail_body<C, QUAD, false>(a, TreeTailExt<typename C::Fp>{});
+}
+template <class C>
+__global__ void __launch_bounds__(512)
+k_tree_tail_ext(TreeTailArgs<typename C::Fp> a, TreeTailExt<typename C::Fp> x) {
+    tree_tail_body<C, true, true>(a, x);
 }
 
 template <class C>
diff --git a/porla_amd/csrc/msm_impl.hip.h b/porla_amd/csrc/msm_impl.hip.h
--- a/porla_amd/csrc/msm_impl.hip.h
+++ b/porla_amd/csrc/msm_impl.hip.h
@@ -103,19 +103,37 @@
     ws->pend_c = 0;
     return PORLA_OK;
 }
+static inline bool poll_sequence(const volatile uint32_t* hdr, uint32_t seq) {
+    const auto t_spin = std::chrono::steady_clock::now();
+    for (uint32_t it = 0;; it++) {
+        if (__atomic_load_n((const uint32_t*)&hdr[0], __ATOMIC_ACQUIRE) == seq) return true;
+        __builtin_ia32_pause();
+        if ((it & 1023u) == 1023u && std::chrono::steady_clock::now() - t_spin > std::chrono::milliseconds(2)) return false;
+    }
+}
+static inline int msm_group_bits() {
+    static const int v = [] {
+        const char* e = getenv("PORLA_MSM_GROUP_BITS");
+        const int g = e ? atoi(e) : TREE_GROUP_BITS;
+        return (g == 0 || (g >= 2 && g <= 8)) ? g : TREE_GROUP_BITS;
+    }();
+    return v;
+}
+static inline int msm_tail_wg_fence() {
+    static const int v = (getenv("PORLA_MSM_TAIL_WG_FENCE") && getenv("PORLA_MSM_TAIL_WG_FENCE")[0] == '0') ? 0 : 1;
+    return v;
+}
+static inline bool msm_poll_completion() {
+    static const bool v = !(getenv("PORLA_MSM_POLL") && getenv("PORLA_MSM_POLL")[0] == '0');
+    return v;
+}
+
 template <class C>
 static int msm_small_pair_finish(Workspace* ws, int which, XYZZ<typename C::Fp>* total) {
     using M = typename C::Fp;
     const uint8_t* region = (const uint8_t*)ws->h_windows + (size_t)which * SMALL_PAIR_STRIDE;
     const volatile uint32_t* hdr = (const volatile uint32_t*)region;
-    const auto t_spin = std::chrono::steady_clock::now();
-    bool seen = false;
-    for (uint32_t it = 0;; it++) {
-        if (__atomic_load_n((const uint32_t*)&hdr[0], __ATOMIC_ACQUIRE) == ws->small_seq) { seen = true; break; }
-        __builtin_ia32_pause();
-        if ((it & 1023u) == 1023u && std::chrono::steady_clock::now() - t_spin > std::chrono::milliseconds(2)) break;
-    }
-    if (!seen) PORLA_HIP(hipEventSynchronize(ws->done));
+    if (!poll_sequence(hdr, ws->small_seq)) PORLA_HIP(hipEventSynchronize(ws->done));
     const int W = (int)hdr[1], c = (int)hdr[2];
     if (hdr[0] != ws->small_seq || W < 1 || c < 1 || c > SMALL_MAX_C || (size_t)W * c * sizeof(XYZZ<M>) + SMALL_HDR_WORDS * 4 > SMALL_PAIR_STRIDE) {
         set_last_error("porla: the single-launch MSM pair left no valid result header");
@@ -303,20 +321,35 @@
     static thread_local int plan_c = 0, plan_W = 0, plan_lone = -1;
     if (plan_c != c || plan_W != W || plan_lone != (ws->lone ? 1 : 0)) {
         plan_c = 0;
-        const std::string refused = tree_plan(plan, c, W, ws->lone, C::F30_LAZY);
+        TreeOptions opt;
+        opt.group_bits = msm_group_bits();
+        opt.tail_wg_fence = msm_tail_wg_fence();
+        const std::string refused = tree_plan(plan, c, W, ws->lone, C::F30_LAZY, opt);
         if (!refused.empty()) { set_last_error("porla: reduction tree: " + refused); return PORLA_ERR_STATE; }
         plan_c = c; plan_W = W; plan_lone = ws->lone ? 1 : 0;
     }
     if ((rc = ws->tree_s.ensure(plan.s_entries * sizeof(XYZZ<M>)))) return rc;
     if ((rc = ws->tree_m.ensure(plan.m_entries * sizeof(XYZZ<M>)))) return rc;
     if ((rc = ws->tree_mt.ensure(plan.mt_entries * sizeof(XYZZ<M>)))) return rc;
-    if (ws->h_windows_cap < (size_t)W * c * sizeof(XYZZ<M>) || ws->h_windows_cap < 64 * 1024) {
+    const size_t fin_bytes = SMALL_HDR_WORDS * 4 + plan.fin_entries * sizeof(XYZZ<M>);
+    if (ws->h_windows_cap < fin_bytes || ws->h_windows_cap < 64 * 1024) {
         if (ws->h_windows) PORLA_HIP(hipHostFree(ws->h_windows));
-        ws->h_windows_cap = 64 * 1024;
+        ws->h_windows_cap = fin_bytes > 64 * 1024 ? fin_bytes : 64 * 1024;
         PORLA_HIP(hipHostMalloc(&ws->h_windows, ws->h_windows_cap, hipHostMallocMapped | hipHostMallocCoherent));
     }
     void* h_windows_dev = nullptr;
     PORLA_HIP(hipHostGetDevicePointer(&h_windows_dev, ws->h_windows, 0));
+    if (ws->tree_done.cap < 256) {
+        if ((rc = ws->tree_done.ensure(256))) return rc;
+        PORLA_HIP(hipMemsetAsync(ws->tree_done.p, 0, 256, stream));
+    }
+    ws->small_seq++;
+    if (ws->small_seq == 0) ws->small_seq = 1;
+    ((volatile uint32_t*)ws->h_windows)[0] = 0;
+    TreeCompletion done;
+    done.arrivals = (uint32_t*)ws->tree_done.p;
+    done.hdr = (uint32_t*)h_windows_dev;
+    done.seq = ws->small_seq;
     const int parts = (int)plan.parts;
     if (parts == 2) {
         if (!ws->aux_stream) PORLA_HIP(hipStreamCreateWithFlags(&ws->aux_stream, hipStreamNonBlocking));
@@ -326,7 +359,7 @@
         PORLA_HIP(hipStreamWaitEvent(ws->aux_stream, ws->fork_ev, 0));
     }
     PORLA_HIP((tree_enqueue<C, ProfScope>(plan, buckets, (XYZZ<M>*)ws->tree_s.p, (XYZZ<M>*)ws->tree_m.p, (XYZZ<M>*)ws->tree_mt.p,
-                                          (XYZZ<M>*)h_windows_dev, stream, ws->aux_stream)));
+                                          (XYZZ<M>*)((uint8_t*)h_windows_dev + SMALL_HDR_WORDS * 4), stream, ws->aux_stream, done)));
     if (parts == 2) {
         PORLA_HIP(hipEventRecord(ws->join_ev, ws->aux_stream));
         PORLA_HIP(hipStreamWaitEvent(stream, ws->join_ev, 0));
@@ -335,6 +368,7 @@
     PORLA_HIP(hipEventRecord(ws->done, stream));
     ws->pend_W = W;
     ws->pend_c = c;
+    ws->pend_g = (int)plan.group_bits;
     g_last_shape[0] = c; g_last_shape[1] = W; g_last_shape[2] = glv ? 1 : 0;
     return PORLA_OK;
 }
@@ -345,14 +379,7 @@
     if (ws->pend_W == 0) { *total = xyzz_inf<M>(); return PORLA_OK; }
     if (ws->pend_W < 0) {
         const volatile uint32_t* hdr = (const volatile uint32_t*)ws->h_windows;
-        const auto t_spin = std::chrono::steady_clock::now();
-        bool seen = false;
-        for (uint32_t it = 0;; it++) {
-            if (__atomic_load_n((const uint32_t*)&hdr[0], __ATOMIC_ACQUIRE) == ws->small_seq) { seen = true; break; }
-            __builtin_ia32_pause();
-            if ((it & 1023u) == 1023u && std::chrono::steady_clock::now() - t_spin > std::chrono::milliseconds(2)) break;
-        }
-        if (!seen) PORLA_HIP(hipEventSynchronize(ws->done));
+        if (!poll_sequence(hdr, ws->small_seq)) PORLA_HIP(hipEventSynchronize(ws->done));
         const int W = (int)hdr[1], c = (int)hdr[2];
         ws->pend_W = 0;
         if (hdr[0] != ws->small_seq || W < 1 || c < 1 || c > SMALL_MAX_C || (size_t)W * c * sizeof(XYZZ<M>) + SMALL_HDR_WORDS * 4 > ws->h_windows_cap) {
@@ -363,9 +390,20 @@
         *total = h_fold_tree64<M>((const XYZZ<M>*)((const uint8_t*)ws->h_windows + SMALL_HDR_WORDS * 4), W, c);
         return PORLA_OK;
     }
-    PORLA_HIP(hipEventSynchronize(ws->done));
-    *total = h_fold_tree64<M>((const XYZZ<M>*)ws->h_windows, ws->pend_W, ws->pend_c);
+    const double t_in = tail_clock_us();
+    const volatile uint32_t* hdr = (const volatile uint32_t*)ws->h_windows;
+    const int W = ws->pend_W, c = ws->pend_c, g = ws->pend_g;
     ws->pend_W = 0;
+    if (!msm_poll_completion() || !poll_sequence(hdr, ws->small_seq)) PORLA_HIP(hipEventSynchronize(ws->done));
+    if (__atomic_load_n((const uint32_t*)&hdr[0], __ATOMIC_ACQUIRE) != ws->small_seq || (int)hdr[1] != W || (int)hdr[2] != c || (int)hdr[3] != g) {
+        set_last_error("porla: the MSM's reduction tree left no valid result header");
+        return PORLA_ERR_HIP;
+    }
+    const double t_woke = tail_clock_us();
+    const XYZZ<M>* fin = (const XYZZ<M>*)((const uint8_t*)ws->h_windows + SMALL_HDR_WORDS * 4);
+    *total = g ? h_fold_tree_grouped64<M>(fin, W, c, g) : h_fold_tree64<M>(fin, W, c);
+    g_tail_stamps.wait_us = t_woke - t_in;
+    g_tail_stamps.fold_us = tail_clock_us() - t_woke;
     return PORLA_OK;
 }
 
diff --git a/porla_amd/csrc/msm_small.hip.h b/porla_amd/csrc/msm_small.hip.h
--- a/porla_amd/csrc/msm_small.hip.h
+++ b/porla_amd/csrc/msm_small.hip.h
@@ -392,15 +392,7 @@
     SMALL_STAMP(9);
     __threadfence_system();
     __syncthreads();
-    if (tid == 0) {
-        const uint32_t old = atomicAdd(&counters[SMALL_DONE_SLOT], 1u);
-        if (old == (uint32_t)win.g.W - 1) {
-            counters[SMALL_DONE_SLOT] = 0;
-            hdr[1] = (uint32_t)win.g.W; hdr[2] = (uint32_t)c; hdr[3] = (uint32_t)win.g.glv;
-            __threadfence_system();
-            __atomic_store_n(&hdr[0], seq, __ATOMIC_RELEASE);
-        }
-    }
-}
-
-}
+    if (tid == 0) publish_when_last(&counters[SMALL_DONE_SLOT], (uint32_t)win.g.W, hdr, seq, (uint32_t)win.g.W, (uint32_t)c, (uint32_t)win.g.glv);
+}
+
+}
diff --git a/porla_amd/csrc/msm_tree.hip.h b/porla_amd/csrc/msm_tree.hip.h
--- a/porla_amd/csrc/msm_tree.hip.h
+++ b/porla_amd/csrc/msm_tree.hip.h
@@ -22,7 +22,13 @@
     int front2 = -1;
     long long quad_max_tasks = -1;
     int l0 = -1;
-};
+    int group_bits = 0;
+    int tail_wg_fence = 0;
+};
+constexpr int TREE_GROUP_BITS = 2;
+static inline uint32_t tree_fin_per_window(uint32_t c, uint32_t group_bits) {
+    return group_bits ? (c - 1 + group_bits - 1) / group_bits : c;
+}
 
 enum TreeKind : uint32_t { TREE_FRONT2 = 0, TREE_LEVEL = 1, TREE_LEVEL_QUAD = 2, TREE_TAIL = 3 };
 static inline const char* tree_kind_name(uint32_t k) {
@@ -44,10 +50,13 @@
     size_t m_tail[2];
     size_t fin;
     uint32_t per_window, nb, B, nlev;
+    size_t bits;
 };
 
 struct TreePlan {
     uint32_t c, W, lone, parts, nlev, B;
+    uint32_t group_bits = 0, fin_per_window = 0;
+    uint32_t tail_wg_fence = 0;
     size_t s_entries, m_entries, mt_entries, fin_entries;
     struct Part { uint32_t w0, Wp, l0, front2; unsigned long long quad_max; } part[2];
     std::vector<TreeLaunch> launches;
@@ -64,7 +73,14 @@
     p.s_entries = nb + 2;
     p.m_entries = 2 * (nb / 4) + 6;
     p.mt_entries = 2 * (size_t)W * (B / 4 + 1) + 4;
-    p.fin_entries = (size_t)W * c;
+    if (o.group_bits != 0 && (o.group_bits < 2 || o.group_bits > 8)) return "group_bits must be 0 or 2 .. 8";
+    if (o.tail_wg_fence != 0 && o.tail_wg_fence != 1) return "tail_wg_fence must be 0 or 1";
+    p.group_bits = (uint32_t)o.group_bits;
+    p.tail_wg_fence = (uint32_t)o.tail_wg_fence;
+    p.fin_per_window = tree_fin_per_window((uint32_t)c, p.group_bits);
+    p.fin_entries = (size_t)W * p.fin_per_window;
+    const size_t bits_at = p.mt_entries;
+    if (p.group_bits) p.mt_entries += (size_t)W * c;
     const int parts = o.parts >= 0 ? o.parts : ((lone && W >= 4 && nb >= ((size_t)1 << 18)) ? 2 : 1);
     if (parts != 1 && parts != 2) return "parts must be 1 or 2";
     if (parts == 2 && W < 2) return "two parts need at least two windows";
@@ -123,7 +139,8 @@
             t.m_global = m_half[(l0 + 1) & 1];
             t.per_window = B / 4 + 1;
             t.m_tail[0] = mt_off; t.m_tail[1] = mt_off + (size_t)Wp * t.per_window + 1;
-            t.fin = (size_t)w0 * c;
+            t.fin = (size_t)w0 * p.fin_per_window;
+            t.bits = p.group_bits ? bits_at + (size_t)w0 * c : 0;
             uint32_t need = (l0 + 2) * (B >> (l0 + 1)) * 4u;
             uint32_t threads = (need + 63) / 64 * 64;
             if (threads > tree_tail_threads()) threads = tree_tail_threads();
@@ -139,10 +156,16 @@
 
 struct TreeNoScope { TreeNoScope(const char*, hipStream_t) {} };
 
+struct TreeCompletion {
+    uint32_t* arrivals = nullptr;
+    uint32_t* hdr = nullptr;
+    uint32_t seq = 0;
+};
+
 template <class C, class Scope = TreeNoScope>
 static hipError_t tree_enqueue(const TreePlan& p, const XYZZ<typename C::Fp>* buckets, XYZZ<typename C::Fp>* s_area,
                                XYZZ<typename C::Fp>* m_area, XYZZ<typename C::Fp>* mt_area, XYZZ<typename C::Fp>* fin,
-                               hipStream_t st0, hipStream_t st1) {
+                               hipStream_t st0, hipStream_t st1, const TreeCompletion& done = TreeCompletion()) {
     using M = typename C::Fp;
     static_assert(C::F30_LAZY, "the tree's quad forms read the reduced-radix memory form");
     size_t at = 0;
@@ -178,7 +201,17 @@
             t.m_tail[0] = mt_area + q.m_tail[0]; t.m_tail[1] = mt_area + q.m_tail[1];
             t.fin = fin + q.fin;
             t.nb = q.nb; t.B = q.B; t.l0 = q.l; t.nlev = q.nlev;
-            hipLaunchKernelGGL((k_tree_tail<C, true>), dim3(q.grid), dim3(q.block), 0, st, t);
+            if (p.group_bits || p.tail_wg_fence || done.hdr) {
+                TreeTailExt<M> x;
+                x.bits = mt_area + q.bits;
+                x.group_bits = p.group_bits;
+                x.arrivals = done.arrivals; x.arrive_total = p.W;
+                x.hdr = done.hdr; x.seq = done.seq; x.hdr_W = p.W;
+                x.wg_fence = p.tail_wg_fence;
+                hipLaunchKernelGGL((k_tree_tail_ext<C>), dim3(q.grid), dim3(q.block), 0, st, t, x);
+            } else {
+                hipLaunchKernelGGL((k_tree_tail<C, true>), dim3(q.grid), dim3(q.block), 0, st, t);
+            }
         }
         const hipError_t e = hipGetLastError();
         if (e != hipSuccess) return e;
@@ -192,6 +225,10 @@
     snprintf(b, sizeof b, "plan c=%u W=%u lone=%u parts=%u nlev=%u B=%u s_entries=%zu m_entries=%zu mt_entries=%zu fin_entries=%zu tail_threads=%u\n",
              p.c, p.W, p.lone, p.parts, p.nlev, p.B, p.s_entries, p.m_entries, p.mt_entries, p.fin_entries, tree_tail_threads());
     out += b;
+    if (p.group_bits || p.tail_wg_fence) {
+        snprintf(b, sizeof b, "grouped group_bits=%u fin_per_window=%u tail_wg_fence=%u\n", p.group_bits, p.fin_per_window, p.tail_wg_fence);
+        out += b;
+    }
     for (uint32_t i = 0; i < p.parts; i++) {
         snprintf(b, sizeof b, "part part=%u w0=%u Wp=%u l0=%u front2=%u quad_max=%llu\n", i, p.part[i].w0, p.part[i].Wp, p.part[i].l0,
                  p.part[i].front2, p.part[i].quad_max);
@@ -211,6 +248,7 @@
                  q.per_window, q.fin, q.nb, q.B, q.nlev);
         out += b;
         for (uint32_t l = 0; l < q.nlev; l++) { snprintf(b, sizeof b, "%s%zu", l ? "," : "", q.s_lev[l]); out += b; }
+        if (p.group_bits) { snprintf(b, sizeof b, " bits=%zu", q.bits); out += b; }
         out += "\n";
     }
     return out;
diff --git a/porla_amd/loader.py b/porla_amd/loader.py
--- a/porla_amd/loader.py
+++ b/porla_amd/loader.py
@@ -241,6 +241,9 @@
     L.porla_gpu_set_msm_glv.argtypes = [ctypes.c_int]; L.porla_gpu_set_msm_glv.restype = ctypes.c_int
     L.porla_gpu_set_msm_small.argtypes = [ctypes.c_int, ctypes.c_int]; L.porla_gpu_set_msm_small.restype = ctypes.c_int
     L.porla_gpu_last_msm_shape.argtypes = [ctypes.POINTER(ctypes.c_int)] * 3; L.porla_gpu_last_msm_shape.restype = ctypes.c_int
+    L.porla_gpu_msm_tail_stamps.argtypes = [ctypes.POINTER(ctypes.c_double)] * 3; L.porla_gpu_msm_tail_stamps.restype = ctypes.c_int
+    L.porla_gpu_msm_completion_word.argtypes = [ctypes.c_int] + [ctypes.POINTER(ctypes.c_uint)] * 2
+    L.porla_gpu_msm_completion_word.restype = ctypes.c_int
     L.porla_glv_split.argtypes = [ctypes.c_int, u8p, u8p, ctypes.POINTER(ctypes.c_int), u8p, ctypes.POINTER(ctypes.c_int)]
     L.porla_glv_split.restype = ctypes.c_int
     L.porla_diag_fe_op.argtypes = [ctypes.c_int, ctypes.c_int, u8p, u8p, u8p]; L.porla_diag_fe_op.restype = ctypes.c_int
diff --git a/porla_amd/multiexp.py b/porla_amd/multiexp.py
--- a/porla_amd/multiexp.py
+++ b/porla_amd/multiexp.py
@@ -801,6 +801,22 @@
     return c.value, w.value, bool(g.value)
 
 
+def msm_tail_stamps():
+    w, f, a = ctypes.c_double(0), ctypes.c_double(0), ctypes.c_double(0)
+    lib.porla_gpu_msm_tail_stamps(ctypes.byref(w), ctypes.byref(f), ctypes.byref(a))
+    return w.value, f.value, a.value
+
+
+def msm_completion_word(slot):
+    h, q = ctypes.c_uint(0), ctypes.c_uint(0)
+    _check(lib.porla_gpu_msm_completion_word(slot, ctypes.byref(h), ctypes.byref(q)))
+    return h.value, q.value
+
+
+def set_msm_window(c):
+    _check(lib.porla_gpu_set_msm_window(c))
+
+
 def profile_get():
     res = []
     i = 0
```

Measured after the change: 791.2 Mmul/s (median of 6 runs). No clear change (+0.8%).
